# tungphambasement/DCNN

Hardware: AMD Instinct MI355X
Metric: images/sec (whole node) ResNet-18 Tiny-ImageNet training at 1/2/4/8 MI355X (higher is better)
Workload: dtype bf16; 1 GPU; model=resnet18_tiny_imagenet, global_batch=256, per_gpu_batch=256, parallelism=dp1, optimizer=adam, hipgraph=True, engine=native (C++ host API)

## Files before the change

### dcnn_amd/csrc/host/dcnn/nn.hpp

```cpp
#pragma once
#include <cmath>
#include <functional>
#include <map>
#include <memory>
#include <string>
#include <vector>

#include "json.hpp"
#include "ops.hpp"
#include "tensor.hpp"

namespace dcnn {

struct ParamArena;
struct OptimSegments;
struct Param {
  std::string name;
  std::vector<int64_t> shape;
  Layout layout = Layout::NCHW;
  Tensor value, grad, shadow;
  Tensor m, v;
  Tensor ema;
  bool no_decay = false;
  std::shared_ptr<ParamArena> arena;
};

struct ParamArena {
  Tensor value, grad, m, v, shadow;
  size_t n = 0, count = 0;
  Tensor nodecay;
  Tensor ema;
  std::shared_ptr<const OptimSegments> segments[2];
  Tensor seg_chunks, seg_info[2];
  Tensor wt_table;
  int n_wt = 0;
  long wt_tiles = 0;
  bool wt_valid = false;
  void refresh_transposes();
};

class Layer {
 public:
  explicit Layer(std::string name) : name_(std::move(name)) {}
  virtual ~Layer() = default;
  virtual std::string type() const = 0;
  virtual json::Value parameters_config() const = 0;
  virtual std::vector<int64_t> output_shape(const std::vector<int64_t>& in) const = 0;
  virtual void build(const std::vector<int64_t>& in, Device dev, uint64_t seed) { (void)in; (void)seed; dev_ = dev; }
  virtual Tensor forward(const Tensor& x, bool training) = 0;
  virtual Tensor backward(const Tensor& dy) = 0;
  virtual void sync_shadow();
  virtual void collect_params(std::vector<Param*>& out) {
    for (auto& p : params_) out.push_back(&p);
  }
  virtual void collect_layers(std::vector<Layer*>& out) { out.push_back(this); }
  std::vector<Param>& params() { return params_; }
  const std::string& name() const { return name_; }
  Device device() const { return dev_; }
  virtual void set_micro_batch(int mb) { mb_ = mb; }
  void clear_caches() { caches_.clear(); }
  void set_input_grad(bool b) { input_grad_ = b; }
  bool input_grad() const { return input_grad_; }
  virtual bool takes_raw_input(const std::vector<int64_t>& in) const { (void)in; return false; }
  virtual double flops(const std::vector<int64_t>& in) const { (void)in; return 0; }

 protected:
  struct MbCache {
    Tensor a, b, c, d;
    std::vector<int64_t> shape;
    uint64_t u = 0;
    bool flag = false;
  };
  MbCache& mbc() { return caches_[mb_]; }
  std::map<int, MbCache> caches_;
  int mb_ = 0;
  bool input_grad_ = true;
  Param& add_param(const std::string& n, const std::vector<int64_t>& shape, Layout phys, const std::vector<float>& init);
  std::string name_;
  Device dev_ = Device::cpu();
  std::vector<Param> params_;
};

class ConvBase : public Layer {
 public:
  std::vector<int64_t> output_shape(const std::vector<int64_t>& in) const override;
  void build(const std::vector<int64_t>& in, Device dev, uint64_t seed) override;
  Tensor forward(const Tensor& x, bool training) override;
  Tensor backward(const Tensor& dy) override { return backward_impl(dy, nullptr); }
  double flops(const std::vector<int64_t>& in) const override;
  virtual bool backward_residual(const Tensor& dy, const Tensor& residual, Tensor& dx) {
    (void)dy; (void)residual; (void)dx;
    return false;
  }
  int stride_h() const { return sh_; }
  int stride_w() const { return sw_; }

 protected:
  ConvBase(int in_ch, int out_ch, int kh, int kw, int groups, int sh, int sw, int ph, int pw, bool bias,
           std::string name)
      : Layer(std::move(name)), ci_(in_ch), co_(out_ch), kh_(kh), kw_(kw), g_(groups), sh_(sh), sw_(sw), ph_(ph),
        pw_(pw), bias_(bias) {}
  ConvShape shape_for(const std::vector<int64_t>& in) const;
  void geometry_config(json::Value& p) const;
  const float* bias_value() const { return bias_ ? params_[1].value.ptr<float>() : nullptr; }
  float* bias_grad() { return bias_ ? params_[1].grad.ptr<float>() : nullptr; }
  virtual bool depthwise() const { return false; }
  int group_in() const { return depthwise() ? 1 : ci_ / g_; }
  Tensor backward_impl(const Tensor& dy, const Tensor* residual);
  int ci_, co_, kh_, kw_, g_, sh_, sw_, ph_, pw_;
  bool bias_;
};

class Conv2D : public ConvBase {
 public:
  Conv2D(int in_ch, int out_ch, int kh, int kw, int sh = 1, int sw = 1, int ph = 0, int pw = 0, bool bias = true,
         std::string name = "conv2d");
  std::string type() const override { return "conv2d"; }
  json::Value parameters_config() const override;
  Tensor forward(const Tensor& x, bool training) override;
  Tensor backward(const Tensor& dy) override;
  bool takes_raw_input(const std::vector<int64_t>& in) const override;
  void set_stats_consumer(class BatchNorm* bn) { stats_to_ = bn; }
  void set_bnb_producer(class BatchNorm* bn) { bnb_from_ = bn; }
  void set_block_bnb_producer(class BatchNorm* bn) { bnb_block_from_ = bn; }
  bool backward_residual(const Tensor& dy, const Tensor& residual, Tensor& dx) override;
  bool compact_grad_ok() const;
  Tensor backward_compact(const Tensor& dy);
  bool takes_compact_residual(int sh, int sw) const;
  bool ran_stem() const;
  void backward_stem_bn(const Tensor& dy, const gpu_ops::StemBn& bn);
  void sync_shadow() override;
  bool make_transposed_operand(std::vector<int64_t>& row, long& tiles);

 private:
  class BatchNorm* stats_to_ = nullptr;
  class BatchNorm* bnb_from_ = nullptr;
  class BatchNorm* bnb_block_from_ = nullptr;
  Tensor wt_;
  const void* dgrad_operand(bool& transposed) const;
};

class DepthwiseConv2D : public ConvBase {
 public:
  DepthwiseConv2D(int channels, int kh, int kw, int sh = 1, int sw = 1, int ph = 0, int pw = 0, bool bias = true,
                  std::string name = "depthwise_conv2d");
  std::string type() const override { return "depthwise_conv2d"; }
  json::Value parameters_config() const override;
  bool backward_residual(const Tensor& dy, const Tensor& residual, Tensor& dx) override;

 protected:
  bool depthwise() const override { return true; }
};

class GroupedConv2D : public ConvBase {
 public:
  GroupedConv2D(int in_ch, int out_ch, int kh, int kw, int groups, int sh = 1, int sw = 1, int ph = 0, int pw = 0,
                bool bias = true, std::string name = "grouped_conv2d");
  std::string type() const override { return "grouped_conv2d"; }
  json::Value parameters_config() const override;
  bool backward_residual(const Tensor& dy, const Tensor& residual, Tensor& dx) override;
};

class Dense : public Layer {
 public:
  Dense(int in_features, int out_features, bool bias = true, std::string name = "dense");
  std::string type() const override { return "dense"; }
  json::Value parameters_config() const override;
  std::vector<int64_t> output_shape(const std::vector<int64_t>& in) const override;
  void build(const std::vector<int64_t>& in, Device dev, uint64_t seed) override;
  Tensor forward(const Tensor& x, bool training) override;
  Tensor backward(const Tensor& dy) override;
  double flops(const std::vector<int64_t>& in) const override { return 6.0 * in[0] * in_ * out_; }
  void set_head_pool(class Pool2D* p) { head_pool_ = p; }
  bool run_head(const Tensor& x, const PoolShape& p, Tensor& pooled);
  bool is_head_dx(const Tensor& dy, bool take);

 private:
  int in_, out_;
  bool bias_;
  class Pool2D* head_pool_ = nullptr;
};

class BatchNorm : public Layer {
 public:
  explicit BatchNorm(int num_features, float eps = 1e-5f, float momentum = 0.1f, bool affine = true,
                     std::string name = "batchnorm");
  std::string type() const override { return "batchnorm"; }
  json::Value parameters_config() const override;
  std::vector<int64_t> output_shape(const std::vector<int64_t>& in) const override { return in; }
  double flops(const std::vector<int64_t>& in) const override {
    return 15.0 * (double)in[0] * (double)in[1] * (double)in[2] * (double)in[3];
// ... 87 lines not shown
  Tensor forward(const Tensor& x, bool training) override;
  Tensor backward(const Tensor& dy) override;

 private:
  int c_;
  float eps_;
  bool affine_;
};

class LayerScale : public Layer {
 public:
  explicit LayerScale(int num_channels, float init_value = 1e-6f, std::string name = "layer_scale");
  std::string type() const override { return "layer_scale"; }
  json::Value parameters_config() const override;
  std::vector<int64_t> output_shape(const std::vector<int64_t>& in) const override { return in; }
  void build(const std::vector<int64_t>& in, Device dev, uint64_t seed) override;
  Tensor forward(const Tensor& x, bool training) override { return forward_residual(x, nullptr, training); }
  Tensor forward_residual(const Tensor& x, const Tensor* residual, bool training, const Tensor* mask = nullptr);
  Tensor backward(const Tensor& dy) override;

 private:
  int c_;
  float init_;
};

class DropPath : public Layer {
 public:
  explicit DropPath(float rate, std::string name = "drop_path", bool has_seed = false, uint64_t seed = 0);
  std::string type() const override { return "drop_path"; }
  json::Value parameters_config() const override;
  std::vector<int64_t> output_shape(const std::vector<int64_t>& in) const override { return in; }
  double flops(const std::vector<int64_t>& in) const override;
  void build(const std::vector<int64_t>& in, Device dev, uint64_t seed) override;
  Tensor forward(const Tensor& x, bool training) override;
  Tensor backward(const Tensor& dy) override;
  float rate() const { return p_; }
  uint64_t mask_seed() const { return has_seed_ ? explicit_seed_ : seed_; }
  const Tensor* draw_mask(int64_t N, bool training);
  const Tensor& last_mask() { return mbc().a; }
  Tensor& draw_counter() { return ctr_; }

 private:
  float p_;
  bool has_seed_;
  uint64_t explicit_seed_, seed_ = 0, draws_ = 0;
  Tensor ctr_;
};

class Dropout : public Layer {
 public:
  explicit Dropout(float rate = 0.5f, std::string name = "dropout");
  std::string type() const override { return "dropout"; }
  json::Value parameters_config() const override;
  std::vector<int64_t> output_shape(const std::vector<int64_t>& in) const override { return in; }
  void build(const std::vector<int64_t>& in, Device dev, uint64_t seed) override;
  Tensor forward(const Tensor& x, bool training) override;
  Tensor backward(const Tensor& dy) override;

 private:
  float p_;
  uint64_t seed_ = 0, draw_ = 0;
};

class Pool2D : public Layer {
 public:
  Pool2D(bool max, int kh, int kw, int sh, int sw, int ph, int pw, std::string name);
  std::string type() const override { return max_ ? "maxpool2d" : "avgpool2d"; }
  json::Value parameters_config() const override;
  std::vector<int64_t> output_shape(const std::vector<int64_t>& in) const override;
  Tensor forward(const Tensor& x, bool training) override;
  Tensor backward(const Tensor& dy) override;
  bool is_max() const { return max_; }
  PoolShape shape_for(const std::vector<int64_t>& in) const;
  void set_fused_producer(class BatchNorm* bn) { bn_ = bn; }
  uint8_t* accept_prepooled(const Tensor& ypool, const std::vector<int64_t>& in);
  void clear_prepooled() { mbc().flag = false; }
  void set_head_dense(class Dense* d) { head_ = d; }

 private:
  class BatchNorm* bn_ = nullptr;
  class Dense* head_ = nullptr;
  bool max_;
  int kh_, kw_, sh_, sw_, ph_, pw_;
};

class Flatten : public Layer {
 public:
  explicit Flatten(std::string name = "flatten") : Layer(std::move(name)) {}
  std::string type() const override { return "flatten"; }
  json::Value parameters_config() const override { return json::Value::object(); }
  std::vector<int64_t> output_shape(const std::vector<int64_t>& in) const override;
  Tensor forward(const Tensor& x, bool training) override;
  Tensor backward(const Tensor& dy) override;
  void set_head_dense(class Dense* d) { head_ = d; }

 private:
  class Dense* head_ = nullptr;
};

class ResidualBlock : public Layer {
 public:
  ResidualBlock(std::vector<std::unique_ptr<Layer>> main, std::vector<std::unique_ptr<Layer>> shortcut,
                std::string activation = "relu", std::string name = "residual_block");
  std::string type() const override { return "residual_block"; }
  json::Value parameters_config() const override;
  std::vector<int64_t> output_shape(const std::vector<int64_t>& in) const override;
  double flops(const std::vector<int64_t>& in) const override;
  void build(const std::vector<int64_t>& in, Device dev, uint64_t seed) override;
  Tensor forward(const Tensor& x, bool training) override;
  Tensor backward(const Tensor& dy) override;
  void sync_shadow() override;
  void collect_params(std::vector<Param*>& out) override;
  void collect_layers(std::vector<Layer*>& out) override;
  void set_micro_batch(int mb) override;
  const std::vector<std::unique_ptr<Layer>>& main_path() const { return main_; }
  const std::vector<std::unique_ptr<Layer>>& shortcut_path() const { return short_; }
  class BatchNorm* fused_tail() const;
  class Conv2D* head_conv() const;
  class BatchNorm* dual_shortcut() const;
  class LayerScale* scale_tail() const;
  class DropPath* drop_tail() const;

 private:
  std::vector<std::unique_ptr<Layer>> main_, short_;
  std::string act_;
};

std::unique_ptr<Layer> create_layer(const json::Value& rec);

void fuse_bn_relu(std::vector<std::unique_ptr<Layer>>& seq, bool on);
void fuse_blocks(std::vector<std::unique_ptr<Layer>>& seq, bool on);

class Sequential {
 public:
  explicit Sequential(std::string name = "sequential") : name_(std::move(name)) {}
  Sequential(Sequential&&) = default;
  Sequential& operator=(Sequential&&) = default;
  void add(std::unique_ptr<Layer> l) { layers_.push_back(std::move(l)); }
  void set_input_shape(const std::vector<int64_t>& chw) { input_chw_ = chw; }
  void set_device(Device d);
  Device device() const { return dev_; }
  void initialize(uint64_t seed = 0);
  void set_training(bool t) { training_ = t; }
  bool is_training() const { return training_; }
  Tensor forward(const Tensor& x, int mb = 0);
  void backward(const Tensor& dlogits, int mb = 0);
  Tensor forward_activation(const Tensor& x, int mb);
  Tensor backward_activation(const Tensor& g, int mb);
  Tensor input_activation(const Tensor& x) const;
  std::vector<Param*> parameters();
  std::vector<double> layer_flops(const std::vector<int64_t>& in) const;
  std::vector<BatchNorm*> batchnorms();
  void zero_grad();
  size_t num_parameters();
  const std::vector<std::unique_ptr<Layer>>& layers() const { return layers_; }
  const std::string& name() const { return name_; }
  void set_backward_hook(std::function<void(size_t)> f) { bwd_hook_ = std::move(f); }

  json::Value get_config() const;
  void print_config() const;
  static Sequential load_from_config(const json::Value& cfg);
  void save_to_file(const std::string& path) const;
  void load_weights_file(const std::string& path);
  void load_bn_stats(const std::string& path);
  static Sequential from_file(const std::string& path, Device dev = Device::cpu());

 private:
  std::string name_;
  std::vector<std::unique_ptr<Layer>> layers_;
  std::vector<int64_t> input_chw_;
  Device dev_ = Device::cpu();
  bool training_ = true;
  bool initialized_ = false;
  std::shared_ptr<ParamArena> arena_;
  std::function<void(size_t)> bwd_hook_;
  void pack_params();
};

class SequentialBuilder {
 public:
  explicit SequentialBuilder(std::string name = "sequential") : model_(std::move(name)) {}
  SequentialBuilder& input(const std::vector<int64_t>& chw);
  SequentialBuilder& conv2d(int out_ch, int kh, int kw, int sh = 1, int sw = 1, int ph = 0, int pw = 0,
                            bool bias = true, const std::string& name = "");
  SequentialBuilder& depthwise_conv2d(int kh, int kw, int sh = 1, int sw = 1, int ph = 0, int pw = 0, bool bias = true,
                                      const std::string& name = "");
  SequentialBuilder& grouped_conv2d(int out_ch, int kh, int kw, int groups, int sh = 1, int sw = 1, int ph = 0,
                                    int pw = 0, bool bias = true, const std::string& name = "");
  SequentialBuilder& batchnorm(float eps = 1e-5f, float momentum = 0.1f, bool affine = true,
                               const std::string& name = "");
  SequentialBuilder& activation(const std::string& kind = "relu", const std::string& name = "");
  SequentialBuilder& maxpool2d(int kh, int kw, int sh = 0, int sw = 0, int ph = 0, int pw = 0,
                               const std::string& name = "");
  SequentialBuilder& avgpool2d(int kh, int kw, int sh = 1, int sw = 1, int ph = 0, int pw = 0,
                               const std::string& name = "");
  SequentialBuilder& flatten(const std::string& name = "");
  SequentialBuilder& dense(int out_features, bool bias = true, const std::string& name = "");
  SequentialBuilder& groupnorm(int num_groups, float eps = 1e-5f, bool affine = true, const std::string& name = "");
  SequentialBuilder& dropout(float rate, const std::string& name = "");
  SequentialBuilder& drop_path(float rate, const std::string& name = "");
  SequentialBuilder& layernorm(float eps = 1e-6f, bool affine = true, const std::string& name = "");
  SequentialBuilder& layer_scale(float init_value = 1e-6f, const std::string& name = "");
  SequentialBuilder& convnext_block(int channels, float layer_scale_init = 1e-6f, const std::string& name = "",
                                    float drop_path = 0.f, bool has_seed = false, uint64_t drop_path_seed = 0);
  SequentialBuilder& convnext_downsample(int out_ch, const std::string& name = "convnext_downsample");
  SequentialBuilder& residual(std::vector<std::unique_ptr<Layer>> main, std::vector<std::unique_ptr<Layer>> shortcut,
                              const std::string& activation = "relu", const std::string& name = "");
  SequentialBuilder& basic_residual_block(int in_ch, int out_ch, int stride = 1, const std::string& name = "");
  SequentialBuilder& bottleneck_residual_block(int in_ch, int mid_ch, int out_ch, int stride = 1,
                                               const std::string& name = "");
  SequentialBuilder& resnext_bottleneck_block(int in_ch, int mid_ch, int out_ch, int groups, int stride = 1,
                                              const std::string& name = "");
  Sequential build();

 private:
  std::string auto_name(const std::string& given, const std::string& kind);
  int conv_in() const;
  SequentialBuilder& add_conv(std::unique_ptr<Layer> l);
  Sequential model_;
  std::vector<int64_t> cur_;
  int count_ = 0;
};

struct LossResult {
  double loss = 0;
  long correct = 0;
  Tensor grad;
};
LossResult softmax_cross_entropy(const Tensor& logits, const Tensor& labels);

class Optimizer {
 public:
  explicit Optimizer(float lr) : lr_(lr) {}
  virtual ~Optimizer() = default;
  virtual void step(const std::vector<Param*>& params) = 0;
  void set_learning_rate(float lr) { lr_ = lr; }
  float learning_rate() const { return lr_; }
  void set_max_grad_norm(float max_norm);
  float max_grad_norm() const { return max_norm_; }
  void set_ema_decay(float decay);
  float ema_decay() const { return ema_decay_; }
  void set_no_decay_norm_bias(bool on) { no_decay_ = on; }
  bool no_decay_norm_bias() const { return no_decay_; }
  void prepare(const std::vector<Param*>& params);
  void swap_ema(const std::vector<Param*>& params);
  float last_grad_norm() const;
  virtual bool capturable() const { return false; }
  virtual long step_count() const { return t_; }
  virtual void set_step_count(long t) { t_ = t; }
  virtual void before_replay();
  virtual void upload_hyper();

 protected:
  bool tail() const { return max_norm_ > 0.f || ema_decay_ > 0.f; }
  const float* launch_norm(ParamArena* a);
  const double* host_coef(const std::vector<Param*>& params);
  template <class Owner>
  float* ema_of(Owner* x) const {
    return ema_decay_ > 0.f ? x->ema.template ptr<float>() : nullptr;
  }
  void sync_hyper(ParamArena* a, const char* what);
  float lr_;
  float max_norm_ = 0.f, ema_decay_ = 0.f;
  bool no_decay_ = false;
  long t_ = 0;
  Tensor norm_;
  float host_norm_ = std::nanf("");
  double host_coef_ = 1.0;
  Tensor hyper_;
  float hyper_lr_ = -1.f;
  long hyper_t_ = -1;
};

class SGD : public Optimizer {
 public:
  explicit SGD(float lr, float momentum = 0.f) : Optimizer(lr), momentum_(momentum) {}
  void step(const std::vector<Param*>& params) override;
  float momentum() const { return momentum_; }

 private:
  float momentum_;
};

class Adam : public Optimizer {
 public:
  explicit Adam(float lr, float b1 = 0.9f, float b2 = 0.999f, float eps = 1e-8f, float wd = 0.f,
                bool decoupled = false)
      : Optimizer(lr), b1_(b1), b2_(b2), eps_(eps), wd_(wd), decoupled_(decoupled) {}
  void step(const std::vector<Param*>& params) override;
  bool capturable() const override { return true; }
  void before_replay() override;

 protected:
  float b1_, b2_, eps_, wd_;
  bool decoupled_;
};

class LayerwiseState {
 public:
  std::vector<float> last_trust_ratios() const;

 protected:
  void workspace(ParamArena* a);
  struct One {
    std::vector<int> chunks, segs;
  };
  static One one_segment(long n, bool adapt);
  template <class StepOne>
  void step_each(const std::vector<Param*>& params, const char* who, bool no_decay, StepOne step_one);
  Tensor part_, out_;
  size_t nsegs_ = 0;
  std::vector<double> trust_;
};

class LAMB : public Adam, public LayerwiseState {
 public:
  explicit LAMB(float lr = 1e-3f, double b1 = 0.9, double b2 = 0.999, float eps = 1e-6f, float wd = 0.01f)
      : Adam(lr, (float)b1, (float)b2, eps, wd, false), b1d_(b1), b2d_(b2) {}
  void step(const std::vector<Param*>& params) override;

 private:
  double b1d_, b2d_;
};

class LARS : public SGD, public LayerwiseState {
 public:
  explicit LARS(float lr = 0.1f, float momentum = 0.9f, float wd = 5e-4f, float trust_coefficient = 1e-3f,
                float eps = 1e-8f)
      : SGD(lr, momentum), wd_(wd), tc_(trust_coefficient), eps_(eps) {}
  void step(const std::vector<Param*>& params) override;
  bool capturable() const override { return true; }

 private:
  float wd_, tc_, eps_;
};


class DataSource {
 public:
  virtual ~DataSource() = default;
  virtual void reset(uint64_t epoch) = 0;
  virtual bool next(int batch, Tensor& x, Tensor& labels) = 0;
  virtual size_t size() const = 0;
};

class SyntheticClassification : public DataSource {
 public:
  SyntheticClassification(size_t n, int c, int h, int w, int classes, uint64_t seed, float noise = 0.5f);
  void reset(uint64_t epoch) override;
  bool next(int batch, Tensor& x, Tensor& labels) override;
  size_t size() const override { return n_; }

 private:
  size_t n_;
  int c_, h_, w_, classes_;
  uint64_t seed_;
  float noise_;
  std::vector<float> proto_;
  std::vector<size_t> order_;
  size_t pos_ = 0;
};

struct TrainingConfig {
  int epochs = 1;
  int batch_size = 64;
  int max_steps = -1;
  int progress_interval = 50;
  float lr_decay = 1.0f;
  uint64_t seed = 0;
};

struct EpochStats {
  double train_loss = 0, train_acc = 0, val_loss = 0, val_acc = 0, seconds = 0;
};

LossResult train_step(Sequential& model, Optimizer& opt, const Tensor& x, const Tensor& labels);
EpochStats evaluate(Sequential& model, DataSource& src, int batch_size);
std::vector<EpochStats> train_classification_model(Sequential& model, DataSource& train, DataSource* val,
                                                   Optimizer& opt, const TrainingConfig& cfg);

}
```

### dcnn_amd/csrc/host/dcnn/ops.hpp

```cpp
#pragma once
#include <cstdint>

namespace dcnn {

struct ConvShape {
  int N, C, H, W, Co, KH, KW, SH, SW, PH, PW, OH, OW;
};
struct PoolShape {
  int N, C, H, W, OH, OW, KH, KW, SH, SW, PH, PW;
};
enum ActKind {
  ACT_RELU = 0, ACT_LEAKY_RELU = 1, ACT_ELU = 2, ACT_SIGMOID = 3, ACT_TANH = 4, ACT_LINEAR = 5,
  ACT_GELU = 6
};

struct MixPlan {
  int mode;
  double lam;
  int yl, yh, xl, xh;
};

namespace cpu_ops {
void conv_fwd(const float* x, const float* w, const float* b, float* y, const ConvShape& s);
void conv_bwd(const float* x, const float* w, const float* dy, float* dx, float* dw, float* db, const ConvShape& s);
void dwconv_fwd(const float* x, const float* w, const float* b, float* y, const ConvShape& s);
void dwconv_bwd(const float* x, const float* w, const float* dy, float* dx, float* dw, float* db, const ConvShape& s);
void gconv_fwd(const float* x, const float* w, const float* b, float* y, const ConvShape& s, int groups);
void gconv_bwd(const float* x, const float* w, const float* dy, float* dx, float* dw, float* db, const ConvShape& s,
               int groups);
void dense_fwd(const float* x, const float* w, const float* b, float* y, long N, long In, long Out);
void dense_bwd(const float* x, const float* w, const float* dy, float* dx, float* dw, float* db, long N, long In,
               long Out);
void bn_fwd(const float* x, float* y, long N, long C, long HW, const float* g, const float* b, float eps, bool train,
            float* rmean, float* rvar, float momentum, float* smean, float* sistd);
void bn_bwd(const float* x, const float* dy, const float* mean, const float* istd, const float* g, float* dx,
            float* dg, float* db, long N, long C, long HW, bool train);
void maxpool_fwd(const float* x, float* y, int32_t* idx, const PoolShape& p);
void maxpool_bwd(const float* dy, const int32_t* idx, float* dx, const PoolShape& p);
void avgpool_fwd(const float* x, float* y, const PoolShape& p);
void avgpool_bwd(const float* dy, float* dx, const PoolShape& p);
void act_fwd(int kind, const float* x, float* y, long n, float alpha);
void act_bwd(int kind, const float* x, const float* dy, float* dx, long n, float alpha);
double softmax_ce(const float* pred, const int64_t* labels, float* grad, long N, long C, long* correct);
double loss(int kind, const float* pred, const float* target, const int64_t* labels, float* grad, long N, long C,
            float param, long* correct);
void groupnorm_fwd(const float* x, float* y, long N, long C, long HW, long G, const float* g, const float* b, float eps,
                   float* smean, float* sistd);
void groupnorm_bwd(const float* x, const float* dy, const float* mean, const float* istd, const float* g, float* dx,
                   float* dg, float* db, long N, long C, long HW, long G);
void layernorm_fwd(const float* x, float* y, long N, long C, long HW, const float* g, const float* b, float eps,
                   float* smean, float* srstd);
void layernorm_bwd(const float* x, const float* dy, const float* mean, const float* rstd, const float* g, float* dx,
                   float* dg, float* db, long N, long C, long HW);
void layer_scale_fwd(const float* x, const float* g, const float* residual, float* y, long N, long C, long HW);
void layer_scale_bwd(const float* x, const float* dy, const float* g, float* dx, float* dg, long N, long C, long HW);
void softmax_fwd(const float* x, float* y, long N, long C, long HW);
void softmax_bwd(const float* y, const float* dy, float* dx, long N, long C, long HW);
void dropout(const float* x, float* y, long n, float p, uint64_t seed);
void add(const float* a, const float* b, float* y, long n, bool relu);
void relu_mask(const float* dy, const float* y, float* dx, long n);
void adam(float* p, const float* g, float* m, float* v, long n, float lr, float b1, float b2, float eps, float bc1,
          float bc2, float wd, bool decoupled);
void sgd(float* p, const float* g, float* vel, long n, float lr, float momentum);
double grad_sumsq(const float* g, long n);
void adam_tail(float* p, const float* g, float* m, float* v, long n, float lr, float b1, float b2, float eps, float bc1,
               float bc2, float wd, bool decoupled, const uint8_t* nodecay, const double* coef, float* ema,
               float decay);
void sgd_tail(float* p, const float* g, float* vel, long n, float lr, float momentum, const double* coef, float* ema,
              float decay);
void ema_swap(float* a, float* b, long n);
void lamb(float* p, const float* g, float* m, float* v, long n, float lr, double b1, double b2, float eps, double bc1,
          double bc2, float wd, const double* coef, float* ema, float decay, const int* chunks, int nchunks,
          const int* segs, int nsegs, double* out);
void lars(float* p, const float* g, float* vel, long n, float lr, float momentum, float wd, float tc, float eps,
          const double* coef, float* ema, float decay, const int* chunks, int nchunks, const int* segs, int nsegs,
          double* out);
void drop_path_mask(float* mask, long N, float p, uint64_t seed, uint64_t draw);
void drop_path_scale(const float* x, const float* mask, float* y, long N, long row);
MixPlan mix_plan(uint64_t seed, uint64_t step, int H, int W, double mixup_alpha, double cutmix_alpha, double prob,
                 double switch_prob);
void mix_batch(float* x, const int64_t* labels, float* target, long B, long C, long H, long W, int mode, double lam,
               int yl, int yh, int xl, int xh, long K);
}

namespace gpu_ops {
void begin_deferred_reduce();
void end_deferred_reduce();
void flush_deferred_reduce();
void set_fault(int f);
void input_to_nhwc(const float* x, void* y, int N, int C, int HW);
void nhwc_to_nchw(const void* x, void* y, int N, int HW, int C);
void nchw_to_nhwc_bf16(const void* x, void* y, int N, int HW, int C);
void cast_bf16(const float* x, void* y, long n);
void zero(void* p, long nbytes);
const float* conv_fwd(const void* x, const void* w, const float* bias, void* y, const ConvShape& s,
                      int* stat_rows = nullptr);
struct BnbOperands {
  const void* y;
  const void* x;
  const float* mean;
  const float* istd;
  const float* gamma = nullptr;
  const float* beta = nullptr;
  bool mask_from_x = false;
};
struct DgradOpts {
  bool residual_compact = false;
  bool dense_g2 = false;
};
const float* conv_dgrad(const void* dy, const void* w, void* dx, const ConvShape& s, const void* residual = nullptr,
                        bool w_transposed = false, const BnbOperands* bnb = nullptr, int* bnb_rows = nullptr,
                        DgradOpts opt = {});
bool conv_dgrad_takes_compact(const ConvShape& s);
void conv_dgrad_compact(const void* dy, const void* w, void* dxc, const ConvShape& s, bool w_transposed);
bool compact_shortcut_grad_enabled();
void weight_transpose(const void* w, void* wt, int Co, int T, int C);
void multi_weight_transpose(const int64_t* table, int n, long max_tiles);
void conv_wgrad(const void* dy, const void* x, float* gw, float* gb, const ConvShape& s);
void dwconv_fwd(const void* x, const void* w, const float* bias, void* y, const ConvShape& s);
void dwconv_dgrad(const void* dy, const void* w, void* dx, const ConvShape& s, const void* residual = nullptr);
void dwconv_wgrad(const void* dy, const void* x, float* gw, float* gb, const ConvShape& s);
void gconv_fwd(const void* x, const void* w, const float* bias, void* y, const ConvShape& s, int groups);
void gconv_dgrad(const void* dy, const void* w, void* dx, const ConvShape& s, int groups,
                 const void* residual = nullptr);
void gconv_wgrad(const void* dy, const void* x, float* gw, float* gb, const ConvShape& s, int groups);
bool stem_ok(const ConvShape& s);
const float* stem_fwd(const float* x, const void* w, const float* bias, void* y, const ConvShape& s,
                      int* stat_rows = nullptr);
void stem_wgrad(const void* dy, const float* x, float* gw, float* gb, const ConvShape& s);
struct StemBn {
  const void* x;
  const float* mean;
  const float* istd;
  const float* gamma;
  float* dgamma;
  float* dbeta;
  const float* slab;
  int rows;
  bool train;
};
void stem_wgrad_bn(const void* dy, const float* x, float* gw, float* gb, const ConvShape& s, const StemBn& bn);
void dense_fwd(const void* x, const void* w, const float* bias, void* y, int N, int In, int Out);
void dense_dgrad(const void* dy, const void* w, void* dx, int N, int In, int Out);
void dense_wgrad(const void* dy, const void* x, float* gw, float* gb, int N, int In, int Out);
bool head_supported(const PoolShape& p, int Out);
void head_fwd(const void* x, const void* w, const float* bias, void* pooled, void* y, const PoolShape& p, int Out);
void head_bwd(const void* dy, const void* w, const void* pooled, void* dx, float* gw, float* gb, const PoolShape& p,
              int Out);
void bn_fwd(const void* x, void* y, long R, int C, const float* g, const float* b, float eps, bool train,
            float* rmean, float* rvar, float momentum, float* smean, float* sistd, bool relu = false,
            const void* residual = nullptr);
void bn_fwd_slab(const void* x, void* y, long R, int C, const float* slab, int rows, const float* g, const float* b,
                 float eps, float* rmean, float* rvar, float momentum, float* smean, float* sistd, bool relu,
                 const void* residual = nullptr);
void bn_bwd_slab(const void* dy, const void* x, void* dx, long R, int C, const float* mean, const float* istd,
                 const float* g, float* dg, float* db, bool train, const float* slab, int rows);
void bn_bwd(const void* dy, const void* x, void* dx, long R, int C, const float* mean, const float* istd,
            const float* g, float* dg, float* db, bool train, const void* yout = nullptr, void* dy_out = nullptr);
struct SecondaryStats {
  SecondaryStats();
  ~SecondaryStats();
};
struct BnRaw {
  const float* slab;
  int rows;
};
BnRaw bn_stats_raw(const void* x, long R, int C, const float* slab, int rows);
struct BnFwdSide {
  const void* x;
  BnRaw raw;
  const float* g;
  const float* b;
  float eps;
  float* rmean;
  float* rvar;
  float momentum;
  float* smean;
  float* sistd;
};
bool bn_dual_ok(long R, int C);
void bn_fwd_dual(const BnFwdSide& a, const BnFwdSide& b, void* y, long R, int C, bool relu, bool train);
struct BnBwdSides {
  const void* x;
  void* dx;
  const float* mean;
  const float* istd;
  const float* g;
  float* dg;
  float* db;
};
void bn_bwd_dual(const void* dy, const BnBwdSides& a, const float* slab_a, int rows_a, const BnBwdSides& b, long R,
                 int C);
bool bn_relu_maxpool_ok(const PoolShape& p);
void bn_relu_maxpool(const void* x, void* y, uint8_t* idx, const PoolShape& p, const float* slab, int rows,
                     const float* g, const float* b, float eps, float* rmean, float* rvar, float momentum,
                     float* smean, float* sistd);
const float* maxpool_bwd_bnb(const void* dy, const uint8_t* idx, const void* ypool, const void* x, const float* mean,
                             const float* istd, void* dx, const PoolShape& p, int* rows);
void maxpool_fwd(const void* x, void* y, uint8_t* idx, const PoolShape& p);
void maxpool_bwd(const void* dy, const uint8_t* idx, void* dx, const PoolShape& p);
void avgpool_fwd(const void* x, void* y, const PoolShape& p);
void avgpool_bwd(const void* dy, void* dx, const PoolShape& p);
void act_fwd(int kind, const void* x, void* y, long n, float alpha);
void act_bwd(int kind, const void* x, const void* dy, void* dx, long n, float alpha);
double softmax_ce(const void* pred, const int64_t* labels, void* grad, int N, int C, long* correct);
double loss(int kind, const void* pred, const float* target, const int64_t* labels, void* grad, int N, int C,
            float param, long* correct, float grad_scale = 1.f);
void loss_launch(int kind, const void* pred, const float* target, const int64_t* labels, void* grad, int N, int C,
                 float param, float grad_scale = 1.f);
double read_last_loss(long* correct);
void groupnorm_fwd(const void* x, void* y, int N, int HW, int C, int G, const float* g, const float* b, float eps,
                   float* smean, float* sistd);
void groupnorm_bwd(const void* dy, const void* x, void* dx, int N, int HW, int C, int G, const float* g,
                   const float* mean, const float* istd, float* dg, float* db);
void layernorm_fwd(const void* x, void* y, long R, int C, const float* g, const float* b, float eps, float* smean,
                   float* srstd);
void layernorm_bwd(const void* dy, const void* x, void* dx, long R, int C, const float* g, const float* mean,
                   const float* rstd, float* dg, float* db);
void layer_scale_fwd(const void* x, const float* g, const void* residual, void* y, long R, int C);
void layer_scale_bwd(const void* dy, const void* x, const float* g, void* dx, float* dg, long R, int C);
void softmax_fwd(const void* x, void* y, long rows, int C);
void softmax_bwd(const void* y, const void* dy, void* dx, long rows, int C);
void dropout(const void* x, void* y, long n, float p, uint64_t seed);
void add(const void* a, const void* b, void* y, long n, bool relu);
void relu_mask(const void* dy, const void* y, void* dx, long n);
void adam(float* p, const float* g, float* m, float* v, void* shadow, long n, float lr, float b1, float b2, float eps,
          float bc1, float bc2, float wd, bool decoupled);
void sgd(float* p, const float* g, float* vel, void* shadow, long n, float lr, float momentum);
void adam_hyper_step(float* hyper, float b1, float b2);
void adam_dev(float* p, const float* g, float* m, float* v, void* shadow, long n, float b1, float b2, float eps,
              float wd, bool decoupled, const float* hyper, const uint8_t* nodecay);
void grad_norm_workspace(long n);
void grad_sumsq(const float* g, long n, float max_norm, float* out);
void adam_tail(float* p, const float* g, float* m, float* v, void* shadow, long n, float lr, float b1, float b2,
               float eps, float bc1, float bc2, float wd, bool decoupled, const float* hyper, const uint8_t* nodecay,
               const float* coef, float* ema, float decay);
void sgd_tail(float* p, const float* g, float* vel, void* shadow, long n, float lr, float momentum, const float* coef,
              float* ema, float decay);
void ema_swap(float* a, float* b, void* shadow, long n);
void layerwise_workspace();
// ... 21 lines not shown
```

### dcnn_amd/csrc/host/dcnn/tensor.hpp

```cpp
#pragma once
#include <cstdint>
#include <cstring>
#include <iosfwd>
#include <memory>
#include <string>
#include <vector>

#include "layout.hpp"

namespace dcnn {

enum class DeviceType { CPU, GPU };

struct Device {
  DeviceType type = DeviceType::CPU;
  int index = 0;
  static Device cpu() { return {DeviceType::CPU, 0}; }
  static Device gpu(int i = 0) { return {DeviceType::GPU, i}; }
  static Device parse(const std::string& s);
  bool is_gpu() const { return type == DeviceType::GPU; }
  std::string str() const;
  bool operator==(const Device& o) const { return type == o.type && index == o.index; }
  bool operator!=(const Device& o) const { return !(*this == o); }
};

enum class DType { F32, BF16, I32, I64, U8 };
size_t dtype_size(DType t);
const char* dtype_name(DType t);

uint16_t f32_to_bf16(float f);
float bf16_to_f32(uint16_t b);

namespace gpu {
int device_count();
void set_device(int dev);
void* alloc(size_t nbytes);
void free(void* p);
size_t cached_bytes();
void empty_cache();
void copy(void* dst, const void* src, size_t nbytes, int kind);
void copy2_d2d(void* d0, const void* s0, size_t n0, void* d1, const void* s1, size_t n1);
void zero(void* p, size_t nbytes);
void synchronize();

using Flow = void*;
using Event = void*;
Flow flow();
void set_flow(Flow f);
Flow flow_create();
void flow_destroy(Flow f);
void flow_synchronize(Flow f = nullptr);
Event event_create();
void event_destroy(Event e);
void event_record(Event e, Flow f = nullptr);
void flow_wait(Flow f, Event e);
void event_synchronize(Event e);

class Graph {
 public:
  Graph() = default;
  ~Graph();
  Graph(const Graph&) = delete;
  Graph& operator=(const Graph&) = delete;
  void begin();
  void end();
  void replay();
  bool ready() const { return exec_ != nullptr; }
  static bool capturing();

 private:
  void* graph_ = nullptr;
  void* exec_ = nullptr;
  void* pool_ = nullptr;
  Flow flow_ = nullptr;
};
constexpr size_t kIpcHandleBytes = 64;
void* ipc_alloc(size_t nbytes, void* handle_out);
void ipc_free(void* p);
void* ipc_open(const void* handle);
void ipc_close(void* p);
bool stream_values_supported();
Event ipc_event_create(void* handle_out);
Event ipc_event_open(const void* handle);
void flow_write_u32(void* p, uint32_t v);
void flow_wait_u32_geq(void* p, uint32_t v);
}

class Storage {
 public:
  Storage(Device d, size_t nbytes);
  ~Storage();
  Storage(const Storage&) = delete;
  Storage& operator=(const Storage&) = delete;
  void* data() const { return p_; }
  size_t nbytes() const { return n_; }
  Device device() const { return dev_; }

 private:
  Device dev_;
  void* p_ = nullptr;
  size_t n_ = 0;
};

class Tensor {
 public:
  Tensor() = default;
  static Tensor empty(const std::vector<int64_t>& shape, DType dt, Device dev, Layout layout = Layout::NCHW);
  static Tensor zeros(const std::vector<int64_t>& shape, DType dt, Device dev, Layout layout = Layout::NCHW);
  static Tensor from_host(const std::vector<float>& v, const std::vector<int64_t>& shape, Device dev,
                          DType dt = DType::F32, Layout layout = Layout::NCHW);
  static Tensor from_host_i64(const std::vector<int64_t>& v, Device dev);

  bool defined() const { return (bool)st_; }
  const std::vector<int64_t>& shape() const { return shape_; }
  int64_t dim(int k) const { return shape_.at(k); }
  int rank() const { return (int)shape_.size(); }
  int64_t numel() const;
  size_t nbytes() const { return (size_t)numel() * dtype_size(dt_); }
  DType dtype() const { return dt_; }
  Device device() const { return st_ ? st_->device() : Device::cpu(); }
  Layout layout() const { return layout_; }
  void* data() const { return st_ ? static_cast<char*>(st_->data()) + off_ : nullptr; }
  template <typename T>
  T* ptr() const { return static_cast<T*>(data()); }

  Tensor view(const std::vector<int64_t>& shape, Layout layout = Layout::NCHW) const;
  Tensor slice(size_t byte_off, const std::vector<int64_t>& shape, DType dt, Layout layout = Layout::NCHW) const;
  void ensure(const std::vector<int64_t>& shape, DType dt, Device dev, Layout layout = Layout::NCHW);
  Tensor clone() const;
  Tensor to(Device dev) const;
  std::vector<float> to_host_f32() const;
  std::vector<int64_t> to_host_i64() const;
  void zero_();

  void save(std::ostream& os) const;
  static Tensor load(std::istream& is, Device dev = Device::cpu());

 private:
  std::shared_ptr<Storage> st_;
  size_t off_ = 0;
  std::vector<int64_t> shape_;
  DType dt_ = DType::F32;
  Layout layout_ = Layout::NCHW;
};

std::string shape_str(const std::vector<int64_t>& s);

}
```

### dcnn_amd/csrc/host/nn.cpp

```cpp
#include "dcnn/nn.hpp"

#include "../kernels/fusion_plan.h"
#include "../kernels/optim_segments.h"

#include <algorithm>
#include <chrono>
#include <cmath>
#include <cstdio>
#include <cstdlib>
#include <filesystem>
#include <fstream>
#include <iostream>
#include <sstream>
#include <stdexcept>

namespace dcnn {

namespace {
struct Rng {
  uint64_t s;
  explicit Rng(uint64_t seed) : s(seed * 0x9e3779b97f4a7c15ull + 0x632be59bd9b4e019ull) {}
  uint64_t next() {
    uint64_t z = (s += 0x9e3779b97f4a7c15ull);
    z = (z ^ (z >> 30)) * 0xbf58476d1ce4e5b9ull;
    z = (z ^ (z >> 27)) * 0x94d049bb133111ebull;
    return z ^ (z >> 31);
  }
  float uniform() { return (float)((next() >> 40) * (1.0 / 16777216.0)); }
  float normal() {
    const float u1 = std::max(uniform(), 1e-7f), u2 = uniform();
    return std::sqrt(-2.f * std::log(u1)) * std::cos(6.2831853f * u2);
  }
};

std::vector<float> uniform_init(size_t n, float bound, uint64_t seed) {
  Rng r(seed);
  std::vector<float> v(n);
  for (auto& x : v) x = (2.f * r.uniform() - 1.f) * bound;
  return v;
}

Tensor act_empty(const std::vector<int64_t>& shape, Device dev) {
  return dev.is_gpu() ? Tensor::empty(shape, DType::BF16, dev, Layout::NHWC) : Tensor::empty(shape, DType::F32, dev);
}

void check_act(const Tensor& x, Device dev, const char* who) {
  if (x.device() != dev) throw std::runtime_error(std::string(who) + ": input on " + x.device().str() +
                                                  ", layer on " + dev.str());
  if (x.rank() != 4) throw std::runtime_error(std::string(who) + ": expected an (N, C, H, W) tensor");
}

constexpr int ACT_SOFTMAX = 100;

int act_code(const std::string& k) {
  if (k == "softmax") return ACT_SOFTMAX;
  if (k == "relu") return ACT_RELU;
  if (k == "leaky_relu") return ACT_LEAKY_RELU;
  if (k == "elu") return ACT_ELU;
  if (k == "sigmoid") return ACT_SIGMOID;
  if (k == "tanh") return ACT_TANH;
  if (k == "linear") return ACT_LINEAR;
  if (k == "gelu") return ACT_GELU;
  throw std::invalid_argument("unknown activation '" + k + "'");
}
}

Param& Layer::add_param(const std::string& n, const std::vector<int64_t>& shape, Layout phys,
                        const std::vector<float>& init) {
  Param p;
  p.name = n;
  p.shape = shape;
  p.layout = phys;
  p.value = Tensor::from_host(init, shape, dev_, DType::F32, phys);
  p.grad = Tensor::zeros(shape, DType::F32, dev_, phys);
  if (dev_.is_gpu()) {
    p.shadow = Tensor::empty(shape, DType::BF16, dev_, phys);
    gpu_ops::cast_bf16(p.value.ptr<float>(), p.shadow.data(), p.value.numel());
  }
  params_.push_back(std::move(p));
  return params_.back();
}

void Layer::sync_shadow() {
  for (auto& p : params_)
    if (p.shadow.defined()) gpu_ops::cast_bf16(p.value.ptr<float>(), p.shadow.data(), p.value.numel());
}

void ConvBase::geometry_config(json::Value& p) const {
  p["stride_h"] = sh_;
  p["stride_w"] = sw_;
  p["pad_h"] = ph_;
  p["pad_w"] = pw_;
  p["use_bias"] = bias_;
}

ConvShape ConvBase::shape_for(const std::vector<int64_t>& in) const {
  ConvShape s{};
  s.N = (int)in[0];
  s.C = (int)in[1];
  s.H = (int)in[2];
  s.W = (int)in[3];
  s.Co = co_;
  s.KH = kh_;
  s.KW = kw_;
  s.SH = sh_;
  s.SW = sw_;
  s.PH = ph_;
  s.PW = pw_;
  s.OH = (s.H + 2 * ph_ - kh_) / sh_ + 1;
  s.OW = (s.W + 2 * pw_ - kw_) / sw_ + 1;
  if (s.C != ci_) throw std::runtime_error(name_ + ": input has " + std::to_string(s.C) + " channels, expected " +
                                           std::to_string(ci_));
  return s;
}

std::vector<int64_t> ConvBase::output_shape(const std::vector<int64_t>& in) const {
  const ConvShape s = shape_for(in);
  return {in[0], co_, s.OH, s.OW};
}

void ConvBase::build(const std::vector<int64_t>& in, Device dev, uint64_t seed) {
  (void)in;
  dev_ = dev;
  params_.clear();
  const int cig = group_in();
  const float bound = 1.f / std::sqrt((float)(cig * kh_ * kw_));
  const Layout wl = dev.is_gpu() && !depthwise() ? Layout::NHWC : Layout::NCHW;
  add_param("weights", {co_, cig, kh_, kw_}, wl, uniform_init((size_t)co_ * cig * kh_ * kw_, bound, seed));
  if (bias_) add_param("bias", {co_, 1, 1, 1}, Layout::NCHW, uniform_init((size_t)co_, bound, seed + 1)).no_decay = true;
}

double ConvBase::flops(const std::vector<int64_t>& in) const {
  const ConvShape s = shape_for(in);
  const double out = (double)s.N * s.OH * s.OW, k = (double)group_in() * kh_ * kw_;
  return 6.0 * co_ * k * out + (bias_ ? 2.0 * co_ * out : 0.0);
}

Tensor ConvBase::forward(const Tensor& x, bool training) {
  (void)training;
  check_act(x, dev_, type().c_str());
  const ConvShape s = shape_for(x.shape());
  Tensor y = act_empty({s.N, s.Co, s.OH, s.OW}, dev_);
  const float* b = bias_value();
  if (dev_.is_gpu()) {
    const void* w = params_[0].shadow.data();
    if (depthwise())
      gpu_ops::dwconv_fwd(x.data(), w, b, y.data(), s);
    else
      gpu_ops::gconv_fwd(x.data(), w, b, y.data(), s, g_);
  } else {
    const float* w = params_[0].value.ptr<float>();
    if (depthwise())
      cpu_ops::dwconv_fwd(x.ptr<float>(), w, b, y.ptr<float>(), s);
    else
      cpu_ops::gconv_fwd(x.ptr<float>(), w, b, y.ptr<float>(), s, g_);
  }
// ... 1487 lines not shown
    if (p.get_bool("has_projection", false)) sc = path("shortcut_path");
    return std::make_unique<ResidualBlock>(std::move(main), std::move(sc), p.get_string("activation", "relu"), name);
  }
  throw std::invalid_argument("C++ host API: unsupported layer type '" + type + "'");
}

namespace {
void assign_values(Tensor& dst, const std::vector<float>& v, const std::vector<int64_t>& shape, Layout layout) {
  const Tensor h = Tensor::from_host(v, shape, Device::cpu(), DType::F32, layout);
  if (h.nbytes() != dst.nbytes()) throw std::runtime_error("parameter size mismatch");
  if (dst.device().is_gpu())
    gpu::copy(dst.data(), h.data(), h.nbytes(), 0);
  else
    std::memcpy(dst.data(), h.data(), h.nbytes());
}
}

void Sequential::pack_params() {
  arena_.reset();
  std::vector<Param*> ps = parameters();
  if (ps.empty() || !dev_.is_gpu()) return;
  auto A = std::make_shared<ParamArena>();
  std::vector<size_t> off;
  for (Param* p : ps) {
    off.push_back(A->n);
    A->n += ((size_t)p->value.numel() + 63) / 64 * 64;
  }
  A->count = ps.size();
  const int64_t n = (int64_t)A->n;
  A->value = Tensor::zeros({n}, DType::F32, dev_);
  A->grad = Tensor::zeros({n}, DType::F32, dev_);
  A->m = Tensor::zeros({n}, DType::F32, dev_);
  A->v = Tensor::zeros({n}, DType::F32, dev_);
  A->shadow = Tensor::zeros({n}, DType::BF16, dev_);
  for (size_t k = 0; k < ps.size(); ++k) {
    Param* p = ps[k];
    const auto& sh = p->value.shape();
    const Layout lay = p->value.layout();
    Tensor nv = A->value.slice(off[k] * 4, sh, DType::F32, lay);
    gpu::copy(nv.data(), p->value.data(), p->value.nbytes(), 2);
    p->value = nv;
    p->grad = A->grad.slice(off[k] * 4, sh, DType::F32, lay);
    p->m = A->m.slice(off[k] * 4, sh, DType::F32, lay);
    p->v = A->v.slice(off[k] * 4, sh, DType::F32, lay);
    Tensor ns = A->shadow.slice(off[k] * 2, sh, DType::BF16, lay);
    if (p->shadow.defined()) gpu::copy(ns.data(), p->shadow.data(), p->shadow.nbytes(), 2);
    p->shadow = ns;
    p->arena = A;
  }
  {
    std::vector<uint8_t> tab(A->n / 64, 0);
    for (size_t k = 0; k < ps.size(); ++k)
      if (ps[k]->no_decay)
        for (size_t b = off[k] / 64; b < (off[k] + (size_t)ps[k]->value.numel() + 63) / 64; ++b) tab[b] = 1;
    A->nodecay = Tensor::empty({(int64_t)tab.size()}, DType::U8, dev_);
    gpu::copy(A->nodecay.data(), tab.data(), tab.size(), 0);
  }
  {
    std::vector<long> offs, counts;
    std::vector<unsigned char> flags;
    for (size_t k = 0; k < ps.size(); ++k) {
      offs.push_back((long)off[k]);
      counts.push_back((long)ps[k]->value.numel());
      flags.push_back(ps[k]->no_decay ? 1 : 0);
    }
    for (int e = 0; e < 2; ++e) {
      auto t = std::make_shared<OptimSegments>(
          build_optim_segments(offs.data(), counts.data(), flags.data(), (int)ps.size(), e == 1, (long)A->n));
      check_optim_segments(t->chunks.data(), (int)t->chunks.size(), t->segs.data(), (int)t->segs.size(), (long)A->n);
      A->seg_info[e] = Tensor::empty({(int64_t)(t->segs.size() * sizeof(SegInfo))}, DType::U8, dev_);
      gpu::copy(A->seg_info[e].data(), t->segs.data(), t->segs.size() * sizeof(SegInfo), 0);
      if (e == 0 && !t->chunks.empty()) {
        A->seg_chunks = Tensor::empty({(int64_t)(t->chunks.size() * sizeof(SegChunk))}, DType::U8, dev_);
        gpu::copy(A->seg_chunks.data(), t->chunks.data(), t->chunks.size() * sizeof(SegChunk), 0);
      }
      A->segments[e] = t;
    }
  }
  std::vector<Layer*> all;
  for (auto& l : layers_) l->collect_layers(all);
  std::vector<int64_t> table;
  for (Layer* l : all) {
    auto* c = dynamic_cast<Conv2D*>(l);
    std::vector<int64_t> row;
    long tiles = 0;
    if (c == nullptr || !c->make_transposed_operand(row, tiles)) continue;
    table.insert(table.end(), row.begin(), row.end());
    ++A->n_wt;
    A->wt_tiles = std::max(A->wt_tiles, tiles);
  }
  if (A->n_wt) {
    A->wt_table = Tensor::empty({(int64_t)table.size()}, DType::I64, dev_);
    gpu::copy(A->wt_table.data(), table.data(), table.size() * 8, 0);
    A->refresh_transposes();
  }
  arena_ = A;
}

void Sequential::set_device(Device d) {
  if (d.is_gpu() && gpu::device_count() <= d.index) throw std::runtime_error(d.str() + " not available");
  if (initialized_ && d != dev_) {
    std::vector<std::vector<float>> vals;
    for (auto* p : parameters()) vals.push_back(p->value.to_host_f32());
    dev_ = d;
    initialized_ = false;
    initialize(0);
    size_t i = 0;
    for (auto* p : parameters()) assign_values(p->value, vals[i++], p->shape, p->layout);
    for (auto& l : layers_) l->sync_shadow();
    return;
  }
  dev_ = d;
}

void Sequential::initialize(uint64_t seed) {
  if (input_chw_.empty()) {
    input_chw_ = {0, 0, 0};
  }
  std::vector<int64_t> shape{1, input_chw_[0], input_chw_[1], input_chw_[2]};
  fuse_bn_relu(layers_, dev_.is_gpu());
  uint64_t k = 0;
  for (auto& l : layers_) {
    l->build(shape, dev_, seed * 1000003ull + (k++) * 7919ull);
    if (shape[1] > 0 && shape[2] > 0) shape = l->output_shape(shape);
  }
  fuse_blocks(layers_, dev_.is_gpu());
  pack_params();
  initialized_ = true;
}

std::vector<Param*> Sequential::parameters() {
  std::vector<Param*> out;
  for (auto& l : layers_) l->collect_params(out);
  return out;
}

std::vector<BatchNorm*> Sequential::batchnorms() {
  std::vector<Layer*> all;
  for (auto& l : layers_) l->collect_layers(all);
  std::vector<BatchNorm*> out;
  for (auto* l : all)
    if (auto* bn = dynamic_cast<BatchNorm*>(l)) out.push_back(bn);
  return out;
}

size_t Sequential::num_parameters() {
  size_t n = 0;
  for (auto* p : parameters()) n += (size_t)p->value.numel();
  return n;
}

void Sequential::zero_grad() {
  if (arena_) {
    gpu_ops::zero(arena_->grad.data(), (long)arena_->grad.nbytes());
    return;
  }
  for (auto* p : parameters()) {
    if (dev_.is_gpu())
      gpu_ops::zero(p->grad.data(), (long)p->grad.nbytes());
    else
      p->grad.zero_();
  }
}

std::vector<double> Sequential::layer_flops(const std::vector<int64_t>& in) const {
  std::vector<double> out;
  std::vector<int64_t> s = in;
  for (auto& l : layers_) {
    out.push_back(l->flops(s));
    s = l->output_shape(s);
  }
  return out;
}

Tensor Sequential::input_activation(const Tensor& x_in) const {
  if (x_in.rank() != 4 || x_in.dtype() != DType::F32) throw std::runtime_error("forward: expected fp32 (N, C, H, W)");
  Tensor x = x_in.device() == dev_ ? x_in : x_in.to(dev_);
  if (dev_.is_gpu() && !layers_.empty() && layers_[0]->takes_raw_input(x.shape())) return x;
  if (dev_.is_gpu()) {
    Tensor a = Tensor::empty(x.shape(), DType::BF16, dev_, Layout::NHWC);
    gpu_ops::input_to_nhwc(x.ptr<float>(), a.data(), (int)x.dim(0), (int)x.dim(1), (int)(x.dim(2) * x.dim(3)));
    x = a;
  }
  return x;
}

Tensor Sequential::forward_activation(const Tensor& x_in, int mb) {
  if (!initialized_) throw std::runtime_error("Sequential::forward before initialize()");
  Tensor x = x_in;
  for (auto& l : layers_) {
    l->set_micro_batch(mb);
    x = l->forward(x, training_);
  }
  return x;
}

Tensor Sequential::backward_activation(const Tensor& g_in, int mb) {
  Tensor g = g_in;
  static const bool defer_env = [] {
    const char* v = std::getenv("DCNN_DEFER_REDUCE");
    return !(v && std::string(v) == "0");
  }();
  const bool defer = dev_.is_gpu() && defer_env;
  static const bool stem_bn_env = [] {
    const char* v = std::getenv("DCNN_STEM_BN_FOLD");
    return !(v && std::string(v) == "0");
  }();
  const bool stem_bn_fold = dev_.is_gpu() && stem_bn_env && layers_.size() > 1;
  if (defer) gpu_ops::begin_deferred_reduce();
  try {
    for (size_t i = layers_.size(); i-- > 0;) {
      layers_[i]->set_micro_batch(mb);
      if (i == 1 && stem_bn_fold) {
        auto* bn = dynamic_cast<BatchNorm*>(layers_[1].get());
        auto* conv = dynamic_cast<Conv2D*>(layers_[0].get());
        if (bn && conv) {
          conv->set_micro_batch(mb);
          if (bn->backward_into_stem(g, *conv)) {
            if (bwd_hook_) bwd_hook_(1);
            if (bwd_hook_) bwd_hook_(0);
            g = Tensor();
            break;
          }
        }
      }
      g = layers_[i]->backward(g);
      if (bwd_hook_) bwd_hook_(i);
    }
  } catch (...) {
    if (defer) gpu_ops::end_deferred_reduce();
    throw;
  }
  if (defer) gpu_ops::end_deferred_reduce();
  return g;
}

Tensor Sequential::forward(const Tensor& x_in, int mb) {
  Tensor x = forward_activation(input_activation(x_in), mb);
  return x.view({x.dim(0), x.dim(1) * x.dim(2) * x.dim(3)}, x.layout());
}

void Sequential::backward(const Tensor& dlogits, int mb) {
  if (!layers_.empty()) layers_[0]->set_input_grad(false);
  Tensor g = dlogits.view({dlogits.dim(0), dlogits.dim(1), 1, 1}, dev_.is_gpu() ? Layout::NHWC : Layout::NCHW);
  backward_activation(g, mb);
}

json::Value Sequential::get_config() const {
  json::Value c = json::Value::object();
  c["name"] = name_;
  c["is_training"] = training_;
  json::Value ls = json::Value::array();
  for (auto& l : layers_) {
    json::Value r = json::Value::object();
    r["type"] = l->type();
    r["name"] = l->name();
    r["parameters"] = l->parameters_config();
    ls.push(std::move(r));
  }
  c["layers"] = std::move(ls);
  if (!input_chw_.empty() && input_chw_[0] > 0) {
    json::Value in = json::Value::array();
    for (auto v : input_chw_) in.push(v);
    c["input_shape"] = std::move(in);
  }
  return c;
}

void Sequential::print_config() const { std::cout << get_config().dump(2) << std::endl; }

Sequential Sequential::load_from_config(const json::Value& cfg) {
  Sequential m(cfg.get_string("name", "sequential"));
  for (auto& r : cfg.at("layers").items()) m.add(create_layer(r));
  m.set_training(cfg.get_bool("is_training", true));
  if (const json::Value* in = cfg.find("input_shape")) {
    std::vector<int64_t> chw;
    for (auto& v : in->items()) chw.push_back(v.as_int());
    m.set_input_shape(chw);
  }
  return m;
}

void Sequential::save_to_file(const std::string& path) const {
  const std::filesystem::path dir = std::filesystem::path(path).parent_path();
  if (!dir.empty()) std::filesystem::create_directories(dir);
  {
    std::ofstream f(path + ".json");
    if (!f) throw std::runtime_error("cannot write " + path + ".json");
    f << get_config().dump(4);
  }
  std::ofstream f(path + ".bin", std::ios::binary);
  if (!f) throw std::runtime_error("cannot write " + path + ".bin");
  auto& self = const_cast<Sequential&>(*this);
  for (auto* p : self.parameters()) p->value.view(p->shape, p->layout).save(f);
  std::ofstream s(path + ".bnstats", std::ios::binary);
  for (auto* bn : self.batchnorms()) {
    const int64_t c = bn->running_mean.numel();
    bn->running_mean.view({c, 1, 1, 1}).save(s);
    bn->running_var.view({c, 1, 1, 1}).save(s);
  }
}

void Sequential::load_bn_stats(const std::string& path) {
  std::ifstream f(path, std::ios::binary);
  if (!f) throw std::runtime_error("cannot read " + path);
  for (auto* bn : batchnorms()) {
    const int64_t c = bn->running_mean.numel();
    Tensor m = Tensor::load(f), v = Tensor::load(f);
    if (m.numel() != c || v.numel() != c) throw std::runtime_error("bnstats: channel count mismatch");
    bn->running_mean = Tensor::from_host(m.to_host_f32(), {c}, dev_);
    bn->running_var = Tensor::from_host(v.to_host_f32(), {c}, dev_);
  }
}

void Sequential::load_weights_file(const std::string& path) {
  if (!initialized_) initialize(0);
  std::ifstream f(path, std::ios::binary);
  if (!f) throw std::runtime_error("cannot read " + path);
  for (auto* p : parameters()) {
    Tensor t = Tensor::load(f);
    if (t.numel() != p->value.numel())
      throw std::runtime_error("checkpoint tensor " + shape_str(t.shape()) + " does not match parameter " +
                               shape_str(p->shape));
    assign_values(p->value, t.to_host_f32(), p->shape, p->layout);
  }
  for (auto& l : layers_) l->sync_shadow();
}

Sequential Sequential::from_file(const std::string& path, Device dev) {
  std::ifstream f(path + ".json");
  if (!f) throw std::runtime_error("cannot read " + path + ".json");
  std::stringstream ss;
  ss << f.rdbuf();
  Sequential m = load_from_config(json::Value::parse(ss.str()));
  m.set_device(dev);
  m.initialize(0);
  m.load_weights_file(path + ".bin");
  if (std::ifstream(path + ".bnstats").good()) m.load_bn_stats(path + ".bnstats");
  return m;
}

std::string SequentialBuilder::auto_name(const std::string& given, const std::string& kind) {
  ++count_;
  return given.empty() ? kind + "_" + std::to_string(count_) : given;
}

SequentialBuilder& SequentialBuilder::input(const std::vector<int64_t>& chw) {
  if (chw.size() != 3) throw std::invalid_argument("input: expected {C, H, W}");
  cur_ = chw;
  model_.set_input_shape(chw);
  return *this;
}

int SequentialBuilder::conv_in() const {
  if (cur_.empty()) throw std::logic_error("SequentialBuilder: call input() first");
  return (int)cur_[0];
}

SequentialBuilder& SequentialBuilder::add_conv(std::unique_ptr<Layer> l) {
  const auto o = l->output_shape({1, cur_[0], cur_[1], cur_[2]});
  cur_ = {o[1], o[2], o[3]};
  model_.add(std::move(l));
  return *this;
}

SequentialBuilder& SequentialBuilder::conv2d(int out_ch, int kh, int kw, int sh, int sw, int ph, int pw, bool bias,
                                             const std::string& name) {
  const int ci = conv_in();
  return add_conv(std::make_unique<Conv2D>(ci, out_ch, kh, kw, sh, sw, ph, pw, bias, auto_name(name, "conv2d")));
}

SequentialBuilder& SequentialBuilder::depthwise_conv2d(int kh, int kw, int sh, int sw, int ph, int pw, bool bias,
                                                       const std::string& name) {
  const int c = conv_in();
  return add_conv(
      std::make_unique<DepthwiseConv2D>(c, kh, kw, sh, sw, ph, pw, bias, auto_name(name, "depthwise_conv2d")));
}

SequentialBuilder& SequentialBuilder::grouped_conv2d(int out_ch, int kh, int kw, int groups, int sh, int sw, int ph,
                                                     int pw, bool bias, const std::string& name) {
  const int ci = conv_in();
  return add_conv(std::make_unique<GroupedConv2D>(ci, out_ch, kh, kw, groups, sh, sw, ph, pw, bias,
                                                  auto_name(name, "grouped_conv2d")));
// ... 154 lines not shown

LossResult softmax_cross_entropy(const Tensor& logits, const Tensor& labels_in) {
  if (logits.rank() != 2) throw std::runtime_error("softmax_cross_entropy: expected [N, C] logits");
  const int N = (int)logits.dim(0), C = (int)logits.dim(1);
  const Device dev = logits.device();
  Tensor labels = labels_in.device() == dev ? labels_in : labels_in.to(dev);
  LossResult r;
  if (dev.is_gpu()) {
    r.grad = Tensor::empty({N, C}, DType::BF16, dev, Layout::NHWC);
    r.loss = gpu_ops::softmax_ce(logits.data(), labels.ptr<int64_t>(), r.grad.data(), N, C, &r.correct);
  } else {
    r.grad = Tensor::empty({N, C}, DType::F32, dev);
    r.loss = cpu_ops::softmax_ce(logits.ptr<float>(), labels.ptr<int64_t>(), r.grad.ptr<float>(), N, C, &r.correct);
  }
  return r;
}

namespace {
ParamArena* whole_arena(const std::vector<Param*>& params) {
  if (params.empty() || !params[0]->arena || params[0]->arena->count != params.size()) return nullptr;
  ParamArena* a = params[0]->arena.get();
  for (auto* p : params)
    if (p->arena.get() != a) return nullptr;
  return a;
}

float* state_of(const Param* p, Tensor& state) {
  if (!state.defined()) state = Tensor::zeros(p->value.shape(), DType::F32, p->value.device());
  return state.ptr<float>();
}
}

void Optimizer::set_max_grad_norm(float max_norm) {
  if (!(max_norm >= 0.f) || std::isinf(max_norm))
    throw std::invalid_argument("max_grad_norm " + std::to_string(max_norm) + " is not a finite value >= 0");
  max_norm_ = max_norm;
}

void Optimizer::set_ema_decay(float decay) {
  if (!(decay >= 0.f && decay < 1.f))
    throw std::invalid_argument("ema_decay " + std::to_string(decay) + " is not in [0, 1)");
  ema_decay_ = decay;
}

void Optimizer::prepare(const std::vector<Param*>& params) {
  if (!tail()) return;
  if (ParamArena* a = whole_arena(params)) {
    if (ema_decay_ > 0.f && !a->ema.defined()) a->ema = a->value.clone();
    if (max_norm_ > 0.f) {
      if (!norm_.defined()) norm_ = Tensor::zeros({4}, DType::F32, a->value.device());
      gpu_ops::grad_norm_workspace((long)a->n);
    }
    return;
  }
  for (auto* p : params) {
    if (p->value.device().is_gpu())
      throw std::runtime_error("gradient clipping / weight EMA on the GPU need all parameters of one arena");
    if (ema_decay_ > 0.f && !p->ema.defined()) p->ema = p->value.clone();
  }
}

const float* Optimizer::launch_norm(ParamArena* a) {
  if (!(max_norm_ > 0.f)) return nullptr;
  gpu_ops::grad_sumsq(a->grad.ptr<float>(), (long)a->n, max_norm_, norm_.ptr<float>());
  return norm_.ptr<float>() + 2;
}

const double* Optimizer::host_coef(const std::vector<Param*>& params) {
  if (!(max_norm_ > 0.f)) return nullptr;
  double sumsq = 0.0;
  for (auto* p : params) sumsq += cpu_ops::grad_sumsq(p->grad.ptr<float>(), p->value.numel());
  const double norm = std::sqrt(sumsq), c = max_norm_ / (norm + 1e-6);
  host_norm_ = (float)norm;
  host_coef_ = c < 1.0 || c != c ? c : 1.0;
  return &host_coef_;
}

void Optimizer::upload_hyper() {
  if (!hyper_.defined()) return;
  const float h[4] = {lr_, 0.f, 0.f, (float)t_};
  gpu::copy(hyper_.data(), h, sizeof h, 0);
  hyper_lr_ = lr_;
  hyper_t_ = t_;
}

void Optimizer::before_replay() {
  if (hyper_.defined() && hyper_lr_ != lr_) {
    gpu::copy(hyper_.data(), &lr_, sizeof lr_, 0);
    hyper_lr_ = lr_;
  }
}

void Optimizer::sync_hyper(ParamArena* a, const char* what) {
  if (!hyper_.defined()) hyper_ = Tensor::zeros({4}, DType::F32, a->value.device());
  if (hyper_lr_ != lr_ || hyper_t_ != t_) {
    if (gpu::Graph::capturing()) throw std::runtime_error(std::string(what) + " changed inside a graph capture");
    upload_hyper();
  }
}

float Optimizer::last_grad_norm() const {
  if (!(max_norm_ > 0.f)) return std::nanf("");
  if (!norm_.defined()) return host_norm_;
  gpu::flow_synchronize();
  float h[4];
  gpu::copy(h, norm_.data(), sizeof h, 1);
  return h[1];
}

void Optimizer::swap_ema(const std::vector<Param*>& params) {
  if (!(ema_decay_ > 0.f)) return;
  prepare(params);
  if (ParamArena* a = whole_arena(params)) {
    gpu_ops::ema_swap(a->value.ptr<float>(), a->ema.ptr<float>(), a->shadow.data(), (long)a->n);
    a->refresh_transposes();
    return;
  }
  for (auto* p : params) cpu_ops::ema_swap(p->value.ptr<float>(), p->ema.ptr<float>(), p->value.numel());
}

void SGD::step(const std::vector<Param*>& params) {
  if (tail()) prepare(params);
  if (ParamArena* a = whole_arena(params)) {
    float* vel = momentum_ != 0.f ? a->m.ptr<float>() : nullptr;
    if (tail())
      gpu_ops::sgd_tail(a->value.ptr<float>(), a->grad.ptr<float>(), vel, a->shadow.data(), (long)a->n, lr_, momentum_,
                        launch_norm(a), ema_of(a), ema_decay_);
    else
      gpu_ops::sgd(a->value.ptr<float>(), a->grad.ptr<float>(), vel, a->shadow.data(), (long)a->n, lr_, momentum_);
    a->refresh_transposes();
    return;
  }
  const double* coef = host_coef(params);
  for (auto* p : params) {
    if (p->arena) p->arena->wt_valid = false;
    float* vel = momentum_ != 0.f ? state_of(p, p->m) : nullptr;
    if (tail())
      cpu_ops::sgd_tail(p->value.ptr<float>(), p->grad.ptr<float>(), vel, p->value.numel(), lr_, momentum_, coef,
                        ema_of(p), ema_decay_);
    else if (p->value.device().is_gpu())
      gpu_ops::sgd(p->value.ptr<float>(), p->grad.ptr<float>(), vel, p->shadow.data(), p->value.numel(), lr_,
                   momentum_);
    else
      cpu_ops::sgd(p->value.ptr<float>(), p->grad.ptr<float>(), vel, p->value.numel(), lr_, momentum_);
  }
}

void Adam::before_replay() {
  Optimizer::before_replay();
  ++t_;
  ++hyper_t_;
}

void Adam::step(const std::vector<Param*>& params) {
  if (tail()) prepare(params);
  if (ParamArena* a = whole_arena(params)) {
    sync_hyper(a, "Adam: step scalars");
    ++t_;
    ++hyper_t_;
    gpu_ops::adam_hyper_step(hyper_.ptr<float>(), b1_, b2_);
    const uint8_t* nodecay = no_decay_ ? static_cast<const uint8_t*>(a->nodecay.data()) : nullptr;
    if (tail())
      gpu_ops::adam_tail(a->value.ptr<float>(), a->grad.ptr<float>(), a->m.ptr<float>(), a->v.ptr<float>(),
                         a->shadow.data(), (long)a->n, 0.f, b1_, b2_, eps_, 1.f, 1.f, wd_, decoupled_,
                         hyper_.ptr<float>(), nodecay, launch_norm(a), ema_of(a), ema_decay_);
    else
      gpu_ops::adam_dev(a->value.ptr<float>(), a->grad.ptr<float>(), a->m.ptr<float>(), a->v.ptr<float>(),
                        a->shadow.data(), (long)a->n, b1_, b2_, eps_, wd_, decoupled_, hyper_.ptr<float>(), nodecay);
    a->refresh_transposes();
    return;
  }
  ++t_;
  const float bc1 = 1.f - std::pow(b1_, (float)t_), bc2 = 1.f - std::pow(b2_, (float)t_);
  const double* coef = host_coef(params);
  for (auto* p : params) {
    if (p->arena) p->arena->wt_valid = false;
    float *m = state_of(p, p->m), *v = state_of(p, p->v);
    const float wd = no_decay_ && p->no_decay ? 0.f : wd_;
    if (tail())
      cpu_ops::adam_tail(p->value.ptr<float>(), p->grad.ptr<float>(), m, v, p->value.numel(), lr_, b1_, b2_, eps_, bc1,
                         bc2, wd, decoupled_, nullptr, coef, ema_of(p), ema_decay_);
    else if (p->value.device().is_gpu())
      gpu_ops::adam(p->value.ptr<float>(), p->grad.ptr<float>(), m, v, p->shadow.data(), p->value.numel(), lr_, b1_,
                    b2_, eps_, bc1, bc2, wd, decoupled_);
    else
      cpu_ops::adam(p->value.ptr<float>(), p->grad.ptr<float>(), m, v, p->value.numel(), lr_, b1_, b2_, eps_, bc1, bc2,
                    wd, decoupled_);
  }
}

void LayerwiseState::workspace(ParamArena* a) {
  const OptimSegments& t = *a->segments[0];
  if (part_.defined() && nsegs_ == t.segs.size()) return;
  if (gpu::Graph::capturing()) throw std::runtime_error("layer-wise optimizer: workspace created inside a graph capture");
  nsegs_ = t.segs.size();
  part_ = Tensor::zeros({(int64_t)std::max<size_t>((size_t)kSegPartFloats * t.chunks.size(), 1)}, DType::F32, a->value.device());
  out_ = Tensor::zeros({(int64_t)std::max<size_t>(3 * nsegs_, 1)}, DType::F32, a->value.device());
  gpu_ops::layerwise_workspace();
}

LayerwiseState::One LayerwiseState::one_segment(long n, bool adapt) {
  const long off = 0;
  const OptimSegments t = build_optim_segments(&off, &n, nullptr, 1, false, (n + kSegBlock - 1) / kSegBlock * kSegBlock);
  One o;
  for (const SegChunk& c : t.chunks) o.chunks.insert(o.chunks.end(), {c.first_block, c.blocks, c.segment});
  for (const SegInfo& g : t.segs) o.segs.insert(o.segs.end(), {g.first_chunk, g.chunks, adapt ? 1 : 0, adapt ? 1 : 0});
  return o;
}

std::vector<float> LayerwiseState::last_trust_ratios() const {
  if (!out_.defined()) return std::vector<float>(trust_.begin(), trust_.end());
  gpu::flow_synchronize();
  std::vector<float> h(nsegs_);
  if (nsegs_) gpu::copy(h.data(), out_.data(), nsegs_ * sizeof(float), 1);
  return h;
}

template <class StepOne>
void LayerwiseState::step_each(const std::vector<Param*>& params, const char* who, bool no_decay, StepOne step_one) {
  trust_.assign(params.size(), 1.0);
  for (size_t i = 0; i < params.size(); ++i) {
    Param* p = params[i];
    if (p->value.device().is_gpu())
      throw std::runtime_error(std::string(who) + " on the GPU needs all parameters of one arena");
    const One o = one_segment((long)p->value.numel(), !(no_decay && p->no_decay));
    double out[3] = {1.0, 0.0, 0.0};
    step_one(p, o.chunks.data(), (int)o.chunks.size() / 3, o.segs.data(), out);
    trust_[i] = out[0];
  }
}

void LAMB::step(const std::vector<Param*>& params) {
  if (tail()) prepare(params);
  if (ParamArena* a = whole_arena(params)) {
    workspace(a);
    sync_hyper(a, "LAMB: step scalars");
    ++t_;
    ++hyper_t_;
    gpu_ops::lamb_scalars(hyper_.ptr<float>(), b1d_, b2d_);
    const OptimSegments& t = *a->segments[no_decay_ ? 1 : 0];
    gpu_ops::lamb(a->value.ptr<float>(), a->grad.ptr<float>(), a->m.ptr<float>(), a->v.ptr<float>(), a->shadow.data(),
                  (long)a->n, lr_, b1d_, b2d_, eps_, 1.f, 1.f, wd_, hyper_.ptr<float>(), launch_norm(a), ema_of(a),
                  ema_decay_, a->seg_chunks.data(), (int)t.chunks.size(), a->seg_info[no_decay_ ? 1 : 0].data(),
                  (int)t.segs.size(), t.cover, part_.ptr<float>(), out_.ptr<float>());
    a->refresh_transposes();
    return;
  }
  ++t_;
  const double bc1 = 1.0 - std::pow(b1d_, (double)t_), bc2 = 1.0 - std::pow(b2d_, (double)t_);
  const double* coef = host_coef(params);
  step_each(params, "LAMB", no_decay_, [&](Param* p, const int* chunks, int nchunks, const int* segs, double* out) {
    float *m = state_of(p, p->m), *v = state_of(p, p->v);
    cpu_ops::lamb(p->value.ptr<float>(), p->grad.ptr<float>(), m, v, (long)p->value.numel(), lr_, b1d_, b2d_, eps_,
                  bc1, bc2, wd_, coef, ema_of(p), ema_decay_, chunks, nchunks, segs, 1, out);
  });
}

void LARS::step(const std::vector<Param*>& params) {
  if (tail()) prepare(params);
  const float mom = momentum();
  if (ParamArena* a = whole_arena(params)) {
    workspace(a);
    sync_hyper(a, "LARS: the learning rate");
    const OptimSegments& t = *a->segments[no_decay_ ? 1 : 0];
    gpu_ops::lars(a->value.ptr<float>(), a->grad.ptr<float>(), mom != 0.f ? a->m.ptr<float>() : nullptr,
                  a->shadow.data(), (long)a->n, lr_, mom, wd_, tc_, eps_, hyper_.ptr<float>(), launch_norm(a),
                  ema_of(a), ema_decay_, a->seg_chunks.data(), (int)t.chunks.size(),
                  a->seg_info[no_decay_ ? 1 : 0].data(), (int)t.segs.size(), t.cover, part_.ptr<float>(),
                  out_.ptr<float>());
    a->refresh_transposes();
    return;
  }
  const double* coef = host_coef(params);
  step_each(params, "LARS", no_decay_, [&](Param* p, const int* chunks, int nchunks, const int* segs, double* out) {
    cpu_ops::lars(p->value.ptr<float>(), p->grad.ptr<float>(), mom != 0.f ? state_of(p, p->m) : nullptr,
                  (long)p->value.numel(), lr_, mom, wd_, tc_, eps_, coef, ema_of(p), ema_decay_, chunks, nchunks, segs,
                  1, out);
  });
}

SyntheticClassification::SyntheticClassification(size_t n, int c, int h, int w, int classes, uint64_t seed,
                                                 float noise)
    : n_(n), c_(c), h_(h), w_(w), classes_(classes), seed_(seed), noise_(noise) {
  Rng r(seed ^ 0x5151u);
  proto_.resize((size_t)classes * c * h * w);
  for (auto& v : proto_) v = r.normal();
  order_.resize(n);
  for (size_t i = 0; i < n; ++i) order_[i] = i;
}

void SyntheticClassification::reset(uint64_t epoch) {
  Rng r(seed_ + 977 * (epoch + 1));
  for (size_t i = n_; i > 1; --i) std::swap(order_[i - 1], order_[(size_t)(r.next() % i)]);
  pos_ = 0;
}

bool SyntheticClassification::next(int batch, Tensor& x, Tensor& labels) {
  if (pos_ >= n_) return false;
  const int b = (int)std::min<size_t>((size_t)batch, n_ - pos_);
  const size_t per = (size_t)c_ * h_ * w_;
  std::vector<float> xs((size_t)b * per);
  std::vector<int64_t> ys((size_t)b);
  for (int i = 0; i < b; ++i) {
    const size_t idx = order_[pos_ + i];
    Rng r(seed_ * 1315423911ull + idx);
    const int cls = (int)(idx % (size_t)classes_);
    ys[i] = cls;
    const float* pr = proto_.data() + (size_t)cls * per;
    for (size_t k = 0; k < per; ++k) xs[i * per + k] = pr[k] + noise_ * r.normal();
  }
  pos_ += (size_t)b;
  x = Tensor::from_host(xs, {b, c_, h_, w_}, Device::cpu());
  labels = Tensor::from_host_i64(ys, Device::cpu());
  return true;
// ... 72 lines not shown
```

### dcnn_amd/csrc/host/ops_gpu.hip

```cpp
#include <hip/hip_runtime.h>

#include <algorithm>
#include <cmath>
#include <cstdio>
#include <cstdlib>
#include <cstring>
#include <map>
#include <mutex>
#include <stdexcept>
#include <string>
#include <unordered_map>
#include <vector>

#include "../kernels/api.h"
#include "dcnn/ops.hpp"
#include "dcnn/tensor.hpp"

#define HOST_HIP_CHECK(x)                                                                    \
  do {                                                                                       \
    hipError_t e_ = (x);                                                                     \
    if (e_ != hipSuccess) throw std::runtime_error(std::string(#x) + ": " + hipGetErrorString(e_)); \
  } while (0)

namespace dcnn {

namespace gpu {
namespace {
struct CapturePool {
  std::map<std::pair<int, size_t>, std::vector<void*>> free_blocks;
  std::vector<void*> owned;
};
struct BlockPool {
  std::mutex mu;
  std::map<std::pair<int, size_t>, std::vector<void*>> free_blocks;
  std::unordered_map<void*, std::pair<int, size_t>> owner;
  std::unordered_map<void*, CapturePool*> graph_owned;
  size_t cached = 0;
};
BlockPool& pool() {
  static BlockPool* p = new BlockPool;
  return *p;
}
thread_local CapturePool* t_capture = nullptr;
size_t size_class(size_t n) {
  if (n <= 512) return 512;
  int lg = 63 - __builtin_clzll((unsigned long long)(n - 1));
  const size_t step = (size_t)1 << (lg - 1);
  return (n + step - 1) / step * step;
}
void release_cached(BlockPool& bp) {
  HOST_HIP_CHECK(hipDeviceSynchronize());
  for (auto& kv : bp.free_blocks)
    for (void* p : kv.second) {
      bp.owner.erase(p);
      (void)hipFree(p);
    }
  bp.free_blocks.clear();
  bp.cached = 0;
}
}

int device_count() {
  int n = 0;
  if (hipGetDeviceCount(&n) != hipSuccess) return 0;
  return n;
}
void set_device(int dev) { HOST_HIP_CHECK(hipSetDevice(dev)); }
void* alloc(size_t nbytes) {
  int dev = 0;
  HOST_HIP_CHECK(hipGetDevice(&dev));
  const size_t cls = size_class(nbytes);
  BlockPool& bp = pool();
  std::lock_guard<std::mutex> g(bp.mu);
  CapturePool* cp = t_capture;
  if (cp) {
    auto it = cp->free_blocks.find({dev, cls});
    if (it != cp->free_blocks.end() && !it->second.empty()) {
      void* p = it->second.back();
      it->second.pop_back();
      return p;
    }
  }
  void* p = nullptr;
  auto it = bp.free_blocks.find({dev, cls});
  if (it != bp.free_blocks.end() && !it->second.empty()) {
    p = it->second.back();
    it->second.pop_back();
    bp.cached -= cls;
  } else {
    const hipError_t e = hipMalloc(&p, cls);
    if (e != hipSuccess) {
      (void)hipGetLastError();
      if (cp) throw std::runtime_error(std::string("gpu::alloc: hipMalloc failed while capturing a graph: ") +
                                       hipGetErrorString(e));
      release_cached(bp);
      HOST_HIP_CHECK(hipMalloc(&p, cls));
    }
    bp.owner[p] = {dev, cls};
  }
  if (cp) {
    bp.graph_owned[p] = cp;
    cp->owned.push_back(p);
  }
  return p;
}
void free(void* p) {
  if (p == nullptr) return;
  BlockPool& bp = pool();
  std::lock_guard<std::mutex> g(bp.mu);
  auto it = bp.owner.find(p);
  if (it == bp.owner.end()) {
    (void)hipFree(p);
    return;
  }
  auto gi = bp.graph_owned.find(p);
  if (gi != bp.graph_owned.end()) {
    gi->second->free_blocks[it->second].push_back(p);
    return;
  }
  bp.free_blocks[it->second].push_back(p);
  bp.cached += it->second.second;
}
size_t cached_bytes() {
  BlockPool& bp = pool();
  std::lock_guard<std::mutex> g(bp.mu);
  return bp.cached;
}
void empty_cache() {
  BlockPool& bp = pool();
  std::lock_guard<std::mutex> g(bp.mu);
  release_cached(bp);
}
namespace {
thread_local hipStream_t t_flow = nullptr;
thread_local hipStream_t t_default[64] = {};
}
Flow flow() {
  if (t_flow) return t_flow;
  int dev = 0;
  HOST_HIP_CHECK(hipGetDevice(&dev));
  if (!t_default[dev]) HOST_HIP_CHECK(hipStreamCreate(&t_default[dev]));
  return t_default[dev];
}
void set_flow(Flow f) { t_flow = static_cast<hipStream_t>(f); }
Flow flow_create() {
  hipStream_t s = nullptr;
  HOST_HIP_CHECK(hipStreamCreate(&s));
  return s;
}
void flow_destroy(Flow f) {
  if (f) (void)hipStreamDestroy(static_cast<hipStream_t>(f));
}
void flow_synchronize(Flow f) { HOST_HIP_CHECK(hipStreamSynchronize(static_cast<hipStream_t>(f ? f : flow()))); }
Event event_create() {
  hipEvent_t e = nullptr;
  HOST_HIP_CHECK(hipEventCreateWithFlags(&e, hipEventDisableTiming));
  return e;
}
void event_destroy(Event e) {
  if (e) (void)hipEventDestroy(static_cast<hipEvent_t>(e));
}
void event_record(Event e, Flow f) {
  HOST_HIP_CHECK(hipEventRecord(static_cast<hipEvent_t>(e), static_cast<hipStream_t>(f ? f : flow())));
}
void flow_wait(Flow f, Event e) {
  HOST_HIP_CHECK(hipStreamWaitEvent(static_cast<hipStream_t>(f ? f : flow()), static_cast<hipEvent_t>(e), 0));
}
void event_synchronize(Event e) { HOST_HIP_CHECK(hipEventSynchronize(static_cast<hipEvent_t>(e))); }

void copy(void* dst, const void* src, size_t nbytes, int kind) {
  static const hipMemcpyKind k[] = {hipMemcpyHostToDevice, hipMemcpyDeviceToHost, hipMemcpyDeviceToDevice};
  hipStream_t s = static_cast<hipStream_t>(flow());
  HOST_HIP_CHECK(hipMemcpyAsync(dst, src, nbytes, k[kind], s));
  if (kind != 2) {
    if (Graph::capturing()) throw std::runtime_error("gpu::copy: a host copy inside a graph capture");
    HOST_HIP_CHECK(hipStreamSynchronize(s));
  }
}
void copy2_d2d(void* d0, const void* s0, size_t n0, void* d1, const void* s1, size_t n1) {
  copy_pair(d0, s0, (long)n0, d1, s1, (long)n1, static_cast<hipStream_t>(flow()));
}
void zero(void* p, size_t nbytes) { HOST_HIP_CHECK(hipMemsetAsync(p, 0, nbytes, static_cast<hipStream_t>(flow()))); }
void synchronize() { HOST_HIP_CHECK(hipDeviceSynchronize()); }

bool Graph::capturing() { return t_capture != nullptr; }
void Graph::begin() {
  if (t_capture) throw std::runtime_error("gpu::Graph: nested capture");
  if (exec_) throw std::runtime_error("gpu::Graph: already captured");
  flow_ = flow();
  auto* cp = new CapturePool;
  pool_ = cp;
  HOST_HIP_CHECK(hipStreamSynchronize(static_cast<hipStream_t>(flow_)));
  HOST_HIP_CHECK(hipStreamBeginCapture(static_cast<hipStream_t>(flow_), hipStreamCaptureModeRelaxed));
  t_capture = cp;
}
void Graph::end() {
  if (t_capture != pool_) throw std::runtime_error("gpu::Graph: end() without begin()");
  t_capture = nullptr;
  hipGraph_t g = nullptr;
  HOST_HIP_CHECK(hipStreamEndCapture(static_cast<hipStream_t>(flow_), &g));
  graph_ = g;
  hipGraphExec_t ex = nullptr;
  HOST_HIP_CHECK(hipGraphInstantiate(&ex, g, nullptr, nullptr, 0));
  exec_ = ex;
}
void Graph::replay() {
  if (!exec_) throw std::runtime_error("gpu::Graph: replay before capture");
  HOST_HIP_CHECK(hipGraphLaunch(static_cast<hipGraphExec_t>(exec_), static_cast<hipStream_t>(flow())));
}
Graph::~Graph() {
  if (t_capture == pool_ && pool_) {
    t_capture = nullptr;
    hipGraph_t g = nullptr;
    (void)hipStreamEndCapture(static_cast<hipStream_t>(flow_), &g);
    if (g) (void)hipGraphDestroy(g);
    (void)hipGetLastError();
  }
  if (exec_ || graph_) (void)hipDeviceSynchronize();
  if (exec_) (void)hipGraphExecDestroy(static_cast<hipGraphExec_t>(exec_));
  if (graph_) (void)hipGraphDestroy(static_cast<hipGraph_t>(graph_));
  if (auto* cp = static_cast<CapturePool*>(pool_)) {
    BlockPool& bp = pool();
    std::lock_guard<std::mutex> g(bp.mu);
    std::unordered_map<void*, bool> is_free;
    for (auto& kv : cp->free_blocks)
      for (void* p : kv.second) is_free[p] = true;
    for (void* p : cp->owned) {
      bp.graph_owned.erase(p);
      if (is_free.count(p)) {
        auto o = bp.owner.find(p);
        bp.free_blocks[o->second].push_back(p);
        bp.cached += o->second.second;
      }
    }
    delete cp;
  }
}

void* ipc_alloc(size_t nbytes, void* handle_out) {
  static_assert(sizeof(hipIpcMemHandle_t) == kIpcHandleBytes, "IPC handle size");
  void* p = nullptr;
  HOST_HIP_CHECK(hipMalloc(&p, nbytes));
  hipIpcMemHandle_t h;
  if (hipIpcGetMemHandle(&h, p) != hipSuccess) {
    (void)hipGetLastError();
    (void)hipFree(p);
    throw std::runtime_error("hipIpcGetMemHandle failed (the host must allow dmabuf IPC)");
  }
  std::memcpy(handle_out, &h, sizeof h);
  return p;
}
void ipc_free(void* p) {
  if (p != nullptr) (void)hipFree(p);
}
void* ipc_open(const void* handle) {
  hipIpcMemHandle_t h;
  std::memcpy(&h, handle, sizeof h);
  void* p = nullptr;
  HOST_HIP_CHECK(hipIpcOpenMemHandle(&p, h, hipIpcMemLazyEnablePeerAccess));
  return p;
}
void ipc_close(void* p) {
  if (p != nullptr) (void)hipIpcCloseMemHandle(p);
}
Event ipc_event_create(void* handle_out) {
  static_assert(sizeof(hipIpcEventHandle_t) == kIpcHandleBytes, "IPC event handle size");
  hipEvent_t e = nullptr;
  if (hipEventCreateWithFlags(&e, hipEventDisableTiming | hipEventInterprocess) != hipSuccess) {
    (void)hipGetLastError();
    return nullptr;
  }
  hipIpcEventHandle_t h;
  if (hipIpcGetEventHandle(&h, e) != hipSuccess) {
    (void)hipGetLastError();
    (void)hipEventDestroy(e);
    return nullptr;
  }
  std::memcpy(handle_out, &h, sizeof h);
  return e;
}
Event ipc_event_open(const void* handle) {
  hipIpcEventHandle_t h;
  std::memcpy(&h, handle, sizeof h);
  hipEvent_t e = nullptr;
  HOST_HIP_CHECK(hipIpcOpenEventHandle(&e, h));
  return e;
}
bool stream_values_supported() {
  static const bool ok = [] {
    int dev = 0, v = 0;
    if (hipGetDevice(&dev) != hipSuccess) return false;
    if (hipDeviceGetAttribute(&v, hipDeviceAttributeCanUseStreamWaitValue, dev) != hipSuccess) {
      (void)hipGetLastError();
      return false;
    }
    return v != 0;
  }();
  return ok;
}
void flow_write_u32(void* p, uint32_t v) {
  HOST_HIP_CHECK(hipStreamWriteValue32(static_cast<hipStream_t>(flow()), p, v, 0));
}
void flow_wait_u32_geq(void* p, uint32_t v) {
  HOST_HIP_CHECK(hipStreamWaitValue32(static_cast<hipStream_t>(flow()), p, v, hipStreamWaitValueGte, 0xffffffffu));
}
}

namespace gpu_ops {
namespace {
constexpr int kPlain = 0, kConvFwd = 1, kConvDgrad = 2;
constexpr int kBF16 = 1;
inline hipStream_t cur() { return static_cast<hipStream_t>(gpu::flow()); }

enum Slot { W_T = 0, SLAB, BSLAB, STAT_SLAB, STAT_SUMS, STAT_PART, LOSS_WS, LOSS_OUT, TICKETS, HPART, HTICKETS, GN_AFF,
            FWD_STATS, BWD_STATS, FWD_STATS2, STAT_SLAB2, STAT_SUMS2, STAT_PART2, LN_WS, GNORM_PART, GNORM_TICKET, LW_TICKET,
            NSLOTS };
void* scratch(Slot s, size_t bytes) {
  static void* p[NSLOTS] = {};
  static size_t n[NSLOTS] = {};
  if (n[s] < bytes) {
    if (p[s]) HOST_HIP_CHECK(hipFree(p[s]));
    HOST_HIP_CHECK(hipMalloc(&p[s], bytes));
    n[s] = bytes;
  }
  return p[s];
}

__global__ void transpose16_kernel(const uint16_t* __restrict__ in, uint16_t* __restrict__ out, int rows, int cols) {
  __shared__ uint16_t t[32][33];
  const long b = blockIdx.z;
  const uint16_t* src = in + b * rows * cols;
  uint16_t* dst = out + b * rows * cols;
  const int c0 = blockIdx.x * 32, r0 = blockIdx.y * 32;
  for (int k = threadIdx.y; k < 32; k += 8) {
    const int r = r0 + k, c = c0 + threadIdx.x;
    if (r < rows && c < cols) t[k][threadIdx.x] = src[(long)r * cols + c];
  }
  __syncthreads();
  for (int k = threadIdx.y; k < 32; k += 8) {
    const int c = c0 + k, r = r0 + threadIdx.x;
    if (r < rows && c < cols) dst[(long)c * rows + r] = t[threadIdx.x][k];
  }
}

void transpose16(const void* in, void* out, int batch, int rows, int cols) {
  dim3 grid((cols + 31) / 32, (rows + 31) / 32, batch);
  hipLaunchKernelGGL(transpose16_kernel, grid, dim3(32, 8), 0, cur(), static_cast<const uint16_t*>(in),
                     static_cast<uint16_t*>(out), rows, cols);
  HOST_HIP_CHECK(hipGetLastError());
}

PoolGeom geom(const PoolShape& p) { return PoolGeom{p.N, p.H, p.W, p.C, p.OH, p.OW, p.KH, p.KW, p.SH, p.SW, p.PH, p.PW}; }

__global__ void add_bf16_kernel(const bf16* __restrict__ a, const bf16* __restrict__ b, bf16* __restrict__ y, long n,
                                int relu) {
  for (long i = blockIdx.x * (long)blockDim.x + threadIdx.x; i < n; i += (long)gridDim.x * blockDim.x) {
    float v = (float)a[i] + (float)b[i];
    if (relu) v = fmaxf(v, 0.f);
    y[i] = (bf16)v;
  }
}
__global__ void relu_mask_bf16_kernel(const bf16* __restrict__ dy, const bf16* __restrict__ yv, bf16* __restrict__ dx,
                                      long n) {
  for (long i = blockIdx.x * (long)blockDim.x + threadIdx.x; i < n; i += (long)gridDim.x * blockDim.x)
    dx[i] = (float)yv[i] > 0.f ? dy[i] : (bf16)0.f;
}
int grid_of(long n) {
  long g = (n + 255) / 256;
  return (int)(g > 8192 ? 8192 : (g < 1 ? 1 : g));
}

FILE* rec_file() {
  static FILE* f = [] {
    const char* p = std::getenv("DCNN_RECORD_OPS");
    return p && *p ? std::fopen(p, "a") : nullptr;
  }();
  return f;
}
void rec(const char* op, const ConvShape& s, int route, std::initializer_list<std::pair<const char*, int>> flags) {
  FILE* f = rec_file();
  if (!f) return;
  std::fprintf(f, "{\"op\": \"%s\", \"shape\": [%d, %d, %d, %d, %d, %d, %d, %d, %d, %d, %d, %d, %d], \"route\": %d", op,
               s.N, s.C, s.H, s.W, s.Co, s.KH, s.KW, s.SH, s.SW, s.PH, s.PW, s.OH, s.OW, route);
  for (const auto& kv : flags) std::fprintf(f, ", \"%s\": %d", kv.first, kv.second);
  std::fprintf(f, "}\n");
  std::fflush(f);
}
int g_fault = [] {
  const char* v = std::getenv("DCNN_TEST_FAULT");
  return v && *v ? std::atoi(v) : 0;
}();

void hconv_workspace(HConvArgs& a) {
  a.splits = hconv_splits(a.NB, a.H, a.W, a.Cs, a.N, a.ntaps);
  a.part = nullptr;
  a.tickets = nullptr;
  if (a.splits <= 1) {
    a.splits = 1;
    return;
  }
  const long tiles = hconv_tiles(a.NB, a.H, a.W, a.Cs, a.N, a.ntaps);
  a.part = static_cast<float*>(scratch(HPART, (size_t)tiles * a.splits * hconv_tile_elems(a.NB, a.H, a.W, a.Cs, a.N,
                                                                                          a.ntaps) * 4));
  static size_t zeroed = 0;
  const size_t need = (size_t)tiles * 64 * 4;
  a.tickets = static_cast<unsigned*>(scratch(HTICKETS, need));
  if (zeroed < need) {
    HOST_HIP_CHECK(hipMemsetAsync(a.tickets, 0, need, cur()));
    zeroed = need;
  }
}

thread_local bool t_secondary = false;
inline Slot fwd_stats_slot() { return t_secondary ? FWD_STATS2 : FWD_STATS; }

ConvRouteGeom route_geom(const ConvShape& s, int g1s_mode) {
  return ConvRouteGeom{s.N, s.C, s.H, s.W, s.Co, s.KH, s.KW, s.SH, s.SW, s.PH, s.PW, s.OH, s.OW, g1s_mode};
}

struct PendingRed {
  Tensor slab;
  float* out;
  long n;
  int splits;
};
std::vector<PendingRed> g_pending;
bool g_defer = false;
size_t g_pending_bytes = 0;
void launch_pending();
size_t reduce_flush_bytes() {
  static const size_t v = [] {
    const char* e = std::getenv("DCNN_REDUCE_FLUSH_MB");
    return (size_t)((e ? std::atof(e) : 96.0) * (1 << 20));
  }();
  return v;
}

float* wgrad_slab(Slot slot, size_t bytes, Tensor& hold) {
  if (!g_defer) return static_cast<float*>(scratch(slot, bytes));
  int dev = 0;
  HOST_HIP_CHECK(hipGetDevice(&dev));
  hold = Tensor::empty({(int64_t)((bytes + 3) / 4)}, DType::F32, Device::gpu(dev));
  return hold.ptr<float>();
}

void wgrad_reduce(const Tensor& hold, const Tensor& bhold, const float* slab, float* gw, long n, const float* bslab,
                  float* gb, long nb, int splits) {
  if (g_defer) {
    g_pending.push_back({hold, gw, n, splits});
    if (gb) g_pending.push_back({bhold, gb, nb, splits});
    g_pending_bytes += (size_t)n * splits * 4 + (gb ? (size_t)nb * splits * 4 : 0);
    if (reduce_flush_bytes() && g_pending_bytes >= reduce_flush_bytes()) launch_pending();
    return;
  }
  if (gb)
    splitk_reduce2(slab, gw, n, bslab, gb, nb, splits, 1, cur());
  else
    splitk_reduce(slab, gw, n, splits, 1, cur());
}

template <class Launch>
void wgrad_split(int splits, long n, long nb, float* gw, float* gb, Launch&& launch) {
  Tensor hold, bhold;
  float* slab = wgrad_slab(SLAB, (size_t)splits * n * 4, hold);
  float* bslab = gb ? wgrad_slab(BSLAB, (size_t)splits * nb * 4, bhold) : nullptr;
  launch(slab, bslab);
  wgrad_reduce(hold, bhold, slab, gw, n, bslab, gb, nb, splits);
}
}

void begin_deferred_reduce() { g_defer = true; }
void set_fault(int f) { g_fault = f; }
void flush_deferred_reduce() {
  const bool on = g_defer;
  end_deferred_reduce();
  g_defer = on;
}
void end_deferred_reduce() {
  launch_pending();
  g_defer = false;
}

namespace {
void launch_pending() {
  for (size_t b = 0; b < g_pending.size(); b += kMaxRed) {
    MultiRed t{};
    t.count = (int)std::min(g_pending.size() - b, (size_t)kMaxRed);
    for (int k = 0; k < t.count; ++k) {
      const PendingRed& e = g_pending[b + k];
      t.e[k].slab = e.slab.ptr<float>();
      t.e[k].out = e.out;
      t.e[k].n = e.n;
      t.e[k].splits = e.splits;
    }
    multi_splitk_reduce(t, cur());
  }
  g_pending.clear();
  g_pending_bytes = 0;
}
}

void input_to_nhwc(const float* x, void* y, int N, int C, int HW) { nchw_to_nhwc(kBF16, x, y, N, C, HW, cur()); }
void nhwc_to_nchw(const void* x, void* y, int N, int HW, int C) { transpose16(x, y, N, HW, C); }
void nchw_to_nhwc_bf16(const void* x, void* y, int N, int HW, int C) { transpose16(x, y, N, C, HW); }
void cast_bf16(const float* x, void* y, long n) { cast_f32_bf16(x, static_cast<bf16*>(y), n, cur()); }
void zero(void* p, long nbytes) { zero_bytes(p, nbytes, cur()); }

const float* conv_fwd(const void* x, const void* w, const float* bias, void* y, const ConvShape& s, int* stat_rows) {
  const long xb = (long)s.N * s.H * s.W * s.C * 2, wb = (long)s.Co * s.KH * s.KW * s.C * 2;
  const bool want = stat_rows != nullptr;
  if (want) *stat_rows = 0;
  auto slab_of = [&](int rows) {
    *stat_rows = rows;
    return static_cast<float*>(scratch(fwd_stats_slot(), (size_t)rows * 3 * s.Co * 4));
  };
  const int M = s.N * s.OH * s.OW;
  const ConvRouteGeom g = route_geom(s, want ? 1 : 0);
  const int route = conv_fwd_route(g);
  rec("fwd", s, route, {{"bias", bias != nullptr}, {"stats", want}});
  if (route == ROUTE_HALO && xb < (1l << 31)) {
    HConvArgs a = hconv_fwd_args(x, w, y, bias, g);
    if (want) a.stats = slab_of(hconv_stat_rows(s.N, s.H, s.W, s.C, s.Co, a.ntaps, 0));
    hconv_workspace(a);
    hconv(a, cur());
    return a.stats;
  }
  if (route == ROUTE_G1S) {
    float* st = want ? slab_of(g1s_rows(M, s.Co, s.C, 1)) : nullptr;
    g1s(static_cast<const bf16*>(x), static_cast<const bf16*>(w), static_cast<bf16*>(y), M, s.Co, s.C, s.H, s.W, s.OH,
        s.OW, s.SH, bias, nullptr, st, 0, nullptr, 0, BnbArgs{}, want ? 1 : 0, cur());
    return st;
  }
  if (route != ROUTE_GENERIC && xb < (1l << 31) && wb < (1l << 31)) {
    G2Args a = g2_fwd_args(x, w, y, bias, g);
    if (want) a.stats = slab_of(gemm_g2_stat_rows(M, s.Co));
    gemm_g2(a, cur());
    return a.stats;
  }
  const int K = s.KH * s.KW * s.C;
  float* st = want ? slab_of(gemm_nt_stat_rows(M, s.Co)) : nullptr;
  NtArgs a{static_cast<const bf16*>(x), static_cast<const bf16*>(w), y, M, s.Co, K, 0, K, s.Co,
           kConvFwd, s.N, s.H, s.W, s.C, s.OH, s.OW, s.KH, s.KW, s.SH, s.SW, s.PH, s.PW, bias, nullptr, st, 0, 0};
  gemm_nt(a, cur());
  return st;
}

void weight_transpose(const void* w, void* wt, int Co, int T, int C) {
  conv_weight_transpose(kBF16, w, static_cast<bf16*>(wt), Co, T, C, cur());
}
void multi_weight_transpose(const int64_t* table, int n, long max_tiles) {
  dcnn::multi_weight_transpose(table, n, max_tiles, cur());
}

namespace {
bool g2_phases_ok(const ConvShape& s, const DgradPhases& p) {
  const std::vector<DgradPhase>& cls = p.phases;
  if (cls.empty() || cls.size() > 4 || p.taps.size() > 64) return false;
  for (const DgradPhase& c : cls)
    if (c.GH != cls[0].GH || c.GW != cls[0].GW) return false;
  const long rows = (long)s.N * cls[0].GH * cls[0].GW;
  return cls.size() == 1 || rows % 128 == 0;
}
bool g2_bytes_ok(const ConvShape& s) {
  const long dyb = (long)s.N * s.OH * s.OW * s.Co * 2, wtb = (long)s.C * s.KH * s.KW * s.Co * 2;
  return dyb < (1l << 31) && wtb < (1l << 31);
}
}

bool compact_shortcut_grad_enabled() {
  static const bool on = [] {
    const char* v = std::getenv("DCNN_COMPACT_SHORTCUT_GRAD");
    return !(v && std::string(v) == "0");
  }();
  return on;
}

bool conv_dgrad_takes_compact(const ConvShape& s) {
  if ((s.SH < 2 && s.SW < 2) || s.H % s.SH || s.W % s.SW || s.C % 8 || s.Co % 8) return false;
  const ConvRouteGeom g = route_geom(s, 0);
  const int route = conv_dgrad_route(g);
  if (route == ROUTE_HALO || route == ROUTE_G1S || route == ROUTE_GENERIC || !g2_bytes_ok(s)) return false;
  const DgradPhases p = conv_dgrad_phases(g);
  if (p.phases.size() < 2 || !g2_phases_ok(s, p)) return false;
  for (const DgradPhase& c : p.phases)
    if (c.ry == 0 && c.rx == 0) return c.nt > 0 && c.GH == s.H / s.SH && c.GW == s.W / s.SW;
  return false;
}

void conv_dgrad_compact(const void* dy, const void* w, void* dxc, const ConvShape& s, bool w_transposed) {
  if (s.KH != 1 || s.KW != 1 || s.PH != 0 || s.PW != 0 || (s.SH < 2 && s.SW < 2) || s.H % s.SH || s.W % s.SW ||
      s.OH != s.H / s.SH || s.OW != s.W / s.SW)
    throw std::invalid_argument("conv_dgrad_compact: a 1x1 pad-0 conv of stride > 1 on a map its stride divides");
  const ConvShape c{s.N, s.C, s.OH, s.OW, s.Co, 1, 1, 1, 1, 0, 0, s.OH, s.OW};
  DgradOpts opt;
  opt.dense_g2 = true;
  conv_dgrad(dy, w, dxc, c, nullptr, w_transposed, nullptr, nullptr, opt);
}

const float* conv_dgrad(const void* dy, const void* w, void* dx, const ConvShape& s, const void* residual,
                        bool w_transposed, const BnbOperands* bnb, int* bnb_rows, DgradOpts opt) {
  const int T = s.KH * s.KW, K = T * s.Co;
  if (opt.residual_compact && (residual == nullptr || !conv_dgrad_takes_compact(s)))
    throw std::invalid_argument("conv_dgrad: a phase-compact residual is taken by the grouped gemm_g2 route only");
  if (opt.dense_g2 && (T != 1 || s.SH != 1 || s.SW != 1 || s.PH != 0 || s.PW != 0 || bnb != nullptr ||
                       s.C % 8 || s.Co % 8 || !g2_bytes_ok(s)))
    throw std::invalid_argument("conv_dgrad: dense_g2 is a plain 1x1 stride-1 data gradient on gemm_g2");
  if (bnb_rows) *bnb_rows = 0;
  BnbArgs ba{};
  if (bnb) {
    ba.y = (g_fault & 1) ? nullptr : static_cast<const bf16*>(bnb->y);
    ba.x = static_cast<const bf16*>(bnb->x);
    ba.mean = bnb->mean;
    ba.istd = bnb->istd;
    static const bool mask_x_env = [] {
      const char* v = std::getenv("DCNN_BNB_MASK_X");
      return !(v && v[0] == '0');
    }();
    if (bnb->mask_from_x && bnb->y && mask_x_env && !(g_fault & 1)) {
      ba.mask_x = 1;
      ba.gamma = bnb->gamma;
      ba.beta = bnb->beta;
    }
  }
  auto slab_of = [&](int rows) {
    *bnb_rows = rows;
    return static_cast<float*>(scratch(BWD_STATS, (size_t)rows * 2 * s.C * 4));
  };
  const bf16* wt = static_cast<const bf16*>(w);
  if (!w_transposed) {
    bf16* t = static_cast<bf16*>(scratch(W_T, (size_t)s.Co * T * s.C * 2));
    conv_weight_transpose(kBF16, w, t, s.Co, T, s.C, cur());
    wt = t;
  }
  const long dyb = (long)s.N * s.OH * s.OW * s.Co * 2, wtb = (long)s.C * T * s.Co * 2;
  const ConvRouteGeom g = route_geom(s, bnb ? 2 : 0);
  const int route = opt.dense_g2 ? (int)ROUTE_GEMM_G2 : conv_dgrad_route(g);
  rec("dgrad", s, route, {{"residual", residual != nullptr}, {"w_t", w_transposed}, {"bnb", bnb != nullptr},
                         {"bnb_mask", bnb != nullptr && bnb->y != nullptr},
                         {"residual_compact", opt.residual_compact}});
  if (route == ROUTE_HALO && dyb < (1l << 31)) {
    HConvArgs a = hconv_dgrad_args(dy, wt, dx, residual, g);
    if (bnb) {
      a.bnb = ba;
      a.stats = slab_of(hconv_stat_rows(s.N, s.OH, s.OW, s.Co, s.C, T, 0));
    }
    hconv_workspace(a);
    hconv(a, cur());
    return a.stats;
  }
  if (route == ROUTE_G1S) {
    const int M = s.N * s.H * s.W;
    float* st = bnb ? slab_of(g1s_rows(M, s.C, s.Co, 2)) : nullptr;
// ... 586 lines not shown
```

### dcnn_amd/csrc/host/train.cpp

```cpp
#include "dcnn/train.hpp"

#include <algorithm>
#include <atomic>
#include <chrono>
#include <cmath>
#include <cstdio>
#include <cstring>
#include <filesystem>
#include <fstream>
#include <sstream>
#include <stdexcept>
#include <thread>

namespace dcnn_native {
bool decode_jpeg(const unsigned char* data, size_t n, std::vector<unsigned char>& rgb, int& w, int& h,
                 std::string* err);
}

namespace dcnn {

LossResult Loss::compute(const Tensor& pred, const Tensor* labels_in, const Tensor* target_in, float grad_scale) const {
  if (pred.rank() != 2) throw std::runtime_error("loss: expected [N, C] predictions");
  const int N = (int)pred.dim(0), C = (int)pred.dim(1);
  const Device dev = pred.device();
  Tensor labels, target;
  if (labels_in) labels = labels_in->device() == dev ? *labels_in : labels_in->to(dev);
  if (target_in) {
    if (target_in->numel() != (int64_t)N * C) throw std::runtime_error("loss: target must be [N, C]");
    target = target_in->device() == dev ? *target_in : target_in->to(dev);
  }
  if (!labels.defined() && !target.defined()) throw std::runtime_error("loss: labels or a target are required");
  const int64_t* lp = labels.defined() ? labels.ptr<int64_t>() : nullptr;
  const float* tp = target.defined() ? target.ptr<float>() : nullptr;
  LossResult r;
  if (dev.is_gpu()) {
    r.grad = Tensor::empty({N, C}, DType::BF16, dev, Layout::NHWC);
    r.loss = gpu_ops::loss(kind_, pred.data(), tp, lp, r.grad.data(), N, C, param_, &r.correct, grad_scale);
  } else {
    r.grad = Tensor::empty({N, C}, DType::F32, dev);
    r.loss = cpu_ops::loss(kind_, pred.ptr<float>(), tp, lp, r.grad.ptr<float>(), N, C, param_, &r.correct);
    if (grad_scale != 1.f) {
      float* g = r.grad.ptr<float>();
      for (int64_t i = 0; i < (int64_t)N * C; ++i) g[i] *= grad_scale;
    }
  }
  return r;
}

void TrainGraph::capture(const Tensor& x, const Tensor& labels) {
  const Device dev = model_.device();
  sx_ = x.to(dev).clone();
  sy_ = labels.to(dev).clone();
  std::vector<Param*> params = model_.parameters();
  ParamArena* a = params.empty() ? nullptr : params[0]->arena.get();
  if (!a) throw std::runtime_error("TrainGraph: the model's parameters are not in a GPU arena");
  const Tensor v0 = a->value.clone(), m0 = a->m.clone(), w0 = a->v.clone(), s0 = a->shadow.clone();
  std::vector<std::pair<Tensor, Tensor>> bn0;
  opt_.prepare(params);
  if (a->ema.defined()) bn0.emplace_back(a->ema, a->ema.clone());
  for (BatchNorm* bn : model_.batchnorms())
    for (Tensor* t : {&bn->running_mean, &bn->running_var})
      if (t->defined()) bn0.emplace_back(*t, t->clone());
  {
    std::vector<Layer*> all;
    for (auto& l : model_.layers()) l->collect_layers(all);
    for (Layer* l : all)
      if (auto* dp = dynamic_cast<DropPath*>(l))
        if (dp->draw_counter().defined()) bn0.emplace_back(dp->draw_counter(), dp->draw_counter().clone());
  }
  const long t0 = opt_.step_count();
  auto eager = [&] {
    model_.zero_grad();
    LossResult r = loss_(model_.forward(sx_), sy_);
    model_.backward(r.grad);
    if (grad_hook_) grad_hook_();
    opt_.step(params);
  };
  for (int i = 0; i < 2; ++i) eager();
  gpu::copy(a->value.data(), v0.data(), v0.nbytes(), 2);
  gpu::copy(a->m.data(), m0.data(), m0.nbytes(), 2);
  gpu::copy(a->v.data(), w0.data(), w0.nbytes(), 2);
  gpu::copy(a->shadow.data(), s0.data(), s0.nbytes(), 2);
  for (auto& [live, snap] : bn0) gpu::copy(live.data(), snap.data(), snap.nbytes(), 2);
  a->refresh_transposes();
  opt_.set_step_count(t0);
  opt_.upload_hyper();
  gpu::flow_synchronize();
  graph_.begin();
  try {
    eager();
  } catch (...) {
    graph_.end();
    throw;
  }
  graph_.end();
  opt_.set_step_count(t0);
  opt_.upload_hyper();
  captured_ = true;
}

double TrainGraph::step(const Tensor& x, const Tensor& labels) {
  const Device dev = model_.device();
  if (!dev.is_gpu()) {
    model_.zero_grad();
    LossResult r = loss_(model_.forward(x), labels);
    model_.backward(r.grad);
    if (grad_hook_) grad_hook_();
    opt_.step(model_.parameters());
    return r.loss;
  }
  if (!captured_) capture(x, labels);
  if (x.numel() != sx_.numel() || labels.numel() != sy_.numel() || labels.dtype() != sy_.dtype())
    throw std::runtime_error("TrainGraph: the batch shape changed after capture (the target slot is " +
                             std::string(dtype_name(sy_.dtype())) + " with " + std::to_string(sy_.numel()) +
                             " elements, got " + dtype_name(labels.dtype()) + " with " +
                             std::to_string(labels.numel()) + ")");
  if (x.device() == dev && labels.device() == dev) {
    gpu::copy2_d2d(sx_.data(), x.data(), sx_.nbytes(), sy_.data(), labels.data(), sy_.nbytes());
  } else {
    if (x.device() == dev) gpu::copy(sx_.data(), x.data(), sx_.nbytes(), 2);
    else gpu::copy(sx_.data(), x.to(dev).data(), sx_.nbytes(), 2);
    if (labels.device() == dev) gpu::copy(sy_.data(), labels.data(), sy_.nbytes(), 2);
    else gpu::copy(sy_.data(), labels.to(dev).data(), sy_.nbytes(), 2);
  }
  opt_.before_replay();
  graph_.replay();
  return std::nan("");
}

double TrainGraph::last_loss() {
  if (!model_.device().is_gpu() || !captured_) return std::nan("");
  float l = 0.f;
  gpu::copy(&l, gpu_ops::loss_device(), sizeof l, 1);
  return l;
}

Loss LossFactory::create(const std::string& name, float param) {
  std::string n = name;
  std::transform(n.begin(), n.end(), n.begin(), ::tolower);
  if (n == "ce" || n == "crossentropy" || n == "cross_entropy")
    return Loss(0, param >= 0 ? param : 1e-15f, "crossentropy");
  if (n == "softmax_ce" || n == "softmax_crossentropy" || n == "softmax_cross_entropy")
    return Loss(1, param >= 0 ? param : 1e-15f, "softmax_crossentropy");
  if (n == "logsoftmax_ce" || n == "logsoftmax_crossentropy" || n == "log_softmax_crossentropy")
    return Loss(2, param >= 0 ? param : 1e-15f, "logsoftmax_crossentropy");
  if (n == "mse") return Loss(3, 0.f, "mse");
  if (n == "mae") return Loss(4, 0.f, "mae");
  if (n == "huber") return Loss(5, param >= 0 ? param : 1.0f, "huber");
  if (n == "soft_crossentropy" || n == "soft_ce" || n == "label_smoothing_ce") {
    const float eps = param >= 0 ? param : 0.f;
    if (!(eps < 1.f)) throw std::invalid_argument("label_smoothing must be in [0, 1), got " + std::to_string(eps));
    return Loss(6, eps, "soft_crossentropy");
  }
  throw std::invalid_argument("unknown loss '" + name + "'");
}

BatchMixer::BatchMixer(int num_classes, double mixup_alpha, double cutmix_alpha, double prob, double switch_prob,
                       uint64_t seed)
    : k_(num_classes), ma_(mixup_alpha), ca_(cutmix_alpha), prob_(prob), sw_(switch_prob), seed_(seed) {
  if (k_ < 1) throw std::invalid_argument("BatchMixer: num_classes " + std::to_string(k_) + " < 1");
  plan(1, 1, 1);
}

MixPlan BatchMixer::plan(uint64_t step, int H, int W) const {
  return cpu_ops::mix_plan(seed_, step, H, W, ma_, ca_, prob_, sw_);
}

void BatchMixer::mix(Tensor& x, const Tensor& labels_in, Tensor& target) {
  if (x.rank() != 4 || x.dtype() != DType::F32) throw std::invalid_argument("BatchMixer: x is fp32 [B, C, H, W]");
  if (labels_in.dtype() != DType::I64 || labels_in.numel() != x.dim(0))
    throw std::invalid_argument("BatchMixer: labels are int64 [B]");
  const Device dev = x.device();
  const long B = x.dim(0), C = x.dim(1), H = x.dim(2), W = x.dim(3);
  const Tensor labels = labels_in.device() == dev ? labels_in : labels_in.to(dev);
  const MixPlan p = plan(++state_, (int)H, (int)W);
  target = Tensor::empty({B, (int64_t)k_}, DType::F32, dev);
  if (dev.is_gpu())
    gpu_ops::mix_batch(x.ptr<float>(), labels.ptr<int64_t>(), target.ptr<float>(), B, C, H, W, p.mode, p.lam, p.yl,
                       p.yh, p.xl, p.xh, k_);
  else
    cpu_ops::mix_batch(x.ptr<float>(), labels.ptr<int64_t>(), target.ptr<float>(), B, C, H, W, p.mode, p.lam, p.yl,
                       p.yh, p.xl, p.xh, k_);
}

namespace {
constexpr double kPi = 3.14159265358979323846;
}

json::Value Scheduler::get_config() const {
  json::Value c = json::Value::object();
  c["type"] = type();
  c["name"] = type();
  c["parameters"] = parameters_config();
  return c;
}

void StepLR::step() {
  ++step_;
  if (step_ % size_ == 0) set_lr(get_lr() * gamma_);
}
json::Value StepLR::parameters_config() const {
  json::Value p = json::Value::object();
  p["step_size"] = size_;
  p["gamma"] = gamma_;
  return p;
}

MultiStepLR::MultiStepLR(Optimizer* o, std::vector<int> milestones, double gamma)
    : Scheduler(o), ms_(std::move(milestones)), gamma_(gamma) {
  std::sort(ms_.begin(), ms_.end());
}
void MultiStepLR::step() {
  ++step_;
  if (idx_ < ms_.size() && step_ >= ms_[idx_]) {
    set_lr(get_lr() * gamma_);
    ++idx_;
  }
}
void MultiStepLR::reset() {
  Scheduler::reset();
  idx_ = 0;
}
json::Value MultiStepLR::parameters_config() const {
  json::Value p = json::Value::object();
// ... 571 lines not shown
```

### dcnn_amd/csrc/kernels/api.h

```cpp
#pragma once
#include <hip/hip_runtime.h>
#include <stdint.h>

#include "fusion_plan.h"
#include "optim_segments.h"
typedef __bf16 bf16;

namespace dcnn {
struct BnbArgs {
  const bf16* y; const bf16* x; const float* mean; const float* istd;
  const float* gamma; const float* beta; int mask_x;
};
struct NtArgs {
  const bf16* A; const bf16* B; void* C;
  int M, N, K; int lda, ldb, ldc; int mode;
  int nb, sh, sw, cs, gh, gw; int kh, kw, strh, strw, padh, padw;
  const float* bias; const bf16* residual; float* stats; int out_f32; int relu;
};
struct TnArgs {
  const bf16* dY; const bf16* X; float* slab; float* bias_slab;
  int M, N, P; int mode; int nb, sh, sw, cs, gh, gw; int kh, kw, strh, strw, padh, padw; int ldx; int k_per_split;
};
struct G2Args {
  const bf16* A; const bf16* B; bf16* C;
  unsigned a_bytes, b_bytes;
  int M, N, Cs, H, W, GH, GW, SY, SX, ntaps;
  int tap_dy[64], tap_dx[64], tap_srcoff[64], tap_b[64];
  int ldb, ldc;
  int OH, OW, OSY, OSX, ORY, ORX;
  const float* bias; const bf16* residual; float* stats; int relu;
  float* zero_ptr; int zero_n;
  BnbArgs bnb;
  int ncls, cls_rows;
  int cls_t0[4], cls_nt[4], cls_ory[4], cls_orx[4];
  int ksplit; float* kpart;
  unsigned fd_ghw[3], fd_gw[3];
  int res_cls = -1;
};
struct T2Args {
  const bf16* dY; const bf16* X; float* slab; float* bias_slab;
  unsigned a_bytes, b_bytes;
  int M, N, P, ldy, Cs, H, W, GH, GW, SY, SX, ntaps;
  int tap_dy[64], tap_dx[64];
  int k_per_split;
};
struct PoolGeom { int N, H, W, C, OH, OW, ph, pw, sh, sw, padh, padw; };
struct ConvGeom { int N, H, W, C, OH, OW, KH, KW, SH, SW, PH, PW; };
struct DwArgs { int N, H, W, C, OH, OW, KH, KW, SH, SW, PH, PW; };
bool dwconv_supported(int dt, DwArgs g);
void dwconv_fwd(int dt, const void* x, const void* w, const float* bias, void* y, DwArgs g, hipStream_t s);
void dwconv_dgrad(int dt, const void* dy, const void* w, const void* residual, void* dx, DwArgs g, hipStream_t s);
int dwconv_wgrad_splits(int dt, DwArgs g);
void dwconv_wgrad(int dt, const void* dy, const void* x, float* slab, float* bias_slab, DwArgs g, hipStream_t s);
struct GcArgs { int N, H, W, Ci, Co, G, OH, OW, KH, KW, SH, SW, PH, PW; };
bool gconv_supported(int dt, GcArgs g);
void gconv_fwd(int dt, const void* x, const void* w, const float* bias, void* y, GcArgs g, hipStream_t s);
void gconv_weight_t(int dt, const void* w, void* wt, GcArgs g, hipStream_t s);
void gconv_dgrad(int dt, const void* dy, const void* wt, const void* residual, void* dx, GcArgs g, hipStream_t s);
int gconv_wgrad_splits(int dt, GcArgs g);
void gconv_wgrad(int dt, const void* dy, const void* x, float* slab, float* bias_slab, GcArgs g, hipStream_t s);
struct HConvArgs {
  const bf16* A; const bf16* B; bf16* C;
  unsigned a_bytes, b_bytes;
  int NB, H, W, Cs, N, ldb, ntaps;
  int tap_dy[9], tap_dx[9], tap_b[9];
  int TH, TW, IMG, HPR;
  const float* bias; const bf16* residual; float* stats; int relu;
  float* zero_ptr; int zero_n;
  BnbArgs bnb;
  float* Cf; const float* residual_f;
  int splits; float* part; unsigned* tickets;
};
void hconv(HConvArgs a, hipStream_t s);
int hconv_splits(int NB, int H, int W, int Cs, int N, int ntaps);
int hconv_tiles(int NB, int H, int W, int Cs, int N, int ntaps);
int hconv_tile_elems(int NB, int H, int W, int Cs, int N, int ntaps);
int hconv_split_target();
void gemm_t2_set_split_target(int t);
void hwgrad_set_split_target(int t);
void hconv3_set_max_splits(int n);
void g1s_set_waves_per_simd(int w);
void hconv_set_split_target(int t);
void hconv_set_split_min_work(int w);
void bn_set_vectorised(int on);
bool hconv_supported(int NB, int H, int W, int Cs, int N, int ntaps);
int hconv_stat_rows(int NB, int H, int W, int Cs, int N, int ntaps, int f32out);
bool hconv3_f32_try(const HConvArgs& a, hipStream_t s);
int hconv3_f32_splits(int NB, int H, int W, int Cs, int N, int ntaps);
bool hconv_v3(int NB, int H, int W, int Cs, int N, int ntaps);
void hconv3_enable(int on);
void hconv3_set_grid_cap(int n);
void hconv3_set_stamps(uintptr_t p);
struct HWArgs {
  const bf16* dY; const bf16* X; float* slab; float* bias_slab;
  unsigned dy_bytes, x_bytes;
  int NB, H, W, Cs, Co, ntaps;
  int tap_dy[9], tap_dx[9];
  int TH, TW, IMG, HPR, tiles_per_split;
  int ldy, ldx, npairs;
  int pair_yoff[3], pair_xoff[3], pair_bias[3];
};
void hwgrad(HWArgs a, int splits, hipStream_t s);
bool hwgrad_supported(int NB, int H, int W, int Cs, int Co, int ntaps);
int hwgrad_splits(int NB, int H, int W, int Cs, int Co);
bool hwgrad_f32_supported(int NB, int H, int W, int Cs, int Co);
int hwgrad_f32_splits(int NB, int H, int W, int Cs, int Co);
void hwgrad_f32(HWArgs a, int splits, hipStream_t s);
void hwgrad_set_version(int v);
bool hwgrad_s2_supported(int NB, int H, int W, int Cs, int Co);
int hwgrad_s2_splits(int NB, int H, int W, int Cs, int Co);
void hwgrad_s2(HWArgs a, int splits, hipStream_t s);

void gemm_nt(const NtArgs& a, hipStream_t s);
void gemm_g2(const G2Args& a, hipStream_t s);
void gemm_g2_set_splitk(int on);
int gemm_g2_splitk_enabled();
int gemm_g2_stat_rows(int M, int N);
int gemm_g2_row_tile(int M, int N);
void gemm_t2(T2Args a, int splits, hipStream_t s);
int g1s_rows(int M, int N, int K, int mode);
void g1s_enable(int on);
void g1s(const bf16* X, const bf16* Wt, bf16* Y, int M, int N, int K, int H, int W, int OH, int OW, int S,
         const float* bias, const bf16* residual, float* stats, int relu, float* zero_ptr, int zero_n, BnbArgs bnb,
         int mode, hipStream_t s);
int g1s_gen_rows(int M, int N, int Kc, int ntaps, int mode);
void g1s_gen(const bf16* X, const bf16* Wt, bf16* Y, int NB, int GH, int GW, int N, int Kc, int ldw,
             const std::vector<std::array<int, 3>>& taps, int H, int W, int OHo, int OWo, int OS, int ORY, int ORX,
             const bf16* residual, float* stats, float* zero_ptr, int zero_n, BnbArgs bnb, int mode, hipStream_t s);
int gemm_t2_splits(int M, int N, int P);
int gemm_nt_stat_rows(int M, int N);
void elementwise(int mode, int op, const float* a, const float* b, float* c, long n, float s0, float s1, hipStream_t s);
void reduce(int op, const float* a, const float* b, long n, float* workspace, float* out, hipStream_t s);
void fill_random(float* out, long n, uint64_t seed, float a, float b, int normal, hipStream_t s);
void transpose_batched(const float* in, float* out, int batch, int rows, int cols, hipStream_t s);
void transpose_batched16(const void* in, void* out, int batch, int rows, int cols, hipStream_t s);
void rows_copy(int kind, const void* src, int lds, void* dst, int ldd, long rows, int cols, hipStream_t s);
void nchw_cnhw(const float* in, float* out, int N, int C, int HW, int to_cnhw, hipStream_t s);
void pad_crop(const float* in, float* out, int NC, int H, int W, int OH, int OW, int top, int left, float value,
              hipStream_t s);
void gemm_g2f(const G2Args& a, hipStream_t s);
int gemm_g2f_stat_rows(int M, int N);
void gemm_t2f(T2Args a, int splits, hipStream_t s);
int gemm_t2f_splits(int M, int N, int P);
void set_f32_mode(int mode);
int get_f32_mode();
void conv_weight_transpose_f32(const float* w, float* wt, int Co, int T_, int Ci, hipStream_t s);
void gemm_tn(TnArgs a, int splits, hipStream_t s);
int gemm_tn_splits(int M, int N, int P);
int gemm_tn_k_per_split(int P, int splits);
int gemm_tn_bias_rows(int M);
struct ConvRouteGeom {
  int N, C, H, W, Co, KH, KW, SH, SW, PH, PW, OH, OW, g1s_mode;
};
enum ConvRoute : int { ROUTE_GENERIC = 0, ROUTE_GEMM_G2 = 1, ROUTE_HALO = 2, ROUTE_G1S = 3, ROUTE_HALO_S2 = 4 };
int conv_fwd_route(ConvRouteGeom g);
int conv_dgrad_route(ConvRouteGeom g);
int conv_wgrad_route(ConvRouteGeom g);
void splitk_reduce(const float* slab, float* out, long n, int splits, int accumulate, hipStream_t s);
void splitk_reduce2(const float* slab, float* out, long n, const float* bslab, float* bout, long nb, int splits,
                    int accumulate, hipStream_t s);

constexpr int kMaxRed = 48;
struct RedEnt { const float* slab; float* out; long n; int splits, unit0, chunks, groups, vec, wpc; };
struct MultiRed { int count; RedEnt e[kMaxRed]; };
void multi_splitk_reduce(MultiRed t, hipStream_t s);

int bn_partial_rows(long R, int C);
void bn_partial(int dtype, const void* x, const void* dy, const void* yout, void* dy_out, const float* mean,
                const float* istd, long R, int C, float* slab, int mode, float* zero_sums, hipStream_t s);
int bn_stat_parts(int rows);
void bn_stat_reduce2(int mode, const float* slab, int rows, float* out, float* part, const float* slab2, int rows2,
                     float* out2, float* part2, int C, hipStream_t s);
void bn_stat_reduce(int mode, const float* slab, int rows, int C, float* out, float* part, unsigned* ticket,
                    hipStream_t s);
void bn_apply(int dtype, const void* x, void* y, long R, int C, const float* sums, int parts, float count, const float* gamma,
              const float* beta, float eps, const void* residual, int relu, float* save_mean, float* save_istd,
              float* run_mean, float* run_var, float momentum, int use_running, hipStream_t s);
struct BnSide {
  const void* x; const float* sums; int parts; float count; const float* gamma; const float* beta; float eps;
  float* save_mean; float* save_istd; float* run_mean; float* run_var; float momentum; int use_running;
};
bool bn_apply_dual(const BnSide& a, const BnSide& b, void* y, long R, int C, int relu, hipStream_t s);
bool bn_apply_dual_supported(long R, int C);
struct BnBwdSide {
  const void* x; void* dx; const float* mean; const float* istd; const float* gamma; const float* sums; int parts;
  float count; float* dgamma; float* dbeta;
};
bool bn_bwd_apply_dual(const void* dy, const BnBwdSide& a, const BnBwdSide& b, long R, int C, hipStream_t s);
void bn_bwd_apply(int dtype, const void* dy, const void* yout, const void* x, void* dx, long R, int C, const float* mean,
                  const float* istd, const float* gamma, const float* sums, int parts, float count, float* dgamma,
                  float* dbeta, int eval_mode, hipStream_t s);
bool bn_relu_maxpool_supported(PoolGeom g);
void bn_relu_maxpool(const bf16* x, bf16* y, uint8_t* idx, PoolGeom g, const float* sums, int parts, float count,
                     const float* gamma, const float* beta, float eps, float* save_mean, float* save_istd,
                     float* run_mean, float* run_var, float momentum, hipStream_t s);
void gn_fwd(int dtype, const void* x, void* y, int N, int HW, int C, int G, const float* gamma, const float* beta,
            float eps, float* save_mean, float* save_istd, hipStream_t s);
void gn_bwd(int dtype, const void* dy, const void* x, void* dx, int N, int HW, int C, int G, const float* gamma,
            const float* mean, const float* istd, float* dgamma, float* dbeta, float* aff, hipStream_t s);
bool ln_supported(int dt, long R, int C);
int ln_partial_rows(long R, int C);
long ln_workspace_bytes(long R, int C);
void ln_fwd(int dt, const void* x, void* y, long R, int C, const float* gamma, const float* beta, float eps,
            float* save_mean, float* save_rstd, hipStream_t s);
void ln_bwd(int dt, const void* dy, const void* x, void* dx, long R, int C, const float* gamma, const float* mean,
            const float* rstd, float* dgamma, float* dbeta, float* workspace, hipStream_t s);
void lscale_fwd(int dt, const void* x, const float* gamma, const void* residual, void* y, long R, int C,
                hipStream_t s);
void lscale_bwd(int dt, const void* dy, const void* x, const float* gamma, void* dx, float* dgamma, long R, int C,
                float* workspace, hipStream_t s);
void lscale_drop_fwd(int dt, const void* x, const float* gamma, const float* mask, const void* residual, void* y,
                     long R, int C, long rows_per_sample, hipStream_t s);
void lscale_drop_bwd(int dt, const void* dy, const void* x, const float* gamma, const float* mask, void* dx,
                     float* dgamma, long R, int C, long rows_per_sample, float* workspace, hipStream_t s);
float drop_path_keep_scale(float p);
void drop_path_mask(float* mask, int N, float p, uint64_t seed, uint64_t draw, const uint64_t* ctr, hipStream_t s);
void drop_path_scale(int dt, const void* x, const float* mask, const void* residual, void* y, long N, long row,
                     hipStream_t s);

void maxpool_fwd(int dt, const void* x, void* y, uint8_t* idx, PoolGeom g, hipStream_t s);
void maxpool_bwd(int dt, const void* dy, const uint8_t* idx, void* dx, PoolGeom g, hipStream_t s);
bool maxpool_bwd_bnb_supported(PoolGeom g);
int maxpool_bwd_bnb_rows(PoolGeom g);
void maxpool_bwd_bnb(const bf16* dy, const uint8_t* idx, const bf16* ypool, const bf16* x, const float* mean,
                     const float* istd, bf16* dx, PoolGeom g, float* slab, float* zero_sums, hipStream_t s);
void avgpool_fwd(int dt, const void* x, void* y, PoolGeom g, hipStream_t s);
void avgpool_bwd(int dt, const void* dy, void* dx, PoolGeom g, hipStream_t s);
bool head_supported(PoolGeom g, int Out);
void head_fwd(const bf16* x, const bf16* w, const float* bias, bf16* pooled, bf16* logits, PoolGeom g, int Out,
              hipStream_t s);
int head_bwd_splits(int N, int In, int Out);
void head_bwd(const bf16* dlogits, const bf16* w, const bf16* pooled, bf16* dx, float* slab, float* bias_slab,
              PoolGeom g, int Out, hipStream_t s);
void act_fwd(int dt, const void* x, void* y, long n, int type, float a, hipStream_t s);
void act_bwd(int dt, const void* x, const void* dy, void* dx, long n, int type, float a, hipStream_t s);
void softmax_rows(int dt, const void* x, void* y, long rows, int C, hipStream_t s);
void softmax_rows_bwd(int dt, const void* y, const void* dy, void* dx, long rows, int C, hipStream_t s);
void dropout(int dt, const void* x, void* y, long n, float p, uint64_t seed, const uint64_t* ctr, hipStream_t s);
void counter_bump(uint64_t* ctr, uint64_t* slot, hipStream_t s);
void nchw_to_nhwc(int dt, const float* x, void* y, int N, int C, int HW, hipStream_t s);
void nchw_to_nhwc_pad(int dt, const float* x, void* y, int N, int C, int Cp, int HW, hipStream_t s);
void conv_weight_transpose(int src_dt, const void* w, bf16* wt, int Co, int T_, int Ci, hipStream_t s);
void cast_f32_bf16(const float* x, bf16* y, long n, hipStream_t s);
struct StemArgs {
  const float* x; const void* w; int w_bf16; long ws[4];
  const float* bias; bf16* y; float* slab; float* zero_ptr; int zero_n;
  const bf16* dy; float* bias_slab; long gs[4]; long n_slab;
  int halo_bytes; int N, Ci, H, W, Co, TH;
  const bf16* bn_x; const float* bn_mean; const float* bn_istd; const float* bn_gamma; const float* bn_sums;
  int bn_parts; float bn_count; float* bn_dgamma; float* bn_dbeta; int bn_eval;
};
bool stem_supported(int N, int Ci, int H, int W, int Co);
int stem_tiles_host(int N, int H, int W);
int stem_wgrad_blocks(int N, int H, int W);
int stem_wgrad_blocks_bnt(int N, int H, int W);
void stem_fwd(StemArgs a, hipStream_t s);
void stem_wgrad(StemArgs a, int blocks, hipStream_t s);
void multi_weight_transpose(const int64_t* table, int n, long max_tiles, hipStream_t s, int f32 = 0);
void im2col(const float* x, float* col, int N, int C, int H, int W, int KH, int KW, int SH, int SW, int PH, int PW,
            int OH, int OW, hipStream_t s);
void col2im(const float* col, float* x, int N, int C, int H, int W, int KH, int KW, int SH, int SW, int PH, int PW,
            int OH, int OW, hipStream_t s);
void mix_batch(float* x, const int64_t* labels, float* target, int B, int C, int H, int W, int mode, float lam, int yl,
               int yh, int xl, int xh, int K, hipStream_t s);
int loss_workspace_floats(int N);
void loss_fused(int dt, const void* pred, const float* target, const int64_t* labels, void* grad, float* loss_out,
                int* correct, int N, int C, int type, float param, float gscale, float* ws, unsigned* ticket,
                hipStream_t s);
void adam_step(float* p, const float* g, float* m, float* v, bf16* shadow, long n, float lr, float b1, float b2,
               float eps, float bc1, float bc2, float wd, int decoupled, const float* hyper, hipStream_t s);
void adam_step_nodecay(float* p, const float* g, float* m, float* v, bf16* shadow, long n, float lr, float b1, float b2,
                       float eps, float bc1, float bc2, float wd, int decoupled, const float* hyper,
                       const uint8_t* nodecay, hipStream_t s);
void sgd_step(float* p, const float* g, float* vel, bf16* shadow, long n, float lr, float mom, const float* hyper,
              hipStream_t s);
void adam_scalars(float* hyper, float b1, float b2, hipStream_t s);
int grad_sumsq_blocks(long n);
void grad_sumsq(const float* g, long n, float max_norm, float* part, unsigned* ticket, float* out, hipStream_t s);
void adam_step_tail(float* p, const float* g, float* m, float* v, bf16* shadow, long n, float lr, float b1, float b2,
                    float eps, float bc1, float bc2, float wd, int decoupled, const float* hyper,
                    const uint8_t* nodecay, const float* coef, float* ema, float decay, hipStream_t s);
void sgd_step_tail(float* p, const float* g, float* vel, bf16* shadow, long n, float lr, float mom, const float* hyper,
                   const float* coef, float* ema, float decay, hipStream_t s);
void ema_swap(float* a, float* b, bf16* shadow, long n, hipStream_t s);
struct LayerwiseTables {
  const SegChunk* chunks;
  int nchunks;
  const SegInfo* segs;
  int nsegs;
  long cover;
  float* part;
  unsigned* ticket;
  float* out;
};
void lamb_step(float* p, const float* g, float* m, float* v, bf16* shadow, long n, float lr, double b1, double b2,
               float eps, float bc1, float bc2, float wd, const float* hyper, const float* coef, float* ema,
               float decay, const LayerwiseTables& t, hipStream_t s);
void lamb_scalars(float* hyper, double b1, double b2, hipStream_t s);
void lars_step(float* p, const float* g, float* vel, bf16* shadow, long n, float lr, float mom, float wd, float tc,
               float eps, const float* hyper, const float* coef, float* ema, float decay, const LayerwiseTables& t,
               hipStream_t s);
void grad_pack_bf16(const float* g, bf16* out, long n, float scale, hipStream_t s);
void grad_sum_chunks_bf16(const bf16* src, int w, long ld, long n, bf16* dst, hipStream_t s);
void grad_unpack_bf16(const bf16* in, float* g, long n, hipStream_t s);
void zero_bytes(void* p, long nbytes, hipStream_t s);
void copy_pair(void* d0, const void* s0, long n0, void* d1, const void* s1, long n1, hipStream_t s);
void split3_bf16(const float* in, bf16* out, long rows, int C, int pattern, hipStream_t s);
void im2col_nhwc(int dt, const void* x, void* col, const ConvGeom& g, hipStream_t s);
void col2im_nhwc(int dt, const void* col, void* x, const void* residual, const ConvGeom& g, int chan_major,
                 hipStream_t s);
enum { AUG_HFLIP = 0, AUG_VFLIP, AUG_ROTATION, AUG_BRIGHTNESS, AUG_CONTRAST, AUG_NOISE, AUG_CROP, AUG_CUTOUT,
       AUG_NORMALIZE };
constexpr int kAugMaxOps = 12;
constexpr int kAugMaxFloats = 16384;
struct AugOpDev {
  int kind;
  float p;
  float a[6];
};
struct AugBatchArgs {
  const void* src;
  int src_u8;
  const int64_t* idx;
  const int64_t* labels;
  int64_t* labels_out;
  float* out;
  int B, C, H, W;
  unsigned long long seed;
  int nops;
  AugOpDev ops[kAugMaxOps];
};
bool augment_batch_supported(int C, int H, int W);
void augment_batch(const AugBatchArgs& a, hipStream_t s);
}

#include "conv_args.h"
```

### dcnn_amd/csrc/kernels/bindings.cpp

```cpp
#include <tuple>
#include <pybind11/pybind11.h>
#include <pybind11/stl.h>
#include <algorithm>
#include <array>
#include <vector>
#include <hip/hip_runtime.h>
#include <stdint.h>

namespace py = pybind11;
#include "api.h"


using namespace dcnn;
void bind_runtime(py::module_& m);
void bind_rccl(py::module_& m);
template <typename T>
static inline T P(uintptr_t x) { return reinterpret_cast<T>(x); }
static inline hipStream_t S(uintptr_t x) { return reinterpret_cast<hipStream_t>(x); }

using Ptr4 = std::array<uintptr_t, 4>;
static BnbArgs bnb_of(const Ptr4& b) {
  return BnbArgs{P<const bf16*>(b[0]), P<const bf16*>(b[1]), P<const float*>(b[2]), P<const float*>(b[3])};
}

// ... 462 lines not shown
                                  uintptr_t run_mean, uintptr_t run_var, float momentum, uintptr_t st) {
    bn_relu_maxpool(P<const bf16*>(x), P<bf16*>(y), P<uint8_t*>(idx), geom(N, H, W, C, OH, OW, ph, pw, sh, sw, padh, padw),
                    P<const float*>(sums), parts, count, P<const float*>(gamma), P<const float*>(beta), eps,
                    P<float*>(save_mean), P<float*>(save_istd), P<float*>(run_mean), P<float*>(run_var), momentum,
                    S(st));
  });
  m.def("maxpool_bwd_bnb_rows", [geom](int N, int H, int W, int C, int OH, int OW, int ph, int pw, int sh, int sw,
                                       int padh, int padw) {
    return maxpool_bwd_bnb_rows(geom(N, H, W, C, OH, OW, ph, pw, sh, sw, padh, padw));
  });
  m.def("maxpool_bwd_bnb", [geom](uintptr_t dy, uintptr_t idx, uintptr_t ypool, uintptr_t x, uintptr_t mean,
                                  uintptr_t istd, uintptr_t dx, int N, int H, int W, int C, int OH, int OW, int ph,
                                  int pw, int sh, int sw, int padh, int padw, uintptr_t slab, uintptr_t zero_sums,
                                  uintptr_t st) {
    maxpool_bwd_bnb(P<const bf16*>(dy), P<const uint8_t*>(idx), P<const bf16*>(ypool), P<const bf16*>(x),
                    P<const float*>(mean), P<const float*>(istd), P<bf16*>(dx),
                    geom(N, H, W, C, OH, OW, ph, pw, sh, sw, padh, padw), P<float*>(slab), P<float*>(zero_sums), S(st));
  });
  m.def("avgpool_fwd", [geom](int dt, uintptr_t x, uintptr_t y, int N, int H, int W, int C, int OH, int OW, int ph,
                              int pw, int sh, int sw, int padh, int padw, uintptr_t st) {
    avgpool_fwd(dt, P<const void*>(x), P<void*>(y), geom(N, H, W, C, OH, OW, ph, pw, sh, sw, padh, padw), S(st));
  });
  m.def("avgpool_bwd", [geom](int dt, uintptr_t dy, uintptr_t dx, int N, int H, int W, int C, int OH, int OW, int ph,
                              int pw, int sh, int sw, int padh, int padw, uintptr_t st) {
    avgpool_bwd(dt, P<const void*>(dy), P<void*>(dx), geom(N, H, W, C, OH, OW, ph, pw, sh, sw, padh, padw), S(st));
  });
  m.def("head_supported", [geom](int N, int H, int W, int C, int OH, int OW, int ph, int pw, int sh, int sw, int padh,
                                 int padw, int Out) {
    return head_supported(geom(N, H, W, C, OH, OW, ph, pw, sh, sw, padh, padw), Out);
  });
  m.def("head_fwd", [geom](uintptr_t x, uintptr_t w, uintptr_t bias, uintptr_t pooled, uintptr_t logits, int N, int H,
                           int W, int C, int OH, int OW, int ph, int pw, int sh, int sw, int padh, int padw, int Out,
                           uintptr_t st) {
    head_fwd(P<const bf16*>(x), P<const bf16*>(w), P<const float*>(bias), P<bf16*>(pooled), P<bf16*>(logits),
             geom(N, H, W, C, OH, OW, ph, pw, sh, sw, padh, padw), Out, S(st));
  });
  m.def("head_bwd_splits", &head_bwd_splits);
  m.def("head_bwd", [geom](uintptr_t dlogits, uintptr_t w, uintptr_t pooled, uintptr_t dx, uintptr_t slab,
                           uintptr_t bias_slab, int N, int H, int W, int C, int OH, int OW, int ph, int pw, int sh,
                           int sw, int padh, int padw, int Out, uintptr_t st) {
    head_bwd(P<const bf16*>(dlogits), P<const bf16*>(w), P<const bf16*>(pooled), P<bf16*>(dx), P<float*>(slab),
             P<float*>(bias_slab), geom(N, H, W, C, OH, OW, ph, pw, sh, sw, padh, padw), Out, S(st));
  });
  m.def("act_fwd", [](int dt, uintptr_t x, uintptr_t y, long n, int type, float a, uintptr_t st) {
    act_fwd(dt, P<const void*>(x), P<void*>(y), n, type, a, S(st));
  });
  m.def("act_bwd", [](int dt, uintptr_t x, uintptr_t dy, uintptr_t dx, long n, int type, float a, uintptr_t st) {
    act_bwd(dt, P<const void*>(x), P<const void*>(dy), P<void*>(dx), n, type, a, S(st));
  });
  m.def("softmax_rows", [](int dt, uintptr_t x, uintptr_t y, long rows, int C, uintptr_t st) {
    softmax_rows(dt, P<const void*>(x), P<void*>(y), rows, C, S(st));
  });
  m.def("softmax_rows_bwd", [](int dt, uintptr_t y, uintptr_t dy, uintptr_t dx, long rows, int C, uintptr_t st) {
    softmax_rows_bwd(dt, P<const void*>(y), P<const void*>(dy), P<void*>(dx), rows, C, S(st));
  });
  m.def("dropout", [](int dt, uintptr_t x, uintptr_t y, long n, float p, uint64_t seed, uintptr_t ctr, uintptr_t st) {
    dropout(dt, P<const void*>(x), P<void*>(y), n, p, seed, P<const uint64_t*>(ctr), S(st));
  });
  m.def("counter_bump", [](uintptr_t ctr, uintptr_t slot, uintptr_t st) {
    counter_bump(P<uint64_t*>(ctr), P<uint64_t*>(slot), S(st));
  });
  m.def("nchw_to_nhwc", [](int dt, uintptr_t x, uintptr_t y, int N, int C, int HW, uintptr_t st) {
    nchw_to_nhwc(dt, P<const float*>(x), P<void*>(y), N, C, HW, S(st));
  });
  m.def("nchw_to_nhwc_pad", [](int dt, uintptr_t x, uintptr_t y, int N, int C, int Cp, int HW, uintptr_t st) {
    nchw_to_nhwc_pad(dt, P<const float*>(x), P<void*>(y), N, C, Cp, HW, S(st));
  });
  m.def("conv_weight_transpose", [](int dt, uintptr_t w, uintptr_t wt, int Co, int T_, int Ci, uintptr_t st) {
    conv_weight_transpose(dt, P<const void*>(w), P<bf16*>(wt), Co, T_, Ci, S(st));
  });
  m.def("multi_splitk_reduce", [](std::vector<std::array<int64_t, 4>> ents, uintptr_t st) {
    for (size_t b = 0; b < ents.size(); b += kMaxRed) {
      MultiRed t{};
      t.count = (int)std::min(ents.size() - b, (size_t)kMaxRed);
      for (int k = 0; k < t.count; ++k) {
        const auto& e = ents[b + k];
        t.e[k].slab = P<const float*>((uintptr_t)e[0]); t.e[k].out = P<float*>((uintptr_t)e[1]);
        t.e[k].n = e[2]; t.e[k].splits = (int)e[3];
      }
      multi_splitk_reduce(t, S(st));
    }
  });
  m.def("multi_red_max", []() { return kMaxRed; });
  m.def("stem_supported", &stem_supported);
  m.def("stem_tiles", &stem_tiles_host);
  m.def("stem_wgrad_blocks", &stem_wgrad_blocks);
  m.def("stem_fwd", [](uintptr_t x, uintptr_t w, int w_bf16, std::array<long, 4> ws, uintptr_t bias, uintptr_t y,
                       uintptr_t slab, uintptr_t zero_ptr, int zero_n, int N, int Ci, int H, int W, int Co,
                       uintptr_t st) {
    StemArgs a{};
    a.x = P<const float*>(x); a.w = P<const void*>(w); a.w_bf16 = w_bf16;
    for (int i = 0; i < 4; ++i) a.ws[i] = ws[i];
    a.bias = P<const float*>(bias); a.y = P<bf16*>(y); a.slab = P<float*>(slab);
    a.zero_ptr = P<float*>(zero_ptr); a.zero_n = zero_n;
    a.N = N; a.Ci = Ci; a.H = H; a.W = W; a.Co = Co;
    stem_fwd(a, S(st));
  });
  m.def("stem_wgrad", [](uintptr_t x, uintptr_t dy, uintptr_t slab, uintptr_t bias_slab, std::array<long, 4> gs,
                         int N, int Ci, int H, int W, int Co, int blocks, uintptr_t st) {
    StemArgs a{};
    a.x = P<const float*>(x); a.dy = P<const bf16*>(dy); a.slab = P<float*>(slab);
    a.bias_slab = P<float*>(bias_slab);
    for (int i = 0; i < 4; ++i) a.gs[i] = gs[i];
    a.n_slab = (long)Co * Ci * 9;
    a.N = N; a.Ci = Ci; a.H = H; a.W = W; a.Co = Co;
    stem_wgrad(a, blocks, S(st));
  });
  m.def("multi_weight_transpose", [](uintptr_t table, int n, long max_tiles, uintptr_t st, int f32) {
    multi_weight_transpose(P<const int64_t*>(table), n, max_tiles, S(st), f32);
  });
  m.def("cast_f32_bf16",[](uintptr_t x, uintptr_t y, long n, uintptr_t st) {
    cast_f32_bf16(P<const float*>(x), P<bf16*>(y), n, S(st));
  });
  m.def("im2col_nhwc", [](int dt, uintptr_t x, uintptr_t col, int N, int H, int W, int C, int OH, int OW, int KH, int KW,
                          int SH, int SW, int PH, int PW, uintptr_t st) {
    im2col_nhwc(dt, P<const void*>(x), P<void*>(col), ConvGeom{N, H, W, C, OH, OW, KH, KW, SH, SW, PH, PW}, S(st));
  });
  m.def("col2im_nhwc", [](int dt, uintptr_t col, uintptr_t x, uintptr_t residual, int N, int H, int W, int C, int OH,
                          int OW, int KH, int KW, int SH, int SW, int PH, int PW, int chan_major, uintptr_t st) {
    col2im_nhwc(dt, P<const void*>(col), P<void*>(x), P<const void*>(residual),
                ConvGeom{N, H, W, C, OH, OW, KH, KW, SH, SW, PH, PW}, chan_major, S(st));
  });
  m.def("im2col", [](uintptr_t x, uintptr_t col, int N, int C, int H, int W, int KH, int KW, int SH, int SW, int PH,
                     int PW, int OH, int OW, uintptr_t st) {
    im2col(P<const float*>(x), P<float*>(col), N, C, H, W, KH, KW, SH, SW, PH, PW, OH, OW, S(st));
  });
  m.def("col2im", [](uintptr_t col, uintptr_t x, int N, int C, int H, int W, int KH, int KW, int SH, int SW, int PH,
                     int PW, int OH, int OW, uintptr_t st) {
    col2im(P<const float*>(col), P<float*>(x), N, C, H, W, KH, KW, SH, SW, PH, PW, OH, OW, S(st));
  });
  m.def("loss_workspace_floats", &loss_workspace_floats);
  m.def("loss_fused", [](int dt, uintptr_t pred, uintptr_t target, uintptr_t labels, uintptr_t grad, uintptr_t loss,
                         uintptr_t correct, int N, int C, int type, float param, float gscale, uintptr_t ws,
                         uintptr_t ticket, uintptr_t st) {
    loss_fused(dt, P<const void*>(pred), P<const float*>(target), P<const int64_t*>(labels), P<void*>(grad),
               P<float*>(loss), P<int*>(correct), N, C, type, param, gscale, P<float*>(ws), P<unsigned*>(ticket),
               S(st));
  });
  m.def("adam_step", [](uintptr_t p, uintptr_t g, uintptr_t mm, uintptr_t v, uintptr_t shadow, long n, float lr,
                        float b1, float b2, float eps, float bc1, float bc2, float wd, int dec, uintptr_t hyper,
                        uintptr_t st) {
    adam_step(P<float*>(p), P<const float*>(g), P<float*>(mm), P<float*>(v), P<bf16*>(shadow), n, lr, b1, b2, eps, bc1,
              bc2, wd, dec, P<const float*>(hyper), S(st));
  });
  m.def("adam_step_nodecay", [](uintptr_t p, uintptr_t g, uintptr_t mm, uintptr_t v, uintptr_t shadow, long n, float lr,
                                float b1, float b2, float eps, float bc1, float bc2, float wd, int dec,
                                uintptr_t hyper, uintptr_t nodecay, uintptr_t st) {
    adam_step_nodecay(P<float*>(p), P<const float*>(g), P<float*>(mm), P<float*>(v), P<bf16*>(shadow), n, lr, b1, b2,
                      eps, bc1, bc2, wd, dec, P<const float*>(hyper), P<const uint8_t*>(nodecay), S(st));
  });
  m.def("adam_scalars", [](uintptr_t hyper, float b1, float b2, uintptr_t st) {
    adam_scalars(P<float*>(hyper), b1, b2, S(st));
  });
  m.def("sgd_step", [](uintptr_t p, uintptr_t g, uintptr_t vel, uintptr_t shadow, long n, float lr, float mom,
                       uintptr_t hyper, uintptr_t st) {
    sgd_step(P<float*>(p), P<const float*>(g), P<float*>(vel), P<bf16*>(shadow), n, lr, mom, P<const float*>(hyper),
             S(st));
  });
  m.def("grad_sumsq_blocks", &grad_sumsq_blocks);
  m.def("grad_sumsq", [](uintptr_t g, long n, float max_norm, uintptr_t part, uintptr_t ticket, uintptr_t out,
                         uintptr_t st) {
    grad_sumsq(P<const float*>(g), n, max_norm, P<float*>(part), P<unsigned*>(ticket), P<float*>(out), S(st));
  });
  m.def("adam_step_tail", [](uintptr_t p, uintptr_t g, uintptr_t mm, uintptr_t v, uintptr_t shadow, long n, float lr,
                             float b1, float b2, float eps, float bc1, float bc2, float wd, int dec, uintptr_t hyper,
                             uintptr_t nodecay, uintptr_t coef, uintptr_t ema, float decay, uintptr_t st) {
    adam_step_tail(P<float*>(p), P<const float*>(g), P<float*>(mm), P<float*>(v), P<bf16*>(shadow), n, lr, b1, b2, eps,
                   bc1, bc2, wd, dec, P<const float*>(hyper), P<const uint8_t*>(nodecay), P<const float*>(coef),
                   P<float*>(ema), decay, S(st));
  });
  m.def("sgd_step_tail", [](uintptr_t p, uintptr_t g, uintptr_t vel, uintptr_t shadow, long n, float lr, float mom,
                            uintptr_t hyper, uintptr_t coef, uintptr_t ema, float decay, uintptr_t st) {
    sgd_step_tail(P<float*>(p), P<const float*>(g), P<float*>(vel), P<bf16*>(shadow), n, lr, mom,
                  P<const float*>(hyper), P<const float*>(coef), P<float*>(ema), decay, S(st));
  });
  m.def("ema_swap", [](uintptr_t a, uintptr_t b, uintptr_t shadow, long n, uintptr_t st) {
    ema_swap(P<float*>(a), P<float*>(b), P<bf16*>(shadow), n, S(st));
  });
  m.def("optim_segments", [](const std::vector<long>& offsets, const std::vector<long>& counts,
                             const std::vector<int>& no_decay, bool exclude, long n) {
    if (offsets.size() != counts.size() || (!no_decay.empty() && no_decay.size() != counts.size()))
      throw std::invalid_argument("optim_segments: offsets, counts and no_decay have one entry per parameter");
    std::vector<unsigned char> nd(no_decay.begin(), no_decay.end());
    const OptimSegments t = build_optim_segments(offsets.data(), counts.data(), nd.empty() ? nullptr : nd.data(),
                                                 (int)counts.size(), exclude, n);
    std::vector<int> c, s;
    for (const SegChunk& k : t.chunks) c.insert(c.end(), {k.first_block, k.blocks, k.segment});
    for (const SegInfo& g : t.segs) s.insert(s.end(), {g.first_chunk, g.chunks, g.adapt, g.decay});
    return py::make_tuple(c, s, t.cover);
  });
  m.def("optim_segments_check", [](const std::vector<int>& chunks, const std::vector<int>& segs, long n) {
    static_assert(sizeof(SegChunk) == 3 * sizeof(int) && sizeof(SegInfo) == 4 * sizeof(int), "flat int32 rows");
    if (chunks.size() % 3 || segs.size() % 4)
      throw std::invalid_argument("optim_segments_check: chunk rows have 3 and segment rows 4 entries");
    check_optim_segments(reinterpret_cast<const SegChunk*>(chunks.data()), (int)(chunks.size() / 3),
                         reinterpret_cast<const SegInfo*>(segs.data()), (int)(segs.size() / 4), n);
  });
  m.def("lamb_scalars", [](uintptr_t hyper, double b1, double b2, uintptr_t st) {
    lamb_scalars(P<float*>(hyper), b1, b2, S(st));
  });
  m.def("lamb_step", [](uintptr_t p, uintptr_t g, uintptr_t mm, uintptr_t v, uintptr_t shadow, long n, float lr,
                        double b1, double b2, float eps, float bc1, float bc2, float wd, uintptr_t hyper, uintptr_t coef,
                        uintptr_t ema, float decay, uintptr_t chunks, int nchunks, uintptr_t segs, int nsegs,
                        long cover, uintptr_t part, uintptr_t ticket, uintptr_t out, uintptr_t st) {
    const LayerwiseTables t{P<const SegChunk*>(chunks), nchunks, P<const SegInfo*>(segs), nsegs, cover,
                            P<float*>(part), P<unsigned*>(ticket), P<float*>(out)};
    lamb_step(P<float*>(p), P<const float*>(g), P<float*>(mm), P<float*>(v), P<bf16*>(shadow), n, lr, b1, b2, eps, bc1,
              bc2, wd, P<const float*>(hyper), P<const float*>(coef), P<float*>(ema), decay, t, S(st));
  });
  m.def("lars_step", [](uintptr_t p, uintptr_t g, uintptr_t vel, uintptr_t shadow, long n, float lr, float mom, float wd,
                        float tc, float eps, uintptr_t hyper, uintptr_t coef, uintptr_t ema, float decay,
                        uintptr_t chunks, int nchunks, uintptr_t segs, int nsegs, long cover, uintptr_t part,
                        uintptr_t ticket, uintptr_t out, uintptr_t st) {
    const LayerwiseTables t{P<const SegChunk*>(chunks), nchunks, P<const SegInfo*>(segs), nsegs, cover,
                            P<float*>(part), P<unsigned*>(ticket), P<float*>(out)};
    lars_step(P<float*>(p), P<const float*>(g), P<float*>(vel), P<bf16*>(shadow), n, lr, mom, wd, tc, eps,
              P<const float*>(hyper), P<const float*>(coef), P<float*>(ema), decay, t, S(st));
  });
  m.def("zero_bytes", [](uintptr_t p, long nbytes, uintptr_t st) { zero_bytes(P<void*>(p), nbytes, S(st)); });
  m.def("grad_pack_bf16", [](uintptr_t g, uintptr_t out, long n, float scale, uintptr_t st) {
    grad_pack_bf16(P<const float*>(g), P<bf16*>(out), n, scale, S(st));
  });
  m.def("grad_sum_chunks_bf16", [](uintptr_t src, int w, long ld, long n, uintptr_t dst, uintptr_t st) {
    grad_sum_chunks_bf16(P<const bf16*>(src), w, ld, n, P<bf16*>(dst), S(st));
  });
  m.def("grad_unpack_bf16", [](uintptr_t in, uintptr_t g, long n, uintptr_t st) {
    grad_unpack_bf16(P<const bf16*>(in), P<float*>(g), n, S(st));
  });
  m.def("mix_batch", [](uintptr_t x, uintptr_t labels, uintptr_t target, long B, long C, long H, long W, int mode,
                        double lam, int yl, int yh, int xl, int xh, long K, uintptr_t st) {
    if (B < 1 || C < 1 || H < 1 || W < 1 || (double)B * C * H * W > 2147483647.0)
      throw std::invalid_argument("mix_batch: " + std::to_string((double)B * C * H * W) +
                                  " elements: the batch is empty or exceeds 2^31 - 1");
    if (K < 1 || (double)B * K > 2147483647.0)
      throw std::invalid_argument("mix_batch: num_classes " + std::to_string(K) + " < 1 or the target exceeds 2^31 - 1");
    mix_batch(P<float*>(x), P<const int64_t*>(labels), P<float*>(target), (int)B, (int)C, (int)H, (int)W, mode,
              (float)lam, yl, yh, xl, xh, (int)K, S(st));
  });
  m.def("augment_batch_supported", &augment_batch_supported);
  m.def("augment_batch", [](uintptr_t src, int src_u8, uintptr_t idx, uintptr_t labels, uintptr_t labels_out,
                            uintptr_t out, int B, int C, int H, int W, unsigned long long seed,
                            const std::vector<std::tuple<int, float, std::vector<float>>>& ops, uintptr_t st) {
    AugBatchArgs a{};
    a.src = P<const void*>(src); a.src_u8 = src_u8; a.idx = P<const int64_t*>(idx);
    a.labels = P<const int64_t*>(labels); a.labels_out = P<int64_t*>(labels_out); a.out = P<float*>(out);
    a.B = B; a.C = C; a.H = H; a.W = W; a.seed = seed;
    if (ops.size() > (size_t)kAugMaxOps) throw std::runtime_error("augment_batch: at most 12 ops");
    a.nops = (int)ops.size();
    for (size_t k = 0; k < ops.size(); ++k) {
      a.ops[k].kind = std::get<0>(ops[k]);
      a.ops[k].p = std::get<1>(ops[k]);
      const auto& v = std::get<2>(ops[k]);
      if (v.size() > 6) throw std::runtime_error("augment_batch: at most 6 op parameters");
      for (size_t j = 0; j < v.size(); ++j) a.ops[k].a[j] = v[j];
    }
    augment_batch(a, S(st));
  });
  m.attr("AUG_KINDS") = py::make_tuple("horizontal_flip", "vertical_flip", "rotation", "brightness", "contrast",
                                       "gaussian_noise", "random_crop", "cutout", "normalize");
}
```

### dcnn_amd/csrc/kernels/loss_optim.hip

```cpp
#include "common.h"
#include "api.h"

namespace dcnn {

enum LossType { kCE = 0, kSoftmaxCE = 1, kLogSoftmaxCE = 2, kMSE = 3, kMAE = 4, kHuber = 5, kSoftCE = 6 };

template <typename T>
__device__ __forceinline__ void loss_row(const T* __restrict__ pred, const float* __restrict__ target,
                                         const int64_t* __restrict__ labels, T* __restrict__ grad, int row, int N,
                                         int C, int type, float param, float gscale, int lane, float* lsum_out,
                                         int* hit) {
  const T* p = pred + (long)row * C;
  auto tgt = [&](int c) -> float {
    if (labels) return (int64_t)c == labels[row] ? 1.f : 0.f;
    return target[(long)row * C + c];
  };
  float pm = -INFINITY, tm = -INFINITY;
  int pi = 0x7fffffff, ti = 0x7fffffff;
  for (int c = lane; c < C; c += 64) {
    const float v = to_f(p[c]), t = tgt(c);
    if (v > pm) { pm = v; pi = c; }
    if (t > tm) { tm = t; ti = c; }
  }
#pragma unroll
// ... 124 lines not shown
  __syncthreads();
  for (int o = 128; o > 0; o >>= 1) {
    if (threadIdx.x < o) { sl[threadIdx.x] += sl[threadIdx.x + o]; sc[threadIdx.x] += sc[threadIdx.x + o]; }
    __syncthreads();
  }
  if (threadIdx.x == 0) {
    *loss_out = sl[0];
    if (correct) *correct = sc[0];
    *ticket = 0u;
  }
}

int loss_workspace_floats(int N) { return 2 * N; }

void loss_fused(int dt, const void* pred, const float* target, const int64_t* labels, void* grad, float* loss_out,
                int* correct, int N, int C, int type, float param, float gscale, float* ws, unsigned* ticket,
                hipStream_t s) {
  const int blocks = (N + 3) / 4;
  if (blocks > 1 && (!ws || !ticket)) throw std::runtime_error("loss_fused: workspace required");
  if (type < 0 || type > kSoftCE) throw std::invalid_argument("loss_fused: unknown loss kind " + std::to_string(type));
  if (type == kSoftCE && !(param >= 0.f && param < 1.f))
    throw std::invalid_argument("loss_fused: label_smoothing " + std::to_string(param) + " is not in [0, 1)");
  if (dt == 0)
    hipLaunchKernelGGL(loss_kernel<float>, dim3(blocks), dim3(256), 0, s, (const float*)pred, target, labels,
                       (float*)grad, loss_out, correct, N, C, type, param, gscale, ws, ticket);
  else
    hipLaunchKernelGGL(loss_kernel<bf16>, dim3(blocks), dim3(256), 0, s, (const bf16*)pred, target, labels,
                       (bf16*)grad, loss_out, correct, N, C, type, param, gscale, ws, ticket);
  DCNN_LAUNCH_CHECK();
}

__device__ __forceinline__ float adam1(float& p, float g, float& m, float& v, float lr, float b1, float b2, float eps,
                                       float bc1, float bc2, float wd, int decoupled) {
  m = b1 * m + (1.f - b1) * g;
  v = b2 * v + (1.f - b2) * g * g;
  float upd = lr * (m / bc1) / (sqrtf(v / bc2) + eps);
  if (wd > 0.f) {
    if (decoupled) p -= wd * lr * p;
    else upd += wd * lr * p;
  }
  p -= upd;
  return p;
}

__global__ void adam_kernel(float* __restrict__ p, const float* __restrict__ g, float* __restrict__ m,
                            float* __restrict__ v, bf16* __restrict__ shadow, long n, float lr, float b1, float b2,
                            float eps, float bc1, float bc2, float wd, int decoupled,
                            const float* __restrict__ hyper) {
  if (hyper) { lr = hyper[0]; bc1 = hyper[1]; bc2 = hyper[2]; }
  const long n4 = n / 4;
  for (long i = blockIdx.x * (long)blockDim.x + threadIdx.x; i < n4; i += (long)gridDim.x * blockDim.x) {
    float4 pp = reinterpret_cast<float4*>(p)[i], gg = reinterpret_cast<const float4*>(g)[i];
    float4 mm = reinterpret_cast<float4*>(m)[i], vv = reinterpret_cast<float4*>(v)[i];
    adam1(pp.x, gg.x, mm.x, vv.x, lr, b1, b2, eps, bc1, bc2, wd, decoupled);
    adam1(pp.y, gg.y, mm.y, vv.y, lr, b1, b2, eps, bc1, bc2, wd, decoupled);
    adam1(pp.z, gg.z, mm.z, vv.z, lr, b1, b2, eps, bc1, bc2, wd, decoupled);
    adam1(pp.w, gg.w, mm.w, vv.w, lr, b1, b2, eps, bc1, bc2, wd, decoupled);
    reinterpret_cast<float4*>(p)[i] = pp;
    reinterpret_cast<float4*>(m)[i] = mm;
    reinterpret_cast<float4*>(v)[i] = vv;
    if (shadow) {
      bf16x4 b = {(bf16)pp.x, (bf16)pp.y, (bf16)pp.z, (bf16)pp.w};
      reinterpret_cast<bf16x4*>(shadow)[i] = b;
    }
  }
  for (long i = n4 * 4 + blockIdx.x * (long)blockDim.x + threadIdx.x; i < n; i += (long)gridDim.x * blockDim.x) {
    float pp = p[i], mm = m[i], vv = v[i];
    adam1(pp, g[i], mm, vv, lr, b1, b2, eps, bc1, bc2, wd, decoupled);
    p[i] = pp; m[i] = mm; v[i] = vv;
    if (shadow) shadow[i] = (bf16)pp;
  }
}

__global__ void adam_nodecay_kernel(float* __restrict__ p, const float* __restrict__ g, float* __restrict__ m,
                                    float* __restrict__ v, bf16* __restrict__ shadow, long n, float lr, float b1,
                                    float b2, float eps, float bc1, float bc2, float wd, int decoupled,
                                    const float* __restrict__ hyper, const uint8_t* __restrict__ nodecay) {
  if (hyper) { lr = hyper[0]; bc1 = hyper[1]; bc2 = hyper[2]; }
  const long n4 = n / 4;
  for (long i = blockIdx.x * (long)blockDim.x + threadIdx.x; i < n4; i += (long)gridDim.x * blockDim.x) {
    const float w = nodecay[i >> 4] ? 0.f : wd;
    float4 pp = reinterpret_cast<float4*>(p)[i], gg = reinterpret_cast<const float4*>(g)[i];
    float4 mm = reinterpret_cast<float4*>(m)[i], vv = reinterpret_cast<float4*>(v)[i];
    adam1(pp.x, gg.x, mm.x, vv.x, lr, b1, b2, eps, bc1, bc2, w, decoupled);
    adam1(pp.y, gg.y, mm.y, vv.y, lr, b1, b2, eps, bc1, bc2, w, decoupled);
    adam1(pp.z, gg.z, mm.z, vv.z, lr, b1, b2, eps, bc1, bc2, w, decoupled);
    adam1(pp.w, gg.w, mm.w, vv.w, lr, b1, b2, eps, bc1, bc2, w, decoupled);
    reinterpret_cast<float4*>(p)[i] = pp;
    reinterpret_cast<float4*>(m)[i] = mm;
    reinterpret_cast<float4*>(v)[i] = vv;
    if (shadow) {
      bf16x4 b = {(bf16)pp.x, (bf16)pp.y, (bf16)pp.z, (bf16)pp.w};
      reinterpret_cast<bf16x4*>(shadow)[i] = b;
    }
  }
  for (long i = n4 * 4 + blockIdx.x * (long)blockDim.x + threadIdx.x; i < n; i += (long)gridDim.x * blockDim.x) {
    float pp = p[i], mm = m[i], vv = v[i];
    adam1(pp, g[i], mm, vv, lr, b1, b2, eps, bc1, bc2, nodecay[i >> 6] ? 0.f : wd, decoupled);
    p[i] = pp; m[i] = mm; v[i] = vv;
    if (shadow) shadow[i] = (bf16)pp;
  }
}

__global__ void sgd_kernel(float* __restrict__ p, const float* __restrict__ g, float* __restrict__ vel,
                           bf16* __restrict__ shadow, long n, float lr, float mom, const float* __restrict__ hyper) {
  if (hyper) lr = hyper[0];
  for (long i = blockIdx.x * (long)blockDim.x + threadIdx.x; i < n; i += (long)gridDim.x * blockDim.x) {
    float pp = p[i];
    if (vel) {
      const float vv = mom * vel[i] - lr * g[i];
      vel[i] = vv;
      pp += vv;
    } else {
      pp -= lr * g[i];
    }
    p[i] = pp;
    if (shadow) shadow[i] = (bf16)pp;
  }
}

void adam_step(float* p, const float* g, float* m, float* v, bf16* shadow, long n, float lr, float b1, float b2,
               float eps, float bc1, float bc2, float wd, int decoupled, const float* hyper, hipStream_t s) {
  hipLaunchKernelGGL(adam_kernel, dim3(grid_for(n / 4 + 1, 256, 4096)), dim3(256), 0, s, p, g, m, v, shadow, n, lr, b1,
                     b2, eps, bc1, bc2, wd, decoupled, hyper);
  DCNN_LAUNCH_CHECK();
}

void adam_step_nodecay(float* p, const float* g, float* m, float* v, bf16* shadow, long n, float lr, float b1, float b2,
                       float eps, float bc1, float bc2, float wd, int decoupled, const float* hyper,
                       const uint8_t* nodecay, hipStream_t s) {
  if (!nodecay) throw std::invalid_argument("adam_step_nodecay: needs the block table ((n + 63) / 64 bytes)");
  hipLaunchKernelGGL(adam_nodecay_kernel, dim3(grid_for(n / 4 + 1, 256, 4096)), dim3(256), 0, s, p, g, m, v, shadow, n,
                     lr, b1, b2, eps, bc1, bc2, wd, decoupled, hyper, nodecay);
  DCNN_LAUNCH_CHECK();
}

__global__ void adam_scalars_kernel(float* hyper, float b1, float b2) {
  if (threadIdx.x == 0) {
    const float t = hyper[3] + 1.f;
    hyper[3] = t;
    hyper[1] = 1.f - powf(b1, t);
    hyper[2] = 1.f - powf(b2, t);
  }
}

void adam_scalars(float* hyper, float b1, float b2, hipStream_t s) {
  hipLaunchKernelGGL(adam_scalars_kernel, dim3(1), dim3(64), 0, s, hyper, b1, b2);
  DCNN_LAUNCH_CHECK();
}

void sgd_step(float* p, const float* g, float* vel, bf16* shadow, long n, float lr, float mom, const float* hyper,
              hipStream_t s) {
  hipLaunchKernelGGL(sgd_kernel, dim3(grid_for(n, 256, 4096)), dim3(256), 0, s, p, g, vel, shadow, n, lr, mom, hyper);
  DCNN_LAUNCH_CHECK();
}

constexpr int kSumsqLanes = 1024;

static int sumsq_per(long n) {
  const long per = (n / 4 + kSumsqLanes * 256L - 1) / (kSumsqLanes * 256L);
  return (int)(per < 1 ? 1 : per > 60 ? 60 : per);
}

int grad_sumsq_blocks(long n) {
  const long span = (long)kSumsqLanes * sumsq_per(n), blocks = (n / 4 + span - 1) / span;
  if (blocks > 0x7fffffffL) throw std::invalid_argument("grad_sumsq: n " + std::to_string(n) + " is too large");
  return (int)(blocks < 1 ? 1 : blocks);
}

__device__ __forceinline__ void clip_block(float* __restrict__ out, float sumsq, float max_norm) {
  const float norm = sqrtf(sumsq), c = max_norm / (norm + 1e-6f);
  out[0] = sumsq;
  out[1] = norm;
  out[2] = c < 1.f || c != c ? c : 1.f;
  out[3] = max_norm;
}

__global__ void __launch_bounds__(kSumsqLanes) grad_sumsq_kernel(const float* __restrict__ g, long n, int per,
                                                                 float max_norm, float* part,
                                                                 unsigned* __restrict__ ticket,
                                                                 float* __restrict__ out) {
  __shared__ float sw[16];
  __shared__ float sl[256];
  __shared__ int last;
  const int lane = threadIdx.x & 63, w = threadIdx.x >> 6;
  const long n4 = n / 4, base = (long)blockIdx.x * per * kSumsqLanes + threadIdx.x;
  float4 a = {0.f, 0.f, 0.f, 0.f};
  for (int k = 0; k < per; k += 4) {
    float4 x[4];
#pragma unroll
    for (int j = 0; j < 4; ++j) {
      const long i = base + (long)(k + j) * kSumsqLanes;
      x[j] = (k + j < per && i < n4) ? reinterpret_cast<const float4*>(g)[i] : float4{0.f, 0.f, 0.f, 0.f};
    }
#pragma unroll
    for (int j = 0; j < 4; ++j) {
      a.x = __fmaf_rn(x[j].x, x[j].x, a.x);
      a.y = __fmaf_rn(x[j].y, x[j].y, a.y);
      a.z = __fmaf_rn(x[j].z, x[j].z, a.z);
      a.w = __fmaf_rn(x[j].w, x[j].w, a.w);
    }
  }
  if (blockIdx.x == gridDim.x - 1) {
    const long i = n4 * 4 + threadIdx.x;
    if (i < n) a.x = __fmaf_rn(g[i], g[i], a.x);
  }
  const float s = wave_sum((a.x + a.y) + (a.z + a.w));
  if (lane == 0) sw[w] = s;
  __syncthreads();
  float blk = 0.f;
  if (threadIdx.x == 0) {
    float t[16];
#pragma unroll
    for (int i = 0; i < 16; ++i) t[i] = sw[i];
#pragma unroll
    for (int o = 8; o > 0; o >>= 1)
#pragma unroll
      for (int i = 0; i < o; ++i) t[i] = t[2 * i] + t[2 * i + 1];
    blk = t[0];
  }
  if (gridDim.x == 1) {
    if (threadIdx.x == 0) clip_block(out, blk, max_norm);
    return;
  }
  if (threadIdx.x == 0) {
    part[blockIdx.x] = blk;
    __builtin_amdgcn_fence(__ATOMIC_RELEASE, "agent");
    asm volatile("s_waitcnt vmcnt(0)" ::: "memory");
    const unsigned old = __hip_atomic_fetch_add(ticket, 1u, __ATOMIC_RELAXED, __HIP_MEMORY_SCOPE_AGENT);
    last = old == gridDim.x - 1;
    if (last) {
      __builtin_amdgcn_fence(__ATOMIC_ACQUIRE, "agent");
      asm volatile("s_waitcnt vmcnt(0)" ::: "memory");
    }
  }
  __syncthreads();
  if (!last) return;
  if (threadIdx.x < 256) {
    float l = 0.f;
    for (unsigned r = threadIdx.x; r < gridDim.x; r += 256) l += part[r];
    sl[threadIdx.x] = l;
  }
  __syncthreads();
  for (int o = 128; o > 0; o >>= 1) {
    if (threadIdx.x < o) sl[threadIdx.x] += sl[threadIdx.x + o];
    __syncthreads();
  }
  if (threadIdx.x == 0) {
    clip_block(out, sl[0], max_norm);
    *ticket = 0u;
  }
}

void grad_sumsq(const float* g, long n, float max_norm, float* part, unsigned* ticket, float* out, hipStream_t s) {
  if (n < 1) throw std::invalid_argument("grad_sumsq: n " + std::to_string(n) + " < 1");
  if (!g || !out || ((uintptr_t)g & 15)) throw std::invalid_argument("grad_sumsq: g (16-byte aligned) and out are required");
  const int blocks = grad_sumsq_blocks(n);
  if (blocks > 1 && (!part || !ticket)) throw std::runtime_error("grad_sumsq: workspace and ticket required");
  hipLaunchKernelGGL(grad_sumsq_kernel, dim3(blocks), dim3(kSumsqLanes), 0, s, g, n, sumsq_per(n), max_norm, part, ticket, out);
  DCNN_LAUNCH_CHECK();
}

__global__ void adam_tail_kernel(float* __restrict__ p, const float* __restrict__ g, float* __restrict__ m,
                                 float* __restrict__ v, bf16* __restrict__ shadow, long n, float lr, float b1, float b2,
                                 float eps, float bc1, float bc2, float wd, int decoupled,
                                 const float* __restrict__ hyper, const uint8_t* __restrict__ nodecay,
                                 const float* __restrict__ coef, float* __restrict__ ema, float decay) {
  if (hyper) { lr = hyper[0]; bc1 = hyper[1]; bc2 = hyper[2]; }
  const float c = coef ? *coef : 1.f, keep = 1.f - decay;
  const long n4 = n / 4;
  for (long i = blockIdx.x * (long)blockDim.x + threadIdx.x; i < n4; i += (long)gridDim.x * blockDim.x) {
    const float w = nodecay && nodecay[i >> 4] ? 0.f : wd;
    float4 pp = reinterpret_cast<float4*>(p)[i], gg = reinterpret_cast<const float4*>(g)[i];
    float4 mm = reinterpret_cast<float4*>(m)[i], vv = reinterpret_cast<float4*>(v)[i];
    if (coef) { gg.x *= c; gg.y *= c; gg.z *= c; gg.w *= c; }
    adam1(pp.x, gg.x, mm.x, vv.x, lr, b1, b2, eps, bc1, bc2, w, decoupled);
    adam1(pp.y, gg.y, mm.y, vv.y, lr, b1, b2, eps, bc1, bc2, w, decoupled);
    adam1(pp.z, gg.z, mm.z, vv.z, lr, b1, b2, eps, bc1, bc2, w, decoupled);
    adam1(pp.w, gg.w, mm.w, vv.w, lr, b1, b2, eps, bc1, bc2, w, decoupled);
    reinterpret_cast<float4*>(p)[i] = pp;
    reinterpret_cast<float4*>(m)[i] = mm;
    reinterpret_cast<float4*>(v)[i] = vv;
    if (ema) {
      float4 e = reinterpret_cast<float4*>(ema)[i];
      e.x = __fmaf_rn(decay, e.x, keep * pp.x);
      e.y = __fmaf_rn(decay, e.y, keep * pp.y);
      e.z = __fmaf_rn(decay, e.z, keep * pp.z);
      e.w = __fmaf_rn(decay, e.w, keep * pp.w);
      reinterpret_cast<float4*>(ema)[i] = e;
    }
    if (shadow) {
      bf16x4 b = {(bf16)pp.x, (bf16)pp.y, (bf16)pp.z, (bf16)pp.w};
      reinterpret_cast<bf16x4*>(shadow)[i] = b;
    }
  }
  for (long i = n4 * 4 + blockIdx.x * (long)blockDim.x + threadIdx.x; i < n; i += (long)gridDim.x * blockDim.x) {
    float pp = p[i], mm = m[i], vv = v[i], gi = g[i];
    if (coef) gi *= c;
    adam1(pp, gi, mm, vv, lr, b1, b2, eps, bc1, bc2, nodecay && nodecay[i >> 6] ? 0.f : wd, decoupled);
    p[i] = pp; m[i] = mm; v[i] = vv;
    if (ema) ema[i] = __fmaf_rn(decay, ema[i], keep * pp);
    if (shadow) shadow[i] = (bf16)pp;
  }
}

__device__ __forceinline__ float sgd1(float& p, float g, float& vel, bool has_vel, float lr, float mom) {
// ... 104 lines not shown
```

Before: 93350 images/sec.

## Fuse split-K weight-gradient reduction into the Adam step

Deferred split-K weight-gradient slabs are kept past backward and reduced directly inside a fused Adam step kernel. This avoids writing the reduced gradient to the arena and reading it back. Parameters the slabs do not cover are updated by a range-restricted Adam kernel, and zero_grad only clears those uncovered ranges. It adds planning state that must match between the eager pass and graph capture, and a new kernel whose per-element work grows with the number of splits.

```diff
diff --git a/dcnn_amd/csrc/host/dcnn/nn.hpp b/dcnn_amd/csrc/host/dcnn/nn.hpp
--- a/dcnn_amd/csrc/host/dcnn/nn.hpp
+++ b/dcnn_amd/csrc/host/dcnn/nn.hpp
@@ -14,6 +14,7 @@
 
 struct ParamArena;
 struct OptimSegments;
+struct WgradStepPlan;
 struct Param {
   std::string name;
   std::vector<int64_t> shape;
@@ -37,6 +38,8 @@
   long wt_tiles = 0;
   bool wt_valid = false;
   void refresh_transposes();
+  std::shared_ptr<const WgradStepPlan> step_plan;
+  Tensor step_ranges;
 };
 
 class Layer {
@@ -430,10 +433,13 @@
   std::vector<double> layer_flops(const std::vector<int64_t>& in) const;
   std::vector<BatchNorm*> batchnorms();
   void zero_grad();
+  void set_fused_wgrad_step(bool on) { fused_step_ = on; }
+  bool fused_wgrad_step() const { return fused_step_; }
   size_t num_parameters();
   const std::vector<std::unique_ptr<Layer>>& layers() const { return layers_; }
   const std::string& name() const { return name_; }
   void set_backward_hook(std::function<void(size_t)> f) { bwd_hook_ = std::move(f); }
+  bool has_backward_hook() const { return (bool)bwd_hook_; }
 
   json::Value get_config() const;
   void print_config() const;
@@ -450,6 +456,7 @@
   Device dev_ = Device::cpu();
   bool training_ = true;
   bool initialized_ = false;
+  bool fused_step_ = false;
   std::shared_ptr<ParamArena> arena_;
   std::function<void(size_t)> bwd_hook_;
   void pack_params();
@@ -524,6 +531,7 @@
   void swap_ema(const std::vector<Param*>& params);
   float last_grad_norm() const;
   virtual bool capturable() const { return false; }
+  virtual bool fuses_wgrad_step() const { return false; }
   virtual long step_count() const { return t_; }
   virtual void set_step_count(long t) { t_ = t; }
   virtual void before_replay();
@@ -567,11 +575,15 @@
       : Optimizer(lr), b1_(b1), b2_(b2), eps_(eps), wd_(wd), decoupled_(decoupled) {}
   void step(const std::vector<Param*>& params) override;
   bool capturable() const override { return true; }
+  bool fuses_wgrad_step() const override { return !tail(); }
   void before_replay() override;
 
  protected:
   float b1_, b2_, eps_, wd_;
   bool decoupled_;
+
+ private:
+  bool step_from_slabs(ParamArena* a, const std::vector<Param*>& params);
 };
 
 class LayerwiseState {
@@ -596,6 +608,7 @@
   explicit LAMB(float lr = 1e-3f, double b1 = 0.9, double b2 = 0.999, float eps = 1e-6f, float wd = 0.01f)
       : Adam(lr, (float)b1, (float)b2, eps, wd, false), b1d_(b1), b2d_(b2) {}
   void step(const std::vector<Param*>& params) override;
+  bool fuses_wgrad_step() const override { return false; }
 
  private:
   double b1d_, b2d_;
diff --git a/dcnn_amd/csrc/host/dcnn/ops.hpp b/dcnn_amd/csrc/host/dcnn/ops.hpp
--- a/dcnn_amd/csrc/host/dcnn/ops.hpp
+++ b/dcnn_amd/csrc/host/dcnn/ops.hpp
@@ -1,5 +1,6 @@
 #pragma once
 #include <cstdint>
+#include <vector>
 
 namespace dcnn {
 
@@ -84,8 +85,24 @@
 }
 
 namespace gpu_ops {
-void begin_deferred_reduce();
+void begin_deferred_reduce(bool keep = false);
 void end_deferred_reduce();
+struct KeptSlab {
+  const float* slab;
+  float* out;
+  long n;
+  int splits;
+};
+std::vector<KeptSlab> kept_slabs();
+bool kept_pending();
+void reduce_kept(const uint8_t* skip);
+void adam_slabs(const uint8_t* take, const long* offs, const uint8_t* nodecay, float* p, float* m, float* v,
+                void* shadow, long n, float b1, float b2, float eps, float wd, bool decoupled, const float* hyper);
+void adam_ranges(float* p, const float* g, float* m, float* v, void* shadow, long n, float b1, float b2, float eps,
+                 float wd, bool decoupled, const float* hyper, const uint8_t* nodecay, const void* ranges, int nranges,
+                 int units);
+void zero_ranges(float* g, const void* ranges, int nranges, int units);
+long fused_wgrad_steps();
 void flush_deferred_reduce();
 void set_fault(int f);
 void input_to_nhwc(const float* x, void* y, int N, int C, int HW);
diff --git a/dcnn_amd/csrc/host/dcnn/tensor.hpp b/dcnn_amd/csrc/host/dcnn/tensor.hpp
--- a/dcnn_amd/csrc/host/dcnn/tensor.hpp
+++ b/dcnn_amd/csrc/host/dcnn/tensor.hpp
@@ -37,6 +37,7 @@
 void* alloc(size_t nbytes);
 void free(void* p);
 size_t cached_bytes();
+size_t reserved_bytes();
 void empty_cache();
 void copy(void* dst, const void* src, size_t nbytes, int kind);
 void copy2_d2d(void* d0, const void* s0, size_t n0, void* d1, const void* s1, size_t n1);
diff --git a/dcnn_amd/csrc/host/nn.cpp b/dcnn_amd/csrc/host/nn.cpp
--- a/dcnn_amd/csrc/host/nn.cpp
+++ b/dcnn_amd/csrc/host/nn.cpp
@@ -2,6 +2,7 @@
 
 #include "../kernels/fusion_plan.h"
 #include "../kernels/optim_segments.h"
+#include "../kernels/wgrad_step_plan.h"
 
 #include <algorithm>
 #include <chrono>
@@ -1795,7 +1796,11 @@
 
 void Sequential::zero_grad() {
   if (arena_) {
-    gpu_ops::zero(arena_->grad.data(), (long)arena_->grad.nbytes());
+    if (fused_step_ && arena_->step_plan)
+      gpu_ops::zero_ranges(arena_->grad.ptr<float>(), arena_->step_ranges.defined() ? arena_->step_ranges.data() : nullptr,
+                           (int)arena_->step_plan->ranges.size(), arena_->step_plan->units);
+    else
+      gpu_ops::zero(arena_->grad.data(), (long)arena_->grad.nbytes());
     return;
   }
   for (auto* p : parameters()) {
@@ -1850,7 +1855,7 @@
     return !(v && std::string(v) == "0");
   }();
   const bool stem_bn_fold = dev_.is_gpu() && stem_bn_env && layers_.size() > 1;
-  if (defer) gpu_ops::begin_deferred_reduce();
+  if (defer) gpu_ops::begin_deferred_reduce(fused_step_ && arena_ != nullptr);
   try {
     for (size_t i = layers_.size(); i-- > 0;) {
       layers_[i]->set_micro_batch(mb);
@@ -1871,7 +1876,10 @@
       if (bwd_hook_) bwd_hook_(i);
     }
   } catch (...) {
-    if (defer) gpu_ops::end_deferred_reduce();
+    if (defer) {
+      gpu_ops::flush_deferred_reduce();
+      gpu_ops::end_deferred_reduce();
+    }
     throw;
   }
   if (defer) gpu_ops::end_deferred_reduce();
@@ -2332,6 +2340,65 @@
   ++hyper_t_;
 }
 
+bool Adam::step_from_slabs(ParamArena* a, const std::vector<Param*>& params) {
+  const std::vector<gpu_ops::KeptSlab> kept = gpu_ops::kept_slabs();
+  float* g0 = a->grad.ptr<float>();
+  const long n = (long)a->n;
+  std::vector<WgradStepEntry> q(kept.size());
+  for (size_t k = 0; k < kept.size(); ++k) {
+    q[k] = WgradStepEntry{-1, kept[k].n, kept[k].splits, 0};
+    for (const Param* p : params)
+      if (p->grad.defined() && p->grad.ptr<float>() == kept[k].out && p->value.numel() == kept[k].n) {
+        q[k].off = (long)(kept[k].out - g0);
+        q[k].nodecay = no_decay_ && p->no_decay ? 1 : 0;
+        break;
+      }
+  }
+  if (tail() || !a->step_plan || !same_queue(*a->step_plan, n, q)) {
+    if (gpu::Graph::capturing())
+      throw std::runtime_error("Adam: the weight-gradient slab queue changed inside a graph capture");
+    if (a->step_plan) {
+      long at = 0;
+      auto zero_run = [&](long b, long e) {
+        if (e > b) gpu_ops::zero(g0 + b, (e - b) * 4);
+      };
+      for (const ArenaRange& r : a->step_plan->ranges) {
+        zero_run(at, r.begin);
+        at = r.end;
+      }
+      zero_run(at, a->step_plan->n);
+    }
+    gpu_ops::reduce_kept(nullptr);
+    a->step_plan.reset();
+    a->step_ranges = Tensor();
+    if (!tail()) {
+      auto plan = std::make_shared<WgradStepPlan>(plan_wgrad_step(n, q));
+      if (!plan->ranges.empty()) {
+        const size_t bytes = plan->ranges.size() * sizeof(ArenaRange);
+        a->step_ranges = Tensor::empty({(int64_t)bytes}, DType::U8, a->value.device());
+        gpu::copy(a->step_ranges.data(), plan->ranges.data(), bytes, 0);
+      }
+      a->step_plan = plan;
+    }
+    return false;
+  }
+  const WgradStepPlan& plan = *a->step_plan;
+  std::vector<long> offs(q.size());
+  std::vector<uint8_t> nd(q.size());
+  for (size_t k = 0; k < q.size(); ++k) {
+    offs[k] = q[k].off;
+    nd[k] = (uint8_t)q[k].nodecay;
+  }
+  gpu_ops::adam_slabs(plan.eligible.data(), offs.data(), nd.data(), a->value.ptr<float>(), a->m.ptr<float>(),
+                      a->v.ptr<float>(), a->shadow.data(), n, b1_, b2_, eps_, wd_, decoupled_, hyper_.ptr<float>());
+  gpu_ops::reduce_kept(plan.eligible.data());
+  gpu_ops::adam_ranges(a->value.ptr<float>(), g0, a->m.ptr<float>(), a->v.ptr<float>(), a->shadow.data(), n, b1_, b2_,
+                       eps_, wd_, decoupled_, hyper_.ptr<float>(),
+                       no_decay_ ? static_cast<const uint8_t*>(a->nodecay.data()) : nullptr,
+                       a->step_ranges.defined() ? a->step_ranges.data() : nullptr, (int)plan.ranges.size(), plan.units);
+  return true;
+}
+
 void Adam::step(const std::vector<Param*>& params) {
   if (tail()) prepare(params);
   if (ParamArena* a = whole_arena(params)) {
@@ -2340,6 +2407,10 @@
     ++hyper_t_;
     gpu_ops::adam_hyper_step(hyper_.ptr<float>(), b1_, b2_);
     const uint8_t* nodecay = no_decay_ ? static_cast<const uint8_t*>(a->nodecay.data()) : nullptr;
+    if (gpu_ops::kept_pending() && step_from_slabs(a, params)) {
+      a->refresh_transposes();
+      return;
+    }
     if (tail())
       gpu_ops::adam_tail(a->value.ptr<float>(), a->grad.ptr<float>(), a->m.ptr<float>(), a->v.ptr<float>(),
                          a->shadow.data(), (long)a->n, 0.f, b1_, b2_, eps_, 1.f, 1.f, wd_, decoupled_,
diff --git a/dcnn_amd/csrc/host/ops_gpu.hip b/dcnn_amd/csrc/host/ops_gpu.hip
--- a/dcnn_amd/csrc/host/ops_gpu.hip
+++ b/dcnn_amd/csrc/host/ops_gpu.hip
@@ -125,6 +125,13 @@
   BlockPool& bp = pool();
   std::lock_guard<std::mutex> g(bp.mu);
   return bp.cached;
+}
+size_t reserved_bytes() {
+  BlockPool& bp = pool();
+  std::lock_guard<std::mutex> g(bp.mu);
+  size_t n = 0;
+  for (const auto& kv : bp.owner) n += kv.second.second;
+  return n;
 }
 void empty_cache() {
   BlockPool& bp = pool();
@@ -426,8 +433,11 @@
 };
 std::vector<PendingRed> g_pending;
 bool g_defer = false;
+bool g_keep = false;
+bool g_kept = false;
+long g_fused_steps = 0;
 size_t g_pending_bytes = 0;
-void launch_pending();
+void launch_pending(const uint8_t* skip = nullptr);
 size_t reduce_flush_bytes() {
   static const size_t v = [] {
     const char* e = std::getenv("DCNN_REDUCE_FLUSH_MB");
@@ -450,7 +460,7 @@
     g_pending.push_back({hold, gw, n, splits});
     if (gb) g_pending.push_back({bhold, gb, nb, splits});
     g_pending_bytes += (size_t)n * splits * 4 + (gb ? (size_t)nb * splits * 4 : 0);
-    if (reduce_flush_bytes() && g_pending_bytes >= reduce_flush_bytes()) launch_pending();
+    if (!g_keep && reduce_flush_bytes() && g_pending_bytes >= reduce_flush_bytes()) launch_pending();
     return;
   }
   if (gb)
@@ -469,35 +479,84 @@
 }
 }
 
-void begin_deferred_reduce() { g_defer = true; }
+void begin_deferred_reduce(bool keep) {
+  if (!g_pending.empty()) launch_pending();
+  g_defer = true;
+  g_keep = keep;
+  g_kept = false;
+}
 void set_fault(int f) { g_fault = f; }
-void flush_deferred_reduce() {
-  const bool on = g_defer;
-  end_deferred_reduce();
-  g_defer = on;
-}
+void flush_deferred_reduce() { launch_pending(); }
 void end_deferred_reduce() {
-  launch_pending();
+  if (!g_keep) launch_pending();
+  g_kept = g_defer && g_keep;
   g_defer = false;
-}
+  g_keep = false;
+}
+bool kept_pending() { return g_kept; }
 
 namespace {
-void launch_pending() {
-  for (size_t b = 0; b < g_pending.size(); b += kMaxRed) {
-    MultiRed t{};
-    t.count = (int)std::min(g_pending.size() - b, (size_t)kMaxRed);
-    for (int k = 0; k < t.count; ++k) {
-      const PendingRed& e = g_pending[b + k];
-      t.e[k].slab = e.slab.ptr<float>();
-      t.e[k].out = e.out;
-      t.e[k].n = e.n;
-      t.e[k].splits = e.splits;
+void launch_pending(const uint8_t* skip) {
+  MultiRed t{};
+  for (size_t k = 0; k < g_pending.size(); ++k) {
+    if (skip && skip[k]) continue;
+    const PendingRed& e = g_pending[k];
+    RedEnt& r = t.e[t.count++];
+    r.slab = e.slab.ptr<float>();
+    r.out = e.out;
+    r.n = e.n;
+    r.splits = e.splits;
+    if (t.count == kMaxRed) {
+      multi_splitk_reduce(t, cur());
+      t = MultiRed{};
     }
-    multi_splitk_reduce(t, cur());
-  }
+  }
+  multi_splitk_reduce(t, cur());
   g_pending.clear();
   g_pending_bytes = 0;
-}
+  g_kept = false;
+}
+}
+
+std::vector<KeptSlab> kept_slabs() {
+  std::vector<KeptSlab> out;
+  if (g_defer) return out;
+  for (const PendingRed& e : g_pending) out.push_back({e.slab.ptr<float>(), e.out, e.n, e.splits});
+  return out;
+}
+void reduce_kept(const uint8_t* skip) { launch_pending(skip); }
+long fused_wgrad_steps() { return g_fused_steps; }
+
+void adam_slabs(const uint8_t* take, const long* offs, const uint8_t* nodecay, float* p, float* m, float* v,
+                void* shadow, long n, float b1, float b2, float eps, float wd, bool decoupled, const float* hyper) {
+  const AdamArena a{p, m, v, static_cast<bf16*>(shadow), n, 0.f, b1, b2, eps, 1.f, 1.f, wd, decoupled ? 1 : 0, hyper};
+  MultiStep t{};
+  for (size_t k = 0; k < g_pending.size(); ++k) {
+    if (!take[k]) continue;
+    const PendingRed& e = g_pending[k];
+    StepEnt& r = t.e[t.count++];
+    r.slab = e.slab.ptr<float>();
+    r.off = offs[k];
+    r.n = e.n;
+    r.splits = e.splits;
+    r.nodecay = nodecay[k];
+    if (t.count == kMaxRed) {
+      multi_splitk_step(t, a, cur());
+      t = MultiStep{};
+    }
+  }
+  multi_splitk_step(t, a, cur());
+  ++g_fused_steps;
+}
+
+void adam_ranges(float* p, const float* g, float* m, float* v, void* shadow, long n, float b1, float b2, float eps,
+                 float wd, bool decoupled, const float* hyper, const uint8_t* nodecay, const void* ranges, int nranges,
+                 int units) {
+  const AdamArena a{p, m, v, static_cast<bf16*>(shadow), n, 0.f, b1, b2, eps, 1.f, 1.f, wd, decoupled ? 1 : 0, hyper};
+  adam_step_ranges(a, g, nodecay, static_cast<const ArenaRange*>(ranges), nranges, units, cur());
+}
+void zero_ranges(float* g, const void* ranges, int nranges, int units) {
+  dcnn::zero_ranges(g, static_cast<const ArenaRange*>(ranges), nranges, units, cur());
 }
 
 void input_to_nhwc(const float* x, void* y, int N, int C, int HW) { nchw_to_nhwc(kBF16, x, y, N, C, HW, cur()); }
diff --git a/dcnn_amd/csrc/host/train.cpp b/dcnn_amd/csrc/host/train.cpp
--- a/dcnn_amd/csrc/host/train.cpp
+++ b/dcnn_amd/csrc/host/train.cpp
@@ -5,6 +5,7 @@
 #include <chrono>
 #include <cmath>
 #include <cstdio>
+#include <cstdlib>
 #include <cstring>
 #include <filesystem>
 #include <fstream>
@@ -69,7 +70,18 @@
         if (dp->draw_counter().defined()) bn0.emplace_back(dp->draw_counter(), dp->draw_counter().clone());
   }
   const long t0 = opt_.step_count();
+  static const bool fused_env = [] {
+    const char* v = std::getenv("DCNN_FUSED_WGRAD_STEP");
+    return !(v && std::string(v) == "0");
+  }();
+  const bool fused = fused_env && !grad_hook_ && !model_.has_backward_hook() && opt_.fuses_wgrad_step() &&
+                     a->shadow.defined() && a->count == params.size();
   auto eager = [&] {
+    struct Scope {
+      Sequential& m;
+      ~Scope() { m.set_fused_wgrad_step(false); }
+    } scope{model_};
+    model_.set_fused_wgrad_step(fused);
     model_.zero_grad();
     LossResult r = loss_(model_.forward(sx_), sy_);
     model_.backward(r.grad);
diff --git a/dcnn_amd/csrc/kernels/api.h b/dcnn_amd/csrc/kernels/api.h
--- a/dcnn_amd/csrc/kernels/api.h
+++ b/dcnn_amd/csrc/kernels/api.h
@@ -4,6 +4,7 @@
 
 #include "fusion_plan.h"
 #include "optim_segments.h"
+#include "wgrad_step_plan.h"
 typedef __bf16 bf16;
 
 namespace dcnn {
@@ -275,6 +276,20 @@
 void sgd_step(float* p, const float* g, float* vel, bf16* shadow, long n, float lr, float mom, const float* hyper,
               hipStream_t s);
 void adam_scalars(float* hyper, float b1, float b2, hipStream_t s);
+struct AdamArena {
+  float *p, *m, *v;
+  bf16* shadow;
+  long n;
+  float lr, b1, b2, eps, bc1, bc2, wd;
+  int decoupled;
+  const float* hyper;
+};
+struct StepEnt { const float* slab; long off, n; int splits, unit0, chunks, groups, vec, wpc, nodecay; };
+struct MultiStep { int count; StepEnt e[kMaxRed]; };
+void multi_splitk_step(MultiStep t, const AdamArena& a, hipStream_t s);
+void adam_step_ranges(const AdamArena& a, const float* g, const uint8_t* nodecay, const ArenaRange* ranges,
+                      int nranges, int units, hipStream_t s);
+void zero_ranges(float* g, const ArenaRange* ranges, int nranges, int units, hipStream_t s);
 int grad_sumsq_blocks(long n);
 void grad_sumsq(const float* g, long n, float max_norm, float* part, unsigned* ticket, float* out, hipStream_t s);
 void adam_step_tail(float* p, const float* g, float* m, float* v, bf16* shadow, long n, float lr, float b1, float b2,
diff --git a/dcnn_amd/csrc/kernels/bindings.cpp b/dcnn_amd/csrc/kernels/bindings.cpp
--- a/dcnn_amd/csrc/kernels/bindings.cpp
+++ b/dcnn_amd/csrc/kernels/bindings.cpp
@@ -638,6 +638,45 @@
   m.def("adam_scalars", [](uintptr_t hyper, float b1, float b2, uintptr_t st) {
     adam_scalars(P<float*>(hyper), b1, b2, S(st));
   });
+  m.def("multi_splitk_step", [](std::vector<std::array<int64_t, 5>> ents, std::array<int64_t, 5> arena,
+                                std::array<float, 7> step, int dec, uintptr_t hyper, uintptr_t st) {
+    const AdamArena a{P<float*>((uintptr_t)arena[0]), P<float*>((uintptr_t)arena[1]), P<float*>((uintptr_t)arena[2]),
+                      P<bf16*>((uintptr_t)arena[3]), (long)arena[4], step[0], step[1], step[2], step[3], step[4],
+                      step[5], step[6], dec, P<const float*>(hyper)};
+    for (size_t b = 0; b < ents.size(); b += kMaxRed) {
+      MultiStep t{};
+      t.count = (int)std::min(ents.size() - b, (size_t)kMaxRed);
+      for (int k = 0; k < t.count; ++k) {
+        const auto& e = ents[b + k];
+        t.e[k].slab = P<const float*>((uintptr_t)e[0]);
+        t.e[k].off = e[1]; t.e[k].n = e[2]; t.e[k].splits = (int)e[3]; t.e[k].nodecay = (int)e[4];
+      }
+      multi_splitk_step(t, a, S(st));
+    }
+  });
+  m.def("wgrad_step_plan", [](long n, std::vector<std::array<int64_t, 4>> ents) {
+    std::vector<WgradStepEntry> q;
+    for (const auto& e : ents) q.push_back({(long)e[0], (long)e[1], (int)e[2], (int)e[3]});
+    const WgradStepPlan p = plan_wgrad_step(n, q);
+    std::vector<int> elig(p.eligible.begin(), p.eligible.end());
+    std::vector<std::array<int64_t, 3>> rows;
+    for (const ArenaRange& r : p.ranges) rows.push_back({r.begin, r.end, (int64_t)r.unit0});
+    return py::make_tuple(elig, py::bytes(reinterpret_cast<const char*>(p.covered.data()), p.covered.size()), rows,
+                          p.units);
+  });
+  m.def("adam_step_ranges", [](std::array<int64_t, 5> arena, uintptr_t g, std::array<float, 7> step, int dec,
+                               uintptr_t hyper, uintptr_t nodecay, uintptr_t ranges, int nranges, int units,
+                               uintptr_t st) {
+    static_assert(sizeof(ArenaRange) == 24, "ArenaRange is three 8-byte words");
+    const AdamArena a{P<float*>((uintptr_t)arena[0]), P<float*>((uintptr_t)arena[1]), P<float*>((uintptr_t)arena[2]),
+                      P<bf16*>((uintptr_t)arena[3]), (long)arena[4], step[0], step[1], step[2], step[3], step[4],
+                      step[5], step[6], dec, P<const float*>(hyper)};
+    adam_step_ranges(a, P<const float*>(g), P<const uint8_t*>(nodecay), P<const ArenaRange*>(ranges), nranges, units,
+                     S(st));
+  });
+  m.def("zero_ranges", [](uintptr_t g, uintptr_t ranges, int nranges, int units, uintptr_t st) {
+    zero_ranges(P<float*>(g), P<const ArenaRange*>(ranges), nranges, units, S(st));
+  });
   m.def("sgd_step", [](uintptr_t p, uintptr_t g, uintptr_t vel, uintptr_t shadow, long n, float lr, float mom,
                        uintptr_t hyper, uintptr_t st) {
     sgd_step(P<float*>(p), P<const float*>(g), P<float*>(vel), P<bf16*>(shadow), n, lr, mom, P<const float*>(hyper),
diff --git a/dcnn_amd/csrc/kernels/loss_optim.hip b/dcnn_amd/csrc/kernels/loss_optim.hip
--- a/dcnn_amd/csrc/kernels/loss_optim.hip
+++ b/dcnn_amd/csrc/kernels/loss_optim.hip
@@ -300,6 +300,214 @@
 void sgd_step(float* p, const float* g, float* vel, bf16* shadow, long n, float lr, float mom, const float* hyper,
               hipStream_t s) {
   hipLaunchKernelGGL(sgd_kernel, dim3(grid_for(n, 256, 4096)), dim3(256), 0, s, p, g, vel, shadow, n, lr, mom, hyper);
+  DCNN_LAUNCH_CHECK();
+}
+
+static constexpr int kStepG = 16;
+
+__global__ void __launch_bounds__(256) multi_splitk_step_kernel(MultiStep t, AdamArena a) {
+  constexpr int G = kStepG;
+  int k = 0;
+  for (int lo = 0, hi = t.count - 1; lo <= hi;) {
+    const int mid = (lo + hi) >> 1;
+    if (t.e[mid].unit0 <= (int)blockIdx.x) {
+      k = mid;
+      lo = mid + 1;
+    } else {
+      hi = mid - 1;
+    }
+  }
+  const float* slab = t.e[k].slab;
+  const long n = t.e[k].n, off = t.e[k].off;
+  const int splits = t.e[k].splits, groups = t.e[k].groups, vec = t.e[k].vec, wpc = t.e[k].wpc;
+  const int lane = threadIdx.x & 63, w = threadIdx.x >> 6;
+  const int chunk = (blockIdx.x - t.e[k].unit0) * (4 / wpc) + w / wpc, wj = w % wpc;
+  float lr = a.lr, bc1 = a.bc1, bc2 = a.bc2;
+  if (a.hyper) { lr = a.hyper[0]; bc1 = a.hyper[1]; bc2 = a.hyper[2]; }
+  const float wd = t.e[k].nodecay ? 0.f : a.wd;
+  __shared__ float4 red[4][64];
+  float4 acc = make_float4(0.f, 0.f, 0.f, 0.f);
+  if (vec) {
+    const long i4 = (long)chunk * 64 + lane;
+    const bool ok = i4 * 4 < n;
+    float4* p4 = reinterpret_cast<float4*>(a.p + off) + i4;
+    float4* m4 = reinterpret_cast<float4*>(a.m + off) + i4;
+    float4* v4 = reinterpret_cast<float4*>(a.v + off) + i4;
+    float4 pp = make_float4(0.f, 0.f, 0.f, 0.f), mm = pp, vv = pp;
+    if (ok && wj == 0) { pp = *p4; mm = *m4; vv = *v4; }
+    for (int g = 0; g < groups; ++g) {
+      const int s0 = g * G * wpc + wj * G;
+      float4 x[G];
+#pragma unroll
+      for (int u = 0; u < G; ++u)
+        x[u] = (ok && s0 + u < splits) ? reinterpret_cast<const float4*>(slab + (long)(s0 + u) * n)[i4]
+                                       : make_float4(0.f, 0.f, 0.f, 0.f);
+#pragma unroll
+      for (int u = 0; u < G; ++u) { acc.x += x[u].x; acc.y += x[u].y; acc.z += x[u].z; acc.w += x[u].w; }
+    }
+    if (wpc > 1) {
+      red[w][lane] = acc;
+      __syncthreads();
+      if (wj > 0) return;
+      for (int j = 1; j < wpc; ++j) {
+        const float4 r = red[w + j][lane];
+        acc.x += r.x; acc.y += r.y; acc.z += r.z; acc.w += r.w;
+      }
+    }
+    if (!ok) return;
+    adam1(pp.x, 0.f + acc.x, mm.x, vv.x, lr, a.b1, a.b2, a.eps, bc1, bc2, wd, a.decoupled);
+    adam1(pp.y, 0.f + acc.y, mm.y, vv.y, lr, a.b1, a.b2, a.eps, bc1, bc2, wd, a.decoupled);
+    adam1(pp.z, 0.f + acc.z, mm.z, vv.z, lr, a.b1, a.b2, a.eps, bc1, bc2, wd, a.decoupled);
+    adam1(pp.w, 0.f + acc.w, mm.w, vv.w, lr, a.b1, a.b2, a.eps, bc1, bc2, wd, a.decoupled);
+    *p4 = pp;
+    *m4 = mm;
+    *v4 = vv;
+    if (a.shadow) {
+      bf16x4 b = {(bf16)pp.x, (bf16)pp.y, (bf16)pp.z, (bf16)pp.w};
+      reinterpret_cast<bf16x4*>(a.shadow + off)[i4] = b;
+    }
+  } else {
+    const long i = (long)chunk * 64 + lane;
+    const bool ok = i < n;
+    float pp = 0.f, mm = 0.f, vv = 0.f;
+    if (ok && wj == 0) { pp = a.p[off + i]; mm = a.m[off + i]; vv = a.v[off + i]; }
+    for (int g = 0; g < groups; ++g) {
+      const int s0 = g * G * wpc + wj * G;
+      float x[G];
+#pragma unroll
+      for (int u = 0; u < G; ++u) x[u] = (ok && s0 + u < splits) ? slab[(long)(s0 + u) * n + i] : 0.f;
+#pragma unroll
+      for (int u = 0; u < G; ++u) acc.x += x[u];
+    }
+    if (wpc > 1) {
+      red[w][lane] = acc;
+      __syncthreads();
+      if (wj > 0) return;
+      for (int j = 1; j < wpc; ++j) acc.x += red[w + j][lane].x;
+    }
+    if (!ok) return;
+    adam1(pp, 0.f + acc.x, mm, vv, lr, a.b1, a.b2, a.eps, bc1, bc2, wd, a.decoupled);
+    a.p[off + i] = pp;
+    a.m[off + i] = mm;
+    a.v[off + i] = vv;
+    if (a.shadow) a.shadow[off + i] = (bf16)pp;
+  }
+}
+
+void multi_splitk_step(MultiStep t, const AdamArena& a, hipStream_t s) {
+  if (t.count <= 0) return;
+  if (t.count > kMaxRed) throw std::runtime_error("multi_splitk_step: too many entries");
+  const bool aligned = ((uintptr_t)a.p % 16) == 0 && ((uintptr_t)a.m % 16) == 0 && ((uintptr_t)a.v % 16) == 0 &&
+                       ((uintptr_t)a.shadow % 8) == 0;
+  for (int k = 0; k < t.count; ++k) {
+    StepEnt& e = t.e[k];
+    if (!e.slab || e.n < 1 || e.splits < 1 || e.off < 0 || e.off > a.n || e.n > a.n - e.off)
+      throw std::invalid_argument("multi_splitk_step: entry " + std::to_string(k) + " (offset " + std::to_string(e.off) +
+                                  ", " + std::to_string(e.n) + " elements, " + std::to_string(e.splits) +
+                                  " slabs) does not lie in an arena of " + std::to_string(a.n) + " elements");
+    e.vec = (e.n % 4 == 0 && e.off % 4 == 0 && aligned && ((uintptr_t)e.slab % 16) == 0) ? 1 : 0;
+    e.wpc = e.splits <= kStepG ? 1 : (e.splits <= 2 * kStepG ? 2 : 4);
+    e.groups = (e.splits + kStepG * e.wpc - 1) / (kStepG * e.wpc);
+  }
+  std::stable_sort(t.e, t.e + t.count, [](const StepEnt& x, const StepEnt& y) { return x.groups > y.groups; });
+  long units = 0;
+  for (int k = 0; k < t.count; ++k) {
+    StepEnt& e = t.e[k];
+    const long per = e.vec ? 256 : 64;
+    const long chunks = (e.n + per - 1) / per;
+    const int cpb = 4 / e.wpc;
+    if (chunks > 0x7fffffffl || units + (chunks + cpb - 1) / cpb > 0x7fffffffl)
+      throw std::invalid_argument("multi_splitk_step: more than 2^31 - 1 work units");
+    e.chunks = (int)chunks;
+    e.unit0 = (int)units;
+    units += (chunks + cpb - 1) / cpb;
+  }
+  hipLaunchKernelGGL(multi_splitk_step_kernel, dim3((unsigned)units), dim3(256), 0, s, t, a);
+  DCNN_LAUNCH_CHECK();
+}
+
+__device__ __forceinline__ int range_of(const ArenaRange* __restrict__ r, int nranges, int unit) {
+  int k = 0;
+  for (int lo = 0, hi = nranges - 1; lo <= hi;) {
+    const int mid = (lo + hi) >> 1;
+    if (r[mid].unit0 <= unit) {
+      k = mid;
+      lo = mid + 1;
+    } else {
+      hi = mid - 1;
+    }
+  }
+  return k;
+}
+
+__global__ void __launch_bounds__(256) adam_ranges_kernel(AdamArena a, const float* __restrict__ g,
+                                                          const uint8_t* __restrict__ nodecay,
+                                                          const ArenaRange* __restrict__ ranges, int nranges) {
+  const int k = range_of(ranges, nranges, blockIdx.x);
+  const long end = ranges[k].end;
+  const long i = ranges[k].begin + ((long)((int)blockIdx.x - ranges[k].unit0) * 256 + threadIdx.x) * 4;
+  if (i >= end) return;
+  float lr = a.lr, bc1 = a.bc1, bc2 = a.bc2;
+  if (a.hyper) { lr = a.hyper[0]; bc1 = a.hyper[1]; bc2 = a.hyper[2]; }
+  const float wd = nodecay && nodecay[i >> 6] ? 0.f : a.wd;
+  if (i + 4 <= end) {
+    float4 pp = *reinterpret_cast<float4*>(a.p + i), gg = *reinterpret_cast<const float4*>(g + i);
+    float4 mm = *reinterpret_cast<float4*>(a.m + i), vv = *reinterpret_cast<float4*>(a.v + i);
+    adam1(pp.x, gg.x, mm.x, vv.x, lr, a.b1, a.b2, a.eps, bc1, bc2, wd, a.decoupled);
+    adam1(pp.y, gg.y, mm.y, vv.y, lr, a.b1, a.b2, a.eps, bc1, bc2, wd, a.decoupled);
+    adam1(pp.z, gg.z, mm.z, vv.z, lr, a.b1, a.b2, a.eps, bc1, bc2, wd, a.decoupled);
+    adam1(pp.w, gg.w, mm.w, vv.w, lr, a.b1, a.b2, a.eps, bc1, bc2, wd, a.decoupled);
+    *reinterpret_cast<float4*>(a.p + i) = pp;
+    *reinterpret_cast<float4*>(a.m + i) = mm;
+    *reinterpret_cast<float4*>(a.v + i) = vv;
+    if (a.shadow) {
+      bf16x4 b = {(bf16)pp.x, (bf16)pp.y, (bf16)pp.z, (bf16)pp.w};
+      *reinterpret_cast<bf16x4*>(a.shadow + i) = b;
+    }
+    return;
+  }
+  for (long j = i; j < end; ++j) {
+    float pp = a.p[j], mm = a.m[j], vv = a.v[j];
+    adam1(pp, g[j], mm, vv, lr, a.b1, a.b2, a.eps, bc1, bc2, wd, a.decoupled);
+    a.p[j] = pp; a.m[j] = mm; a.v[j] = vv;
+    if (a.shadow) a.shadow[j] = (bf16)pp;
+  }
+}
+
+__global__ void __launch_bounds__(256) zero_ranges_kernel(float* __restrict__ g, const ArenaRange* __restrict__ ranges,
+                                                          int nranges) {
+  const int k = range_of(ranges, nranges, blockIdx.x);
+  const long end = ranges[k].end;
+  const long i = ranges[k].begin + ((long)((int)blockIdx.x - ranges[k].unit0) * 256 + threadIdx.x) * 4;
+  if (i >= end) return;
+  if (i + 4 <= end) {
+    *reinterpret_cast<float4*>(g + i) = make_float4(0.f, 0.f, 0.f, 0.f);
+    return;
+  }
+  for (long j = i; j < end; ++j) g[j] = 0.f;
+}
+
+static void check_ranges_launch(const char* who, const void* base, const ArenaRange* ranges, int nranges, int units) {
+  if (nranges < 0 || units < 0 || (nranges > 0 && (!ranges || units < 1)))
+    throw std::invalid_argument(std::string(who) + ": " + std::to_string(nranges) + " ranges in " +
+                                std::to_string(units) + " units");
+  if (reinterpret_cast<uintptr_t>(base) % 16) throw std::invalid_argument(std::string(who) + ": 16-byte aligned buffers only");
+}
+
+void adam_step_ranges(const AdamArena& a, const float* g, const uint8_t* nodecay, const ArenaRange* ranges, int nranges,
+                      int units, hipStream_t s) {
+  check_ranges_launch("adam_step_ranges", a.p, ranges, nranges, units);
+  if (((uintptr_t)g % 16) || ((uintptr_t)a.m % 16) || ((uintptr_t)a.v % 16) || ((uintptr_t)a.shadow % 8))
+    throw std::invalid_argument("adam_step_ranges: 16-byte aligned buffers only");
+  if (nranges == 0) return;
+  hipLaunchKernelGGL(adam_ranges_kernel, dim3(units), dim3(256), 0, s, a, g, nodecay, ranges, nranges);
+  DCNN_LAUNCH_CHECK();
+}
+
+void zero_ranges(float* g, const ArenaRange* ranges, int nranges, int units, hipStream_t s) {
+  check_ranges_launch("zero_ranges", g, ranges, nranges, units);
+  if (nranges == 0) return;
+  hipLaunchKernelGGL(zero_ranges_kernel, dim3(units), dim3(256), 0, s, g, ranges, nranges);
   DCNN_LAUNCH_CHECK();
 }
 
diff --git a/dcnn_amd/csrc/kernels/wgrad_step_plan.cpp b/dcnn_amd/csrc/kernels/wgrad_step_plan.cpp
--- /dev/null
+++ b/dcnn_amd/csrc/kernels/wgrad_step_plan.cpp
@@ -0,0 +1,72 @@
+#include "wgrad_step_plan.h"
+
+#include <stdexcept>
+#include <string>
+
+namespace dcnn {
+
+namespace {
+void blocks_of(const WgradStepEntry& e, long n, long& b0, long& b1) {
+  b0 = b1 = 0;
+  if (e.off < 0 || e.n < 1 || e.off >= n) return;
+  const long end = e.n > n - e.off ? n : e.off + e.n;
+  b0 = e.off / kStepBlock;
+  b1 = (end + kStepBlock - 1) / kStepBlock;
+}
+}
+
+WgradStepPlan plan_wgrad_step(long n, const std::vector<WgradStepEntry>& queue) {
+  if (n < 0) throw std::invalid_argument("plan_wgrad_step: arena of " + std::to_string(n) + " elements");
+  const long nblocks = (n + kStepBlock - 1) / kStepBlock;
+  if (nblocks >= (1l << 31))
+    throw std::invalid_argument("plan_wgrad_step: arena of " + std::to_string(n) + " elements exceeds 2^31 blocks");
+  WgradStepPlan p;
+  p.n = n;
+  p.entries = queue;
+  p.eligible.assign(queue.size(), 0);
+  p.covered.assign((size_t)nblocks, 0);
+  std::vector<uint8_t> touch((size_t)nblocks, 0);
+  for (const WgradStepEntry& e : queue) {
+    long b0, b1;
+    blocks_of(e, n, b0, b1);
+    for (long b = b0; b < b1; ++b)
+      if (touch[(size_t)b] < 2) ++touch[(size_t)b];
+  }
+  for (size_t k = 0; k < queue.size(); ++k) {
+    const WgradStepEntry& e = queue[k];
+    if (e.off < 0 || e.n < 1 || e.splits < 1 || e.off % kStepBlock != 0) continue;
+    if (e.off >= n || e.n > n - e.off) continue;
+    long b0, b1;
+    blocks_of(e, n, b0, b1);
+    bool alone = true;
+    for (long b = b0; b < b1 && alone; ++b) alone = touch[(size_t)b] == 1;
+    if (!alone) continue;
+    p.eligible[k] = 1;
+    p.covered_elems += e.n;
+    for (long b = b0; b < b1; ++b) p.covered[(size_t)b] = 1;
+  }
+  for (long b = 0; b < nblocks;) {
+    if (p.covered[(size_t)b]) {
+      ++b;
+      continue;
+    }
+    long e = b;
+    while (e < nblocks && !p.covered[(size_t)e]) ++e;
+    ArenaRange r{};
+    r.begin = b * kStepBlock;
+    r.end = e * kStepBlock < n ? e * kStepBlock : n;
+    r.unit0 = p.units;
+    const long units = (r.end - r.begin + kRangeUnitElems - 1) / kRangeUnitElems;
+    if (units > (1l << 30) - p.units) throw std::invalid_argument("plan_wgrad_step: too many range units");
+    p.units += (int)units;
+    p.ranges.push_back(r);
+    b = e;
+  }
+  return p;
+}
+
+bool same_queue(const WgradStepPlan& p, long n, const std::vector<WgradStepEntry>& queue) {
+  return p.n == n && p.entries == queue;
+}
+
+}
diff --git a/dcnn_amd/csrc/kernels/wgrad_step_plan.h b/dcnn_amd/csrc/kernels/wgrad_step_plan.h
--- /dev/null
+++ b/dcnn_amd/csrc/kernels/wgrad_step_plan.h
@@ -0,0 +1,39 @@
+#pragma once
+#include <cstdint>
+#include <vector>
+
+namespace dcnn {
+
+constexpr int kStepBlock = 64;
+constexpr int kRangeUnitElems = 1024;
+
+struct WgradStepEntry {
+  long off;
+  long n;
+  int splits;
+  int nodecay;
+};
+inline bool operator==(const WgradStepEntry& a, const WgradStepEntry& b) {
+  return a.off == b.off && a.n == b.n && a.splits == b.splits && a.nodecay == b.nodecay;
+}
+
+struct ArenaRange {
+  long begin, end;
+  int unit0, pad;
+};
+
+struct WgradStepPlan {
+  long n = 0;
+  std::vector<WgradStepEntry> entries;
+  std::vector<uint8_t> eligible;
+  std::vector<uint8_t> covered;
+  std::vector<ArenaRange> ranges;
+  int units = 0;
+  long covered_elems = 0;
+};
+
+WgradStepPlan plan_wgrad_step(long n, const std::vector<WgradStepEntry>& queue);
+
+bool same_queue(const WgradStepPlan& p, long n, const std::vector<WgradStepEntry>& queue);
+
+}
```

Measured after the change: 94110 images/sec, median of 6. Within noise of the previous version (+0.8%).
